# YujiaoShi/HighlyAccurate

Measured on AMD Instinct MI355X. Metric: image-pairs/sec through N-iter LM pose loop, KITTI shapes, higher is better.
Workload: dtype bf16; 1 GPU; BASELINE configs[1]: LM_S2GP.forward(mode='test'), sat 512x512, grd 256x1024, VGG-16 two-branch, level 3, 5 LM iters x 3 levels, 3-DoF, random-init weights; pairs_per_gpu=32, global_batch=32, parallelism=batch-sharded x1, no collective

## Files before the change

### highlyaccurate_amd/VGG.py

```python
from __future__ import annotations

import ctypes as C

import torch
import torch.nn as nn

from . import _lib

_W_ORDER = ['conv0', 'conv2', 'conv5', 'conv7', 'conv10', 'conv12', 'conv14',
            'conv_dec1.1', 'conv_dec1.3', 'conv_dec2.1', 'conv_dec2.3', 'conv_dec3.1', 'conv_dec3.3',
            'conf0.1', 'conf1.1', 'conf2.1', 'conf3.1']
_LEVEL_SEL = {-1: [0], -2: [1], -3: [2], 2: [1, 2], 3: [0, 1, 2], 4: [0, 1, 2, 3]}
_CH = (256, 128, 64, 16)


def _dtype_code(precision: str) -> int:
    if precision == 'bf16':
        return _lib.HLA_BF16
    if precision == 'fp16':
        return _lib.HLA_F16
    if precision == 'fp32':
        return _lib.HLA_F32
    if precision == 'fp16x3':
        return _lib.HLA_F16X3
    raise ValueError(f"precision must be 'fp32', 'fp16x3', 'bf16' or 'fp16', got {precision!r}")


def _param_table(module: 'VGGUnet'):
    sd = dict(module.named_parameters())
    prm = _lib.VggParams()
    keep, versions = [], []
    pad = {11: (64, 128), 12: (64, 64), 16: (1, 64)}
    for i, name in enumerate(_W_ORDER):
        w = sd[name + '.weight']
        versions.append((w.data_ptr(), w._version))
        w = w.detach().contiguous().float()
        if i in pad:
            if module.level != 4:
                continue
            wp = torch.zeros(pad[i][0], pad[i][1], 3, 3, device=w.device, dtype=torch.float32)
            wp[:w.shape[0], :w.shape[1]] = w
            w = wp
        keep.append(w)
        prm.w[i] = w.data_ptr()
        if i < 7:
            b = sd[name + '.bias']
            if i == 0:
                versions.append((b.data_ptr(), b._version))
            b = b.detach().contiguous().float()
            keep.append(b)
            prm.b[i] = b.data_ptr()
    return prm, keep, tuple(versions)


def _packed_weights(module: 'VGGUnet', prm, versions, dt: int, device):
    key = (dt, str(device), versions)
    cache = module.__dict__.setdefault('_hla_packed', {})
    if cache.get('key') != key:
        lib = _lib.load()
        buf = cache.get('buf')
        nbytes = lib.hla_vgg_packed_weight_bytes(dt)
        if buf is None or buf.numel() != nbytes or buf.device != device:
            buf = torch.empty(nbytes, dtype=torch.uint8, device=device)
        _lib.check(lib.hla_vgg_pack_weights(C.byref(prm), _lib.ptr(buf), dt, _lib.stream_ptr()), 'hla_vgg_pack_weights')
        cache['key'], cache['buf'] = key, buf
    return cache['buf']


def _alloc(*shape, dtype, device):
    return torch.empty(*shape, dtype=dtype, device=device)


def _image_window(x: torch.Tensor):
    x = x.float()
    B, _, H, W = x.shape
    sb, sc, sh, sw = x.stride()
    if not (sw == 1 and sh == W and sc >= H * W and (B == 1 or sb == 3 * sc)):
        x = x.contiguous()
        sc = H * W
    return x, sc


@_lib.on_device(lambda module, x, *a, **k: x)
def vgg_forward_nhwc(module: 'VGGUnet', x: torch.Tensor, want_conf: bool = True, defer_norm: bool = False,
                     save_for_backward: bool = False, first_row8: int = 0, feat16: bool = False, first_col32: int = 0,
                     col_state: dict = None):
    _lib.require_gpu(x, 'VGGUnet input')
    if x.dim() != 4 or x.shape[1] != 3:
        raise ValueError(f'expected [B,3,H,W], got {tuple(x.shape)}')
    lib = _lib.load()
    x, x_plane = _image_window(x)
    B, _, H, W = x.shape
    _lib.same_device(('input', x), ('parameters', module.conv0.weight))
    dt = _dtype_code(module.precision)
    prm, keep, versions = _param_table(module)
    packed = _packed_weights(module, prm, versions, dt, x.device)
    L = 4 if module.level == 4 else 3
    fdt = torch.float32
    if feat16:
        if not (defer_norm and not save_for_backward and L == 3 and dt in (_lib.HLA_BF16, _lib.HLA_F16)):
            raise ValueError("feat16 needs precision 'bf16' / 'fp16', defer_norm=True, level 3 and no save_for_backward")
        fdt = torch.float16
    fold = bool(getattr(module, 'folded', False))
    if fold:
        if feat16 or first_row8:
            raise ValueError('VGGUnet_G2S: feat16 / first_row8 do not apply to the folded maps')
        if W % 16:
            raise ValueError(f'VGGUnet_G2S folds [h,w] -> [2h,w/2] down to the W/8-wide map: W must be a multiple of 16, got {W}')

    def hw(l, folded):
        h, w = H >> (3 - l), W >> (3 - l)
        return (2 * h, w // 2) if folded else (h, w)

    feats = [_alloc(B, *hw(l, fold), 64 if l == 3 else _CH[l], device=x.device, dtype=fdt) for l in range(L)]
    confs = [torch.empty(B, *hw(l, fold and l > 0), device=x.device, dtype=torch.float32) if want_conf else None
             for l in range(L)]
    inv_norm = torch.empty(L, B, device=x.device, dtype=torch.float64)
    fp = (C.c_void_p * 4)(*([f.data_ptr() for f in feats] + [0] * (4 - L)))
    cp = (C.c_void_p * 4)(*([(c.data_ptr() if c is not None else 0) for c in confs] + [0] * (4 - L)))
    flags = (_lib.HLA_VGG_WANT_CONF if want_conf else 0) | (_lib.HLA_VGG_DEFER_NORM if defer_norm else 0) | \
            (_lib.HLA_VGG_FEAT16 if feat16 else 0) | (_lib.HLA_VGG_FOLD_DECODER if fold else 0)
    nbytes = lib.hla_vgg_workspace_bytes_flags(B, H, W, L, dt, flags) if fold else lib.hla_vgg_workspace_bytes(B, H, W, L, dt)
    ws = _alloc(nbytes, dtype=torch.uint8, device=x.device)
    if save_for_backward:
        if not defer_norm:
            raise ValueError('save_for_backward needs defer_norm=True (the backward works on the raw maps)')
        flags |= _lib.HLA_VGG_SAVE_FOR_BACKWARD
    c32 = _check_first_col32(first_col32, W)
    rc = lib.hla_vgg_forward_cols(_lib.ptr(x), x_plane, C.byref(prm), _lib.ptr(packed), fp, cp, _lib.ptr(inv_norm), _lib.ptr(ws), nbytes,
                                  B, H, W, L, dt, flags, int(first_row8), c32, None, _lib.stream_ptr())
    _lib.check(rc, 'hla_vgg_forward')
    if col_state is not None:
        col_state.update(x=x, x_plane=x_plane, prm=prm, keep=keep, packed=packed, feats=feats, inv_norm=inv_norm, ws=ws, B=B, H=H, W=W,
                         L=L, dt=dt, flags=flags, first_row8=int(first_row8), first_col32=c32)
    if save_for_backward:
        return feats, confs, inv_norm, dict(x=x, x_version=x._version, x_plane=x_plane, ws=ws, feats=feats, inv_norm=inv_norm, dt=dt, L=L)
    return feats, confs, inv_norm


def _check_first_col32(first_col32, W: int) -> int:
    c = int(first_col32)
    if c < 0 or (c > 0 and 128 * c >= W):
        raise ValueError(f'first_col32 must be 0 or leave a column of the maps (128 * first_col32 < W = {W}), got {first_col32}')
    return c


def promised_cols(first_col32: int):
    c = int(first_col32)
    return (16 * c + 2, 32 * c + 6, 64 * c + 14) if c > 0 else (0, 0, 0)


@_lib.on_device(lambda state, gate, *a, **k: gate)
def vgg_fixup_nhwc(state: dict, gate: torch.Tensor, one_launch: bool = True) -> None:
    s = state
    if not s or not s['first_col32']:
        return
    if gate.dtype != torch.int32 or gate.numel() != s['B'] or not gate.is_contiguous() or gate.device != s['x'].device:
        raise ValueError('gate must be a contiguous int32 [B] tensor on the device of the maps')
    L = s['L']
    fp = (C.c_void_p * 4)(*([f.data_ptr() for f in s['feats']] + [0] * (4 - L)))
    rc = _lib.load().hla_vgg_fixup(_lib.ptr(s['x']), s['x_plane'], C.byref(s['prm']), _lib.ptr(s['packed']), fp,
                                   _lib.ptr(s['inv_norm']), _lib.ptr(s['ws']), s['ws'].numel(), s['B'], s['H'], s['W'], L, s['dt'],
                                   s['flags'], s['first_row8'], s['first_col32'], _lib.ptr(gate), 1 if one_launch else 0,
                                   _lib.stream_ptr())
    _lib.check(rc, 'hla_vgg_fixup')


@_lib.on_device(lambda modules, xs, *a, **k: xs[0])
def vgg_forward_pair_nhwc(modules, xs, first_row8=(0, 0), feat16: bool = False, first_col32=(0, 0), col_state: dict = None):
    lib = _lib.load()
    if len(modules) != 2 or len(xs) != 2:
        raise ValueError('vgg_forward_pair_nhwc takes two modules and two images')
    dt = _dtype_code(modules[0].precision)
    if _dtype_code(modules[1].precision) != dt or any(m.level == 4 or getattr(m, 'folded', False) for m in modules):
        raise ValueError('vgg_forward_pair_nhwc: two unfolded extractors of one precision, level 3')
    if feat16 and dt not in (_lib.HLA_BF16, _lib.HLA_F16):
        raise ValueError("feat16 needs precision 'bf16' / 'fp16'")
    if xs[0].dim() != 4 or xs[1].dim() != 4 or xs[0].shape[1] != 3 or xs[1].shape[1] != 3 or xs[0].shape[0] != xs[1].shape[0]:
        raise ValueError(f'expected two [B,3,H,W] images with one B, got {tuple(xs[0].shape)} and {tuple(xs[1].shape)}')
    br = (_lib.VggBranch * 2)()
    keep, out = [], []
    for k, (module, x) in enumerate(zip(modules, xs)):
        _lib.require_gpu(x, 'VGGUnet input')
        x, x_plane = _image_window(x)
        B, _, H, W = x.shape
        _lib.same_device(('input', x), ('parameters', module.conv0.weight), ('first input', xs[0]))
        prm, kp, versions = _param_table(module)
        packed = _packed_weights(module, prm, versions, dt, x.device)
        feats = [_alloc(B, H >> (3 - l), W >> (3 - l), _CH[l], device=x.device, dtype=torch.float16 if feat16 else torch.float32)
                 for l in range(3)]
        inv_norm = torch.empty(3, B, device=x.device, dtype=torch.float64)
        nbytes = lib.hla_vgg_workspace_bytes(B, H, W, 3, dt)
        ws = _alloc(nbytes, dtype=torch.uint8, device=x.device)
        b = br[k]
        b.x, b.x_plane, b.params, b.packed_weights = x.data_ptr(), x_plane, C.pointer(prm), packed.data_ptr()
        for l in range(3):
            b.feat[l] = feats[l].data_ptr()
        b.inv_norm, b.workspace, b.workspace_bytes = inv_norm.data_ptr(), ws.data_ptr(), nbytes
        b.H, b.W, b.first_row8, b.first_col32 = H, W, int(first_row8[k]), _check_first_col32(first_col32[k], W)
        keep += [x, prm, kp, packed, ws]
        out.append((feats, inv_norm))
        if k == 0 and col_state is not None:
            col_state.update(x=x, x_plane=x_plane, prm=prm, keep=kp, packed=packed, feats=feats, inv_norm=inv_norm, ws=ws, B=B, H=H, W=W,
                             L=3, dt=dt, flags=_lib.HLA_VGG_DEFER_NORM | (_lib.HLA_VGG_FEAT16 if feat16 else 0),
                             first_row8=int(first_row8[k]), first_col32=b.first_col32)
    flags = _lib.HLA_VGG_DEFER_NORM | (_lib.HLA_VGG_FEAT16 if feat16 else 0)
    paired = C.c_int(0)
    rc = lib.hla_vgg_forward_pair(br, xs[0].shape[0], 3, dt, flags, C.byref(paired), _lib.stream_ptr())
    _lib.check(rc, 'hla_vgg_forward_pair')
    return out[0], out[1], bool(paired.value)


@_lib.on_device(lambda module, ctx, *a, **k: ctx['x'])
def vgg_backward_nhwc(module: 'VGGUnet', ctx: dict, d_feats, confs=None, d_confs=None, scale_invariant: bool = False,
                      first_row8: int = 0, flat: bool = False, dense: bool = False, stats: dict = None,
                      wgrad_two_phase: int = 0, workspace: torch.Tensor = None):
    lib = _lib.load()
    x, dt = ctx['x'], ctx['dt']
    if x._version != ctx.get('x_version', x._version):
        raise RuntimeError('the input image saved for the backward of VGGUnet has been modified by an inplace operation '
                           f"(version {x._version}, expected {ctx['x_version']}): conv0's weight gradient reads it again")
    B, _, H, W = x.shape
    prm, keep, versions = _param_table(module)
    cache = module.__dict__.setdefault('_hla_packed_T', {})
    key = (dt, str(x.device), versions)
    if cache.get('key') != key:
        buf = torch.empty(lib.hla_vgg_packed_weight_T_bytes(dt), dtype=torch.uint8, device=x.device)
        _lib.check(lib.hla_vgg_pack_weights_T(C.byref(prm), _lib.ptr(buf), dt, _lib.stream_ptr()), 'hla_vgg_pack_weights_T')
        cache['key'], cache['buf'] = key, buf
    sd = dict(module.named_parameters())
    grads, gs = {}, _lib.VggGrads()
    shapes = [(name + '.weight', tuple(sd[name + '.weight'].shape)) for name in _W_ORDER[:11]] + \
             [(name + '.bias', tuple(sd[name + '.bias'].shape)) for name in _W_ORDER[:7]]
    sizes = [int(torch.Size(shp).numel()) for _, shp in shapes]
    flat_buf = torch.empty(sum(sizes), device=x.device, dtype=torch.float32)
    o = 0
    for (key, shp), n in zip(shapes, sizes):
        grads[key] = flat_buf[o:o + n].view(shp)
        o += n
    for i, name in enumerate(_W_ORDER[:11]):
        gs.dw[i] = grads[name + '.weight'].data_ptr()
        if i < 7:
            gs.db[i] = grads[name + '.bias'].data_ptr()
    L = ctx.get('L', 3)
    padded = {}
    if L == 4:
        for i, name, shape in ((11, 'conv_dec3.1', (64, 128, 3, 3)), (12, 'conv_dec3.3', (64, 64, 3, 3))):
            g = torch.empty(shape, device=x.device, dtype=torch.float32)
            padded[name + '.weight'] = g
            gs.dw[i] = g.data_ptr()
    cp = dcp = None
    if d_confs is not None:
        dcs = [d.contiguous().float() for d in d_confs]
        cp = (C.c_void_p * 4)(*([c.data_ptr() for c in confs] + [0] * (4 - L)))
        dcp = (C.c_void_p * 4)(*([d.data_ptr() for d in dcs] + [0] * (4 - L)))
        for l in range(L):
            name = f'conf{l}.1.weight'
            if l == 3:
                g = torch.empty(1, 64, 3, 3, device=x.device, dtype=torch.float32)
                padded[name] = g
            else:
                g = torch.empty_like(sd[name], dtype=torch.float32, memory_format=torch.contiguous_format)
                grads[name] = g
            gs.dw[13 + l] = g.data_ptr()
    dfs = [d.contiguous().float() for d in d_feats]
    fp = (C.c_void_p * 4)(*([f.data_ptr() for f in ctx['feats']] + [0] * (4 - L)))
    dp = (C.c_void_p * 4)(*([d.data_ptr() for d in dfs] + [0] * (4 - L)))
    fold = bool(getattr(module, 'folded', False))
    nbytes = lib.hla_vgg_bwd_workspace_bytes_flags(B, H, W, L, dt, _lib.HLA_VGG_BWD_FOLD_DECODER) if fold \
        else lib.hla_vgg_bwd_workspace_bytes(B, H, W, L, dt)
    if workspace is None:
        ws = torch.empty(nbytes, dtype=torch.uint8, device=x.device)
    else:
        ws = workspace
        if ws.dtype != torch.uint8 or ws.device != x.device or not ws.is_contiguous():
            raise ValueError('workspace must be a contiguous uint8 tensor on the device of the input')
        if ws.numel() < nbytes:
            raise ValueError(f'workspace too small: {ws.numel()} bytes, the backward needs {nbytes}')
    rc = lib.hla_vgg_backward(_lib.ptr(x), ctx.get('x_plane', 0), C.byref(prm), _lib.ptr(cache['buf']), _lib.ptr(ctx['ws']), fp, _lib.ptr(ctx['inv_norm']),
                              dp, cp, dcp, C.byref(gs), _lib.ptr(ws), nbytes, B, H, W, L, dt,
                              (_lib.HLA_VGG_BWD_SCALE_INVARIANT if scale_invariant else 0)
                              | (_lib.HLA_VGG_BWD_DENSE if dense else 0)
                              | (_lib.HLA_VGG_BWD_WGRAD_TWO_PHASE if int(wgrad_two_phase) & 1 else 0)
                              | (_lib.HLA_VGG_BWD_WGRAD0_UNFUSED if int(wgrad_two_phase) & 2 else 0)
                              | (_lib.HLA_VGG_BWD_FOLD_DECODER if getattr(module, 'folded', False) else 0),
                              int(first_row8), _lib.stream_ptr())
    _lib.check(rc, 'hla_vgg_backward')
    if stats is not None and fold:
        stats['live_tiles'], stats['total_tiles'] = 0, 0
    elif stats is not None:
        torch.cuda.current_stream().synchronize()
        live, total = C.c_longlong(0), C.c_longlong(0)
        _lib.check(lib.hla_vgg_backward_live_tiles(_lib.ptr(ws), B, H, W, L, dt, C.byref(live), C.byref(total)),
                   'hla_vgg_backward_live_tiles')
        stats['live_tiles'], stats['total_tiles'] = live.value, total.value
    for name, g in padded.items():
        co, ci = sd[name].shape[:2]
        grads[name] = g[:co, :ci].contiguous()
    return (grads, flat_buf) if flat else grads


class VGGUnet(nn.Module):
    def __init__(self, level, estimate_depth=0, precision: str = 'fp32'):
        super().__init__()
        if estimate_depth:
            raise NotImplementedError('estimate_depth=1 (Ford height heads, VGG.py:85-118) is out of scope')
        if level not in _LEVEL_SEL:
            raise NotImplementedError(f'VGGUnet level {level}: the reference defines -1, -2, -3, 2, 3, 4')
        self.level = level
        _dtype_code(precision)
        self.precision = precision

        def c(ci, co, bias):
            return nn.Conv2d(ci, co, kernel_size=(3, 3), stride=(1, 1), padding=1, bias=bias)

        self.conv0, self.conv2 = c(3, 64, True), c(64, 64, True)
        self.conv5, self.conv7 = c(64, 128, True), c(128, 128, True)
        self.conv10, self.conv12, self.conv14 = c(128, 256, True), c(256, 256, True), c(256, 256, True)
        self.conv_dec1 = nn.Sequential(nn.ReLU(inplace=True), c(384, 128, False), nn.ReLU(inplace=True), c(128, 128, False))
        self.conv_dec2 = nn.Sequential(nn.ReLU(inplace=True), c(192, 64, False), nn.ReLU(inplace=True), c(64, 64, False))
        self.conv_dec3 = nn.Sequential(nn.ReLU(inplace=True), c(128, 32, False), nn.ReLU(inplace=True), c(32, 16, False))
        self.conf0 = nn.Sequential(nn.ReLU(), c(256, 1, False), nn.Sigmoid())
        self.conf1 = nn.Sequential(nn.ReLU(), c(128, 1, False), nn.Sigmoid())
        self.conf2 = nn.Sequential(nn.ReLU(), c(64, 1, False), nn.Sigmoid())
        self.conf3 = nn.Sequential(nn.ReLU(), c(16, 1, False), nn.Sigmoid())

    def forward(self, x):
        if torch.is_grad_enabled() and any(p.requires_grad for p in self.parameters()):
            names = [n for n, _ in self.named_parameters()]
            out = _VggFn.apply(self, names, x, *[p for _, p in self.named_parameters()])
            L = len(out) // 2
            feats, confs = list(out[:L]), list(out[L:])
        else:
            feats, confs, _ = vgg_forward_nhwc(self, x, want_conf=True)
        sel = _LEVEL_SEL[self.level]
        view = lambda i: (feats[i][..., :_CH[i]] if i == 3 else feats[i]).permute(0, 3, 1, 2)
        return [view(i) for i in sel], [confs[i].unsqueeze(1) for i in sel]


class VGGUnet_G2S(VGGUnet):
    folded = True

    def __init__(self, level, precision: str = 'fp32'):
        super().__init__(level, precision=precision)


class _VggFn(torch.autograd.Function):

    @staticmethod
    def forward(ctx, module, names, x, *params):
        feats, confs, inv, c = vgg_forward_nhwc(module, x, want_conf=True, defer_norm=True, save_for_backward=True)
        B = x.shape[0]
        normed = [(f.double() * inv[l].view(B, 1, 1, 1)).float() for l, f in enumerate(feats)]
        ctx.module, ctx.names, ctx.saved, ctx.n_levels = module, names, c, len(confs)
        confs = tuple(confs)
        ctx.save_for_backward(*confs)
        return tuple(normed) + confs

    @staticmethod
    def backward(ctx, *grads):
        c = ctx.saved
        if c is None:
            raise RuntimeError('VGGUnet: backward through the same forward twice (the saved activations were released after the '
                               'first backward; retain_graph is not supported by the HIP backward)')
        confs = list(ctx.saved_tensors)
        L = ctx.n_levels
        d_feats = [g if g is not None else torch.zeros_like(c['feats'][l]) for l, g in enumerate(grads[:L])]
        d_confs = [g if g is not None else torch.zeros_like(confs[l]) for l, g in enumerate(grads[L:])]
        g = vgg_backward_nhwc(ctx.module, c, d_feats, confs, d_confs, scale_invariant=False)
        ctx.saved = None
        return (None, None, None) + tuple(g.get(n) for n in ctx.names)


def L2_norm(x):
    B = x.shape[0]
    n = x.reshape(B, -1).norm(dim=1).clamp_min(1e-12)
    return x / n.view(B, 1, 1, 1)
```

### highlyaccurate_amd/_lib.py

```python
from __future__ import annotations

import ctypes as C
import os

import torch

HERE = os.path.dirname(os.path.abspath(__file__))
LIB_PATH = os.environ.get('HLA_LIB') or os.path.join(HERE, 'libhla.so')

HLA_F32, HLA_BF16, HLA_F16, HLA_F16X3 = 0, 1, 2, 3
HLA_VGG_WANT_CONF, HLA_VGG_DEFER_NORM, HLA_VGG_SAVE_FOR_BACKWARD, HLA_VGG_FEAT16 = 1, 2, 4, 8
HLA_VGG_FOLD_DECODER = 16
HLA_VGG_BWD_SCALE_INVARIANT = 1
HLA_VGG_BWD_DENSE = 2
HLA_VGG_BWD_WGRAD_TWO_PHASE = 4
HLA_VGG_BWD_WGRAD0_UNFUSED = 8
HLA_VGG_BWD_FOLD_DECODER = 16
ABI_VERSION = 32


class HlaError(RuntimeError):
    pass


class VggParams(C.Structure):
    _fields_ = [('w', C.c_void_p * 17), ('b', C.c_void_p * 7)]


class S2GLevel(C.Structure):
    _fields_ = [('sat_feat', C.c_void_p), ('grd_feat', C.c_void_p), ('grd_conf', C.c_void_p), ('xyz', C.c_void_p),
                ('sat_inv_norm', C.c_void_p), ('grd_inv_norm', C.c_void_p),
                ('A', C.c_int), ('h', C.c_int), ('w', C.c_int), ('C', C.c_int), ('row0', C.c_int), ('grd_row_skip', C.c_int),
                ('meter_per_pixel', C.c_double), ('centre', C.c_double), ('feat_dtype', C.c_int),
                ('ray', C.c_void_p), ('depth', C.c_void_p), ('depth_row', C.c_void_p), ('depth_col', C.c_void_p),
                ('depth_h', C.c_int), ('depth_w', C.c_int)]


class S2GConfig(C.Structure):
    _fields_ = [('ford', C.c_int), ('n_levels', C.c_int), ('n_iters', C.c_int), ('level_first', C.c_int),
                ('using_weight', C.c_int), ('use_hessian', C.c_int), ('dof', C.c_int),
                ('shift_range_lat', C.c_double), ('shift_range_lon', C.c_double), ('rotation_range', C.c_double),
                ('damping', C.c_double * 3), ('keep', C.c_void_p), ('keep_stride', C.c_size_t),
                ('optimizer', C.c_int), ('beta1', C.c_double), ('beta2', C.c_double), ('count_in_view', C.c_int),
                ('grd_grad_overwrite', C.c_int), ('deterministic', C.c_int), ('proj', C.c_int),
                ('reach_mode', C.c_int), ('reach_flag', C.c_void_p), ('reach_col0', C.c_int * 4)]


class VggBranch(C.Structure):
    _fields_ = [('x', C.c_void_p), ('x_plane', C.c_size_t), ('params', C.POINTER(VggParams)), ('packed_weights', C.c_void_p),
                ('feat', C.c_void_p * 4), ('conf', C.c_void_p * 4), ('inv_norm', C.c_void_p), ('workspace', C.c_void_p),
                ('workspace_bytes', C.c_size_t), ('H', C.c_int), ('W', C.c_int), ('first_row8', C.c_int),
                ('first_col32', C.c_int)]


class FillRegion(C.Structure):
    _fields_ = [('ptr', C.c_void_p), ('chunk_bytes', C.c_size_t), ('stride_bytes', C.c_size_t), ('n_chunks', C.c_int)]


class VggGrads(C.Structure):
    _fields_ = [('dw', C.c_void_p * 17), ('db', C.c_void_p * 7)]


class S2GLevelGrad(C.Structure):
    _fields_ = [('d_sat_feat', C.c_void_p), ('d_grd_feat', C.c_void_p), ('d_grd_conf', C.c_void_p)]


class ProfRecord(C.Structure):
    _fields_ = [('kernel_id', C.c_int), ('ms', C.c_float), ('flops', C.c_double), ('bytes', C.c_double)]


HLA_POSE_LOSS_F32, HLA_POSE_LOSS_F64 = 0, 1


class PoseLossArgs(C.Structure):
    _fields_ = [('x', C.c_void_p * 3), ('x_stride', (C.c_longlong * 3) * 3), ('gt', C.c_void_p * 3), ('gt_stride', C.c_longlong * 3),
                ('coe', C.c_double * 3), ('B', C.c_int), ('N', C.c_int), ('L', C.c_int), ('gt_dtype', C.c_int)]


_lib = None


def _check_binary(lib: C.CDLL, path: str) -> None:
    lib.hla_abi_version.restype = C.c_int
    have = lib.hla_abi_version()
    if have != ABI_VERSION:
        raise HlaError(f'{path}: ABI version {have}, this binding needs {ABI_VERSION}; rebuild it '
                       f'(python -m highlyaccurate_amd.build --force)')
    try:
        fn = lib.hla_sizeof_struct
    except AttributeError:
        raise HlaError(f'{path}: no hla_sizeof_struct export; rebuild it') from None
    fn.restype, fn.argtypes = C.c_size_t, [C.c_int]
    for sid, cls in enumerate((VggParams, VggGrads, S2GLevel, S2GConfig, S2GLevelGrad, ProfRecord, PoseLossArgs, FillRegion,
                                VggBranch)):
        if fn(sid) != C.sizeof(cls):
            raise HlaError(f'{path}: sizeof({cls.__name__}) is {fn(sid)} in the library and {C.sizeof(cls)} in the binding')


def load() -> C.CDLL:
    global _lib
    if _lib is not None:
        return _lib
    from . import build as _b
    try:
        want = _b.source_hash()
    except _b.SourcesMissing as e:
        if not os.path.exists(LIB_PATH):
            raise HlaError(f'{LIB_PATH} is missing and so are its sources: {e}') from None
        want = _b.lib_hash(LIB_PATH)
    if _b.lib_hash(LIB_PATH) != want and not (os.environ.get('HLA_LIB') and os.environ.get('HLA_ALLOW_STALE') == '1'):
        if os.environ.get('HLA_LIB'):
            raise HlaError(f'{LIB_PATH} (HLA_LIB) was not built from the sources in {_b.CSRC}; rebuild it')
        if not _b.have_compiler():
            what = 'is missing' if not os.path.exists(LIB_PATH) else 'is stale (built from different sources)'
            raise HlaError(f'{LIB_PATH} {what} and there is no hipcc to rebuild it; highlyaccurate_amd has no fallback path')
        _b.build()
    lib = C.CDLL(LIB_PATH)
    _check_binary(lib, LIB_PATH)
    vp, i, sz = C.c_void_p, C.c_int, C.c_size_t
    lib.hla_last_error.restype = C.c_char_p
    lib.hla_source_hash.restype = C.c_char_p
    lib.hla_vgg_workspace_bytes.restype = sz
    lib.hla_vgg_workspace_bytes.argtypes = [i, i, i, i, i]
    lib.hla_vgg_workspace_bytes_flags.restype = sz
    lib.hla_vgg_workspace_bytes_flags.argtypes = [i, i, i, i, i, i]
    lib.hla_vgg_forward.restype = i
    lib.hla_vgg_forward.argtypes = [vp, sz, C.POINTER(VggParams), vp, C.POINTER(vp), C.POINTER(vp), vp, vp, sz,
                                    i, i, i, i, i, i, i, vp]
    lib.hla_vgg_forward_cols.restype = i
    lib.hla_vgg_forward_cols.argtypes = [vp, sz, C.POINTER(VggParams), vp, C.POINTER(vp), C.POINTER(vp), vp, vp, sz,
                                         i, i, i, i, i, i, i, i, vp, vp]
    lib.hla_vgg_fixup.restype = i
    lib.hla_vgg_fixup.argtypes = [vp, sz, C.POINTER(VggParams), vp, C.POINTER(vp), vp, vp, sz, i, i, i, i, i, i, i, i, vp, i, vp]
    lib.hla_vgg_forward_pair.restype = i
    lib.hla_vgg_forward_pair.argtypes = [C.POINTER(VggBranch), i, i, i, i, C.POINTER(i), vp]
    lib.hla_vgg_packed_weight_bytes.restype = sz
    lib.hla_vgg_packed_weight_bytes.argtypes = [i]
    lib.hla_vgg_pack_weights.restype = i
    lib.hla_vgg_pack_weights.argtypes = [C.POINTER(VggParams), vp, i, vp]
    lib.hla_vgg_packed_weight_T_bytes.restype = sz
    lib.hla_vgg_packed_weight_T_bytes.argtypes = [i]
    lib.hla_vgg_pack_weights_T.restype = i
    lib.hla_vgg_pack_weights_T.argtypes = [C.POINTER(VggParams), vp, i, vp]
    lib.hla_vgg_bwd_workspace_bytes.restype = sz
    lib.hla_vgg_bwd_workspace_bytes.argtypes = [i, i, i, i, i]
    lib.hla_vgg_bwd_workspace_bytes_flags.restype = sz
    lib.hla_vgg_bwd_workspace_bytes_flags.argtypes = [i, i, i, i, i, i]
    lib.hla_vgg_backward_live_tiles.restype = i
    lib.hla_vgg_backward_live_tiles.argtypes = [vp, i, i, i, i, i, C.POINTER(C.c_longlong), C.POINTER(C.c_longlong)]
    lib.hla_vgg_backward.restype = i
    lib.hla_vgg_backward.argtypes = [vp, sz, C.POINTER(VggParams), vp, vp, C.POINTER(vp), vp, C.POINTER(vp), C.POINTER(vp), C.POINTER(vp), C.POINTER(VggGrads),
                                     vp, sz, i, i, i, i, i, i, i, vp]
    lib.hla_resize_bilinear.restype = i
    lib.hla_resize_bilinear.argtypes = [vp, vp, vp, i, vp, vp, i, vp, vp, i, i, i, i, i, vp]
    lib.hla_sat_tile.restype = i
    lib.hla_sat_tile.argtypes = [vp, vp, vp, i, i, i, vp]
    lib.hla_grid_sample.restype = i
    lib.hla_grid_sample.argtypes = [vp, vp, vp, vp, vp, i, i, i, i, i, i, i, vp]
    lib.hla_grid_sample_bwd.restype = i
    lib.hla_grid_sample_bwd.argtypes = [vp, vp, vp, vp, vp, vp, vp, vp, i, i, i, i, i, i, i, vp]
    lib.hla_s2g_workspace_bytes.restype = sz
    lib.hla_s2g_workspace_bytes.argtypes = [C.POINTER(S2GConfig), C.POINTER(S2GLevel), i]
    lib.hla_g2s_workspace_bytes.restype = sz
    lib.hla_g2s_workspace_bytes.argtypes = [C.POINTER(S2GConfig), C.POINTER(S2GLevel), i]
    lib.hla_g2s_lm_solve.restype = i
    lib.hla_g2s_lm_solve.argtypes = [C.POINTER(S2GConfig), C.POINTER(S2GLevel), vp, i, i, vp, vp, vp, vp, sz, i, vp]
    lib.hla_g2s_pose_score_workspace_bytes.restype = sz
    lib.hla_g2s_pose_score_workspace_bytes.argtypes = [C.POINTER(S2GConfig), C.POINTER(S2GLevel), i, i]
    lib.hla_g2s_pose_score.restype = i
    lib.hla_g2s_pose_score.argtypes = [C.POINTER(S2GConfig), C.POINTER(S2GLevel), vp, i, i, vp, i, vp, vp, vp, sz, i, vp]
    lib.hla_g2s_pose_score_bwd_workspace_bytes.restype = sz
    lib.hla_g2s_pose_score_bwd_workspace_bytes.argtypes = [C.POINTER(S2GConfig), C.POINTER(S2GLevel), i, i]
    lib.hla_g2s_pose_score_bwd.restype = i
    lib.hla_g2s_pose_score_bwd.argtypes = [C.POINTER(S2GConfig), C.POINTER(S2GLevel), C.POINTER(S2GLevelGrad), vp, i, i, vp, i,
                                           vp, vp, vp, sz, i, vp]
    lib.hla_g2s_bwd_workspace_bytes.restype = sz
    lib.hla_g2s_bwd_workspace_bytes.argtypes = [C.POINTER(S2GConfig), C.POINTER(S2GLevel), i]
    lib.hla_g2s_lm_solve_bwd.restype = i
    lib.hla_g2s_lm_solve_bwd.argtypes = [C.POINTER(S2GConfig), C.POINTER(S2GLevel), C.POINTER(S2GLevelGrad), vp, i, i, vp, vp,
                                         vp, vp, vp, vp, sz, i, vp]
    lib.hla_s2g_lm_solve.restype = i
    lib.hla_s2g_lm_solve.argtypes = [C.POINTER(S2GConfig), C.POINTER(S2GLevel), vp, vp, vp, vp, vp, vp, vp, sz, i, vp]
    lib.hla_s2g_pose_score_workspace_bytes.restype = sz
    lib.hla_s2g_pose_score_workspace_bytes.argtypes = [C.POINTER(S2GConfig), C.POINTER(S2GLevel), i, i]
    lib.hla_s2g_pose_score.restype = i
    lib.hla_s2g_pose_score.argtypes = [C.POINTER(S2GConfig), C.POINTER(S2GLevel), vp, vp, vp, i, vp, vp, vp, sz, i, vp]
    lib.hla_s2g_pose_score_bwd_workspace_bytes.restype = sz
    lib.hla_s2g_pose_score_bwd_workspace_bytes.argtypes = [C.POINTER(S2GConfig), C.POINTER(S2GLevel), i, i]
    lib.hla_s2g_pose_score_bwd.restype = i
    lib.hla_s2g_pose_score_bwd.argtypes = [C.POINTER(S2GConfig), C.POINTER(S2GLevel), C.POINTER(S2GLevelGrad), vp, vp, vp, i, vp, vp,
                                           vp, sz, i, vp]
    lib.hla_s2g_bwd_workspace_bytes.restype = sz
    lib.hla_s2g_bwd_workspace_bytes.argtypes = [C.POINTER(S2GConfig), C.POINTER(S2GLevel), i]
    lib.hla_s2g_lm_solve_bwd.restype = i
    lib.hla_s2g_lm_solve_bwd.argtypes = [C.POINTER(S2GConfig), C.POINTER(S2GLevel), C.POINTER(S2GLevelGrad), vp, vp, vp, vp,
                                         vp, vp, vp, vp, sz, i, vp]
    lib.hla_zero_fill.restype = i
    lib.hla_zero_fill.argtypes = [C.POINTER(FillRegion), i, i, vp]
    lib.hla_pose_loss.restype = i
    lib.hla_pose_loss.argtypes = [C.POINTER(PoseLossArgs), vp, vp]
    lib.hla_pose_loss_bwd.restype = i
    lib.hla_pose_loss_bwd.argtypes = [C.POINTER(PoseLossArgs), C.POINTER(vp), C.POINTER(vp), C.POINTER((C.c_longlong * 3) * 3), vp]
    ll, dbl = C.c_longlong, C.c_double
    lib.hla_orien_corr_workspace_bytes.restype = sz
    lib.hla_orien_corr_workspace_bytes.argtypes = [i, i, i, i, i]
    lib.hla_orien_corr.restype = i
    lib.hla_orien_corr.argtypes = [vp, vp, vp, vp, vp, vp, vp, vp, vp, sz, i, i, i, i, i, vp]
    lib.hla_orien_corr_bwd.restype = i
    lib.hla_orien_corr_bwd.argtypes = [vp, vp, vp, vp, vp, vp, vp, vp, vp, vp, vp, sz, i, i, i, i, i, vp]
    lib.hla_orien_window_bwd.restype = i
    lib.hla_orien_window_bwd.argtypes = [vp, vp, vp, vp, i, i, i, i, i, i, vp]
    lib.hla_orien_triplet_loss.restype = i
    lib.hla_orien_triplet_loss.argtypes = [vp, vp, ll, dbl, dbl, vp, i, i, i, vp]
    lib.hla_orien_triplet_loss_bwd.restype = i
    lib.hla_orien_triplet_loss_bwd.argtypes = [vp, vp, ll, dbl, dbl, vp, vp, i, i, vp]
    lib.hla_g2s_corr_workspace_bytes.restype = sz
    lib.hla_g2s_corr_workspace_bytes.argtypes = [i, i, i, i, i]
    lib.hla_g2s_corr.restype = i
    lib.hla_g2s_corr.argtypes = [vp, vp, vp, vp, vp, vp, vp, vp, vp, sz, i, i, i, i, i, vp]
    lib.hla_g2s_corr_bwd.restype = i
    lib.hla_g2s_corr_bwd.argtypes = [vp, vp, vp, vp, vp, vp, vp, vp, vp, vp, vp, sz, i, i, i, i, i, vp]
    lib.hla_g2s_corr_triplet_loss.restype = i
    lib.hla_g2s_corr_triplet_loss.argtypes = [vp, vp, ll, vp, ll, dbl, dbl, dbl, vp, i, i, i, i, vp]
    lib.hla_g2s_corr_triplet_loss_bwd.restype = i
    lib.hla_g2s_corr_triplet_loss_bwd.argtypes = [vp, vp, ll, vp, ll, dbl, dbl, dbl, vp, vp, i, i, i, vp]
    lib.hla_prof_enable.restype = i
    lib.hla_prof_enable.argtypes = [i]
    lib.hla_prof_kernel_name.restype = C.c_char_p
    lib.hla_prof_kernel_name.argtypes = [i]
    lib.hla_prof_mfma_peak.restype = i
    lib.hla_prof_mfma_peak.argtypes = [i, i, C.c_float, C.POINTER(C.c_float), vp]
    lib.hla_prof_fetch.restype = i
    lib.hla_prof_fetch.argtypes = [C.POINTER(ProfRecord), i, C.POINTER(i)]
    _lib = lib
    return lib


def zero_fill(regions, max_blocks: int = 0, stream=None) -> None:
    if not regions:
        return
    arr = (FillRegion * len(regions))()
    for k, (t, cb, sb, n) in enumerate(regions):
        arr[k].ptr = t.data_ptr() if hasattr(t, 'data_ptr') else int(t)
        arr[k].chunk_bytes, arr[k].stride_bytes, arr[k].n_chunks = int(cb), int(sb), int(n)
    check(load().hla_zero_fill(arr, len(regions), int(max_blocks), stream_ptr() if stream is None else stream), 'hla_zero_fill')


def prof_enable(on: bool) -> None:
    load().hla_prof_enable(1 if on else 0)


def prof_fetch(max_records: int = 1 << 16):
    lib = load()
    buf = (ProfRecord * max_records)()
    n = C.c_int(0)
    lib.hla_prof_fetch(buf, max_records, C.byref(n))
    return [(lib.hla_prof_kernel_name(buf[k].kernel_id).decode(), buf[k].ms, buf[k].flops, buf[k].bytes)
            for k in range(n.value)]


def check(rc: int, what: str) -> None:
    if rc != 0:
        raise HlaError(f'{what} failed (status {rc}): {load().hla_last_error().decode()}')


def stream_ptr() -> C.c_void_p:
    return C.c_void_p(torch.cuda.current_stream().cuda_stream)


def on_device(pick):
    import functools

    def deco(fn):
        @functools.wraps(fn)
        def wrapper(*a, **k):
            t = pick(*a, **k)
            if t is None or not t.is_cuda:
                return fn(*a, **k)
            if torch.cuda.current_device() == t.device.index:
                return fn(*a, **k)
            with torch.cuda.device(t.device):
                return fn(*a, **k)
        return wrapper
    return deco


def same_device(*named) -> None:
    devs = {(n, str(t.device)) for n, t in named if t is not None}
    if len({d for _, d in devs}) > 1:
        raise ValueError('all inputs and the model must be on one device, got ' + ', '.join(f'{n}: {d}' for n, d in sorted(devs)))


def require_gpu(t: torch.Tensor, name: str) -> None:
    if not t.is_cuda:
        raise HlaError(f'{name} must live on the HIP device (got {t.device}); highlyaccurate_amd has no CPU path')


def image_pair(sat_map, grd_img, param, gpu: bool = True) -> None:
    if gpu:
        require_gpu(sat_map, 'sat_map')
        require_gpu(grd_img, 'grd_img')
    if sat_map.dim() != 4 or grd_img.dim() != 4 or sat_map.shape[0] != grd_img.shape[0] or sat_map.shape[1] != 3 \
            or grd_img.shape[1] != 3 or sat_map.shape[2] != sat_map.shape[3]:
        raise ValueError(f'expected sat_map [B,3,A,A] and grd_img [B,3,H,W] with one B, got {tuple(sat_map.shape)} '
                         f'and {tuple(grd_img.shape)}')
    same_device(('sat_map', sat_map), ('grd_img', grd_img), ('parameters', param))


def ptr(t) -> C.c_void_p:
    return C.c_void_p(0 if t is None else t.data_ptr())


def mfma_sustained_tflops(dtype_code: int, data: int, ms_target: float = 8.0) -> float:
    out = C.c_float(0.0)
    check(load().hla_prof_mfma_peak(dtype_code, data, ms_target, C.byref(out), stream_ptr()), 'hla_prof_mfma_peak')
    return float(out.value)
```

### highlyaccurate_amd/_s2gp.py

```python
from __future__ import annotations

import ctypes as C

import numpy as np
import torch
import torch.nn as nn

from . import _lib, _pose, utils
from ._autograd import _side_stream, extract_saved, extractor_grads, grad_params, take_state
from ._pose import _poses_arg, eligible_cost, pose_grid
from .VGG import VGGUnet, vgg_forward_nhwc, vgg_forward_pair_nhwc, vgg_fixup_nhwc, promised_cols

KITTI_K = [[582.9802, 0.0, 496.2420], [0.0, 482.7076, 125.0034], [0.0, 0.0, 1.0]]
FORD_K_FL = [945.391406, 0.0, 855.502825, 0.0, 945.668274, 566.372868, 0.0, 0.0, 1.0]
FORD_H_FL, FORD_W_FL = 860, 1656


_FEAT_DTYPES = {torch.float32: _lib.HLA_F32, torch.bfloat16: _lib.HLA_BF16, torch.float16: _lib.HLA_F16}

PHASE_HOOK = None


def _phase(name: str):
    h = PHASE_HOOK
    if h is not None:
        h(name)


def _camera_rays(K_ori, grd_H, grd_W, ori_H, ori_W):
    K = torch.tensor(K_ori, dtype=torch.float32).reshape(1, 3, 3)
    Ks = K.clone()
    Ks[:, :1, :] = K[:, :1, :] * grd_W / ori_W
    Ks[:, 1:2, :] = K[:, 1:2, :] * grd_H / ori_H
    Kinv = torch.inverse(Ks)
    v, u = torch.meshgrid(torch.arange(0, grd_H, dtype=torch.float32),
                          torch.arange(0, grd_W, dtype=torch.float32), indexing='ij')
    uv1 = torch.stack([u, v, torch.ones_like(u)], dim=-1).unsqueeze(0)
    return torch.sum(Kinv[:, None, None, :, :] * uv1[:, :, :, None, :], dim=-1)


def ray_table(K_ori, grd_H, grd_W, ori_H, ori_W):
    return _camera_rays(K_ori, grd_H, grd_W, ori_H, ori_W)[0].contiguous()


def ground_plane_table(K_ori, grd_H, grd_W, ori_H, ori_W):
    xyz_w = _camera_rays(K_ori, grd_H, grd_W, ori_H, ori_W)
    y = xyz_w[..., 1:2]
    w = utils.Camera_height / torch.where(torch.abs(y) > utils.EPS, y, utils.EPS * torch.ones_like(y))
    return (xyz_w * w)[0].contiguous()


def nearest_indices(n_in: int, n_out: int):
    scale = np.float32(n_in) / np.float32(n_out)
    src = np.floor(np.arange(n_out, dtype=np.float32) * scale).astype(np.int64)
    return torch.from_numpy(np.minimum(src, n_in - 1).astype(np.int32))


def polar_plane_table(grd_H, grd_W):
    v, u = torch.meshgrid(torch.arange(0, grd_H, dtype=torch.float32),
                          torch.arange(0, grd_W, dtype=torch.float32), indexing='ij')
    theta = u / grd_W * np.pi / 4
    radius = (1 - v / grd_H) * 30
    z = radius * torch.cos(np.pi / 4 - theta)
    x = -radius * torch.sin(np.pi / 4 - theta)
    y = utils.Camera_height * torch.ones_like(z)
    return torch.stack([x, y, z], dim=-1).contiguous()


def ford_K_network_input():
    K = torch.tensor(FORD_K_FL, dtype=torch.float32).reshape(3, 3)
    out = torch.zeros_like(K)
    out[0] = K[0] / FORD_W_FL * 1024
    out[1] = K[1] / FORD_H_FL * 256
    out[2] = K[2]
    return out.tolist()


def _loss_tensor_ops(shift_lats, shift_lons, thetas, gt_shift_lat, gt_shift_lon, gt_theta, coe_shift_lat, coe_shift_lon, coe_theta):
    d_lat = torch.abs(shift_lats - gt_shift_lat[:, None, None]).mean(dim=0)
    d_lon = torch.abs(shift_lons - gt_shift_lon[:, None, None]).mean(dim=0)
    d_th = torch.abs(thetas - gt_theta[:, None, None]).mean(dim=0)
    losses = coe_shift_lat * d_lat + coe_shift_lon * d_lon + coe_theta * d_th
    return (losses.mean(), losses[0] - losses[-1], d_lat[0] - d_lat[-1], d_lon[0] - d_lon[-1], d_th[0] - d_th[-1],
            losses[-1], d_lat[-1], d_lon[-1], d_th[-1])


def _pose_loss_args(xs, gts, coes):
    a = _lib.PoseLossArgs()
    B, N, L = xs[0].shape
    for k in range(3):
        a.x[k], a.gt[k], a.gt_stride[k], a.coe[k] = xs[k].data_ptr(), gts[k].data_ptr(), gts[k].stride(0), float(coes[k])
        for j in range(3):
            a.x_stride[k][j] = xs[k].stride(j)
    a.B, a.N, a.L = B, N, L
    a.gt_dtype = _lib.HLA_POSE_LOSS_F64 if gts[0].dtype == torch.float64 else _lib.HLA_POSE_LOSS_F32
    return a


class _PoseLossFn(torch.autograd.Function):

    @staticmethod
    def forward(ctx, cols, coes, gt_lat, gt_lon, gt_th, *xs):
        views = [xs[0][..., c] for c in cols] if cols is not None else list(xs)
        gts = (gt_lat, gt_lon, gt_th)
        L = views[0].shape[2]
        out = torch.empty(1 + 8 * L, dtype=gt_lat.dtype, device=views[0].device)
        args = _pose_loss_args(views, gts, coes)
        _lib.check(_lib.load().hla_pose_loss(C.byref(args), _lib.ptr(out), _lib.stream_ptr()), 'hla_pose_loss')
        ctx.save_for_backward(*xs, *gts)
        ctx.cols, ctx.coes = cols, coes
        ctx.set_materialize_grads(False)
        return (out[0],) + tuple(out[1 + j * L:1 + (j + 1) * L] for j in range(8))

    @staticmethod
    @torch.autograd.function.once_differentiable
    def backward(ctx, *g):
        cols, saved = ctx.cols, ctx.saved_tensors
        nx = 1 if cols is not None else 3
        xs, gts = saved[:nx], saved[nx:]
        if cols is not None:
            d = torch.empty_like(xs[0]) if xs[0].shape[-1] == 3 and len(set(cols)) == 3 else torch.zeros_like(xs[0])
            views, dviews, grads = [xs[0][..., c] for c in cols], [d[..., c] for c in cols], (d,)
        else:
            views = list(xs)
            grads = tuple(torch.empty(x.shape, dtype=torch.float32, device=x.device) for x in xs)
            dviews = list(grads)
        args = _pose_loss_args(views, gts, ctx.coes)
        vp = C.c_void_p
        gp, keep = (vp * 9)(), []
        for j, t in enumerate(g):
            if t is not None:
                t = t.to(gts[0].dtype).contiguous()
                keep.append(t)
                gp[j] = t.data_ptr()
        dp = (vp * 3)(*[v.data_ptr() for v in dviews])
        ds = ((C.c_longlong * 3) * 3)()
        for k in range(3):
            for j in range(3):
                ds[k][j] = dviews[k].stride(j)
        _lib.check(_lib.load().hla_pose_loss_bwd(C.byref(args), gp, dp, C.byref(ds), _lib.stream_ptr()), 'hla_pose_loss_bwd')
        return (None,) * 5 + grads


def _pose_loss(cols, xs, gts, coes):
    views = [xs[0][..., c] for c in cols] if cols is not None else list(xs)
    fused = (all(isinstance(c, (int, float)) for c in coes)
             and all(v.is_cuda and v.dtype == torch.float32 and v.dim() == 3 and v.shape == views[0].shape for v in views)
             and all(t.is_cuda and t.device == views[0].device and t.dtype == gts[0].dtype and t.dim() == 1
                     and t.shape[0] == views[0].shape[0] and not t.requires_grad for t in gts)
             and gts[0].dtype in (torch.float32, torch.float64) and 0 < views[0].shape[1] * views[0].shape[2] <= 512
             and views[0].shape[0] > 0)
    if not fused:
        return _loss_tensor_ops(*views, *gts, *coes)
    with torch.cuda.device(views[0].device):
        return _PoseLossFn.apply(cols, tuple(float(c) for c in coes), *gts, *xs)


def loss_func(loss_method, ref_feat_list, pred_feat_dict, gt_feat_dict, shift_lats, shift_lons, thetas,
              gt_shift_lat, gt_shift_lon, gt_theta, pred_uv_dict, gt_uv_dict,
              coe_shift_lat=100, coe_shift_lon=100, coe_theta=100, coe_L1=100, coe_L2=100, coe_L3=100, coe_L4=100):
    if loss_method != 0:
        raise NotImplementedError('only loss_method=0 is supported (the reference marks 1-3 as failed trials)')
    out = _pose_loss(None, (shift_lats, shift_lons, thetas), (gt_shift_lat, gt_shift_lon, gt_theta),
                     (coe_shift_lat, coe_shift_lon, coe_theta))
    return (*out, None, None, None, None)


def loss_from_trace(loss_method, trace, cols, gt_shift_lat, gt_shift_lon, gt_theta, coe_shift_lat, coe_shift_lon, coe_theta):
    if loss_method != 0:
        raise NotImplementedError('only loss_method=0 is supported (the reference marks 1-3 as failed trials)')
    out = _pose_loss(tuple(cols), (trace,), (gt_shift_lat, gt_shift_lon, gt_theta), (coe_shift_lat, coe_shift_lon, coe_theta))
    return (*out, None, None, None, None)


class S2GPBase(nn.Module):
    ford = False

    def __init__(self, args):
        super().__init__()
        self.args = args
        self.level = args.level
        self.N_iters = args.N_iters
        self.using_weight = args.using_weight
        self.loss_method = args.loss_method
        if args.level not in ((2, 3, 4) if self.ford else (3, 4)):
            raise NotImplementedError('args.level must be 3 (x15, x18, x21) or 4 (+ x24)' +
                                      (', or 2 (x18, x21)' if self.ford else "; the reference's KITTI model is shape-inconsistent at level 2"))
        proj = getattr(args, 'proj', 'geo')
        if proj not in ('geo', 'polar'):
            raise NotImplementedError(f"{type(self).__name__}: proj must be 'geo' or 'polar', got {proj!r} (the reference runs its "
                                      "polar branch for any other string, 'nn' and 'CrossAttn' included: that accident is not copied)")
        self.polar = proj == 'polar'
        if self.polar and self.ford and args.level == 2:
            raise NotImplementedError("LM_S2GP_Ford(level=2, proj='polar'): the reference pairs the whole-map loop with the "
                                      "ground-plane tables there; that combination is not built (use level 3 or 4)")
        opt = getattr(args, 'Optimizer', 'LM')
        allowed = ('LM', 'GN') if self.ford else ('LM', 'SGD', 'ADAM')
        if opt not in allowed:
            raise NotImplementedError(f"{type(self).__name__}: Optimizer must be one of {allowed} ('NN' needs the NNrefine "
                                      f"network: out of scope; the reference's Ford SGD_update raises as shipped)")
        if getattr(args, 'estimate_depth', 0):
            raise NotImplementedError('estimate_depth (Ford height heads, VGG.py:85-118) is out of scope')
        precision = getattr(args, 'precision', 'fp32')
        self.SatFeatureNet = VGGUnet(self.level, precision=precision)
        self.GrdFeatureNet = VGGUnet(self.level, precision=precision)
        if self.ford or args.rotation_range > 0:
            self.damping = nn.Parameter(torch.zeros(size=(1, 3), dtype=torch.float32))
        else:
            self.damping = nn.Parameter(torch.zeros(size=(), dtype=torch.float32))
        self.meters_per_pixel = [utils.get_meter_per_pixel() * (2 ** (3 - l)) for l in range(4)]
        self._tables = {}
        self._reach = {}
        self._ray_tables = {}
        self._depth_idx = {}
        self.last_trace = None
        self.last_normal_eq = None
        self.last_keep = None
        self.keep_normal_eq = False
        self.keep_features = False
        self.last_features = None
        self.last_reach_flag = None
        self.last_search = None
        self.last_score_loss = None

    def xyz_tables(self, grd_H: int, grd_W: int, device):
        key = (grd_H, grd_W, str(device))
        if key not in self._tables:
            K = ford_K_network_input() if self.ford else KITTI_K
            hw = [(grd_H / 2 ** (3 - l), grd_W / 2 ** (3 - l)) for l in range(4)]
            self._tables[key] = [(polar_plane_table(h, w) if self.polar else ground_plane_table(K, h, w, 256, 1024)).to(device)
                                 for h, w in hw]
        return self._tables[key][1:3] if self.level == 2 else self._tables[key]

    def ray_tables(self, grd_H: int, grd_W: int, device):
        key = (grd_H, grd_W, str(device))
        if key not in self._ray_tables:
            K = ford_K_network_input() if self.ford else KITTI_K
            self._ray_tables[key] = [ray_table(K, grd_H / 2 ** (3 - l), grd_W / 2 ** (3 - l), 256, 1024).to(device) for l in range(4)]
        return self._ray_tables[key][1:3] if self.level == 2 else self._ray_tables[key]

    def depth_indices(self, h: int, w: int, dH: int, dW: int, device):
        key = (h, w, dH, dW, str(device))
        if key not in self._depth_idx:
            self._depth_idx[key] = (nearest_indices(dH, h).to(device), nearest_indices(dW, w).to(device))
        return self._depth_idx[key]

    def _depth_arg(self, gt_depth, B: int, device):
        if gt_depth is None:
            return None
        if self.polar:
            raise NotImplementedError("proj='polar' with a depth map: the reference's polar tables have no camera rays to lift "
                                      "(models_kitti.py:742 raises IndexError)")
        if gt_depth.dim() != 3 or gt_depth.shape[0] != B or gt_depth.shape[1] < 1 or gt_depth.shape[2] < 1:
            raise ValueError(f'gt_depth must be [B,dH,dW] with B = {B}, got {tuple(gt_depth.shape)}')
        return gt_depth.detach().to(device).float().contiguous()

    def sat_first_col32(self, A: int, grd_H: int, grd_W: int) -> int:
        a = self.args
        if self.ford or self.polar or self.level != 3 or A % 8:
            return 0
        key = (A, grd_H, grd_W, float(a.shift_range_lat), float(a.shift_range_lon), float(a.rotation_range))
        if key not in self._reach:
            tables = [t.cpu() for t in self.xyz_tables(grd_H, grd_W, 'cpu')]
            mpp = [utils.get_meter_per_pixel() * utils.get_process_satmap_sidelength() / (A >> (3 - l)) for l in range(3)]
            cols = sat_reach(tables[:3], [A >> (3 - l) for l in range(3)], mpp, key[3], key[4], key[5])
            self._reach[key] = first_col32_of_reach(cols, A)
        return self._reach[key]

    def _levels(self, maps):
        if self.level != 2 or maps is None:
            return maps
        return maps[1:]

    def _config(self, n_levels: int, level_first: int) -> _lib.S2GConfig:
        a = self.args
        cfg = _lib.S2GConfig()
        cfg.ford = 1 if self.ford else 0
        cfg.n_levels, cfg.n_iters, cfg.level_first = n_levels, self.N_iters, 1 if level_first else 0
        cfg.optimizer = {'LM': 0, 'SGD': 1, 'ADAM': 2, 'GN': 3}[getattr(a, 'Optimizer', 'LM')]
        cfg.using_weight = 1 if (self.using_weight and cfg.optimizer in (0, 3)) else 0
        cfg.use_hessian = 1 if getattr(a, 'use_hessian', 0) else 0
        if self.ford:
            cfg.dof = 3
        elif a.rotation_range == 0:
            cfg.dof = 2
        elif a.shift_range_lat == 0 and a.shift_range_lon == 0:
            cfg.dof = 1
        else:
            cfg.dof = 3
        cfg.shift_range_lat, cfg.shift_range_lon = float(a.shift_range_lat), float(a.shift_range_lon)
        cfg.rotation_range = float(a.rotation_range)
        cfg.beta1, cfg.beta2 = float(getattr(a, 'beta1', 0.9)), float(getattr(a, 'beta2', 0.999))
        if getattr(a, 'train_damping', 0):
            lam = (10.0 ** (-6 + torch.sigmoid(self.damping.detach().double()) * 11.0)).reshape(-1).tolist()
        else:
            lam = [float(a.damping)] * 3
        lam = (lam + lam + lam)[:3]
        if not self.ford and cfg.dof == 1 and getattr(a, 'train_damping', 0):
            lam = [lam[0]] * 3
        for i in range(3):
            cfg.damping[i] = lam[i]
        return cfg

    def _draw_reinit(self, n_steps: int, B: int, device):
        return draw_reinit(n_steps, B, device)

    def _draw_dropout(self, lv, level_first, device):
        if not getattr(self.args, 'dropout', 0) or getattr(self.args, 'Optimizer', 'LM') != 'LM':
            return None
        L, N = len(lv), self.N_iters
        order = [l for l in range(L) for _ in range(N)] if level_first else [l for _ in range(N) for l in range(L)]
        npix = [(lv[l].h - lv[l].row0) * lv[l].w for l in range(L)]
        keep = np.zeros((len(order), max(npix)), np.uint8)
        for k, l in enumerate(order):
            inds = np.random.permutation(np.arange(npix[l]))[: npix[l] // 2]
            keep[k, inds] = 1
        return torch.from_numpy(keep).to(device)

    def _lm_structs(self, sat_feats, grd_feats, grd_confs, grd_hw, extra, level_first, sat_inv_norm, grd_inv_norm, depth=None):
        dev = sat_feats[0].device
        L = len(sat_feats)
        tables = self.xyz_tables(grd_hw[0], grd_hw[1], dev)
        rays = self.ray_tables(grd_hw[0], grd_hw[1], dev) if depth is not None else None
        cfg = self._config(L, level_first)
        lv = (_lib.S2GLevel * L)()
        for l in range(L):
            s, g = sat_feats[l], grd_feats[l]
            A, w, Cn = s.shape[1], g.shape[2], g.shape[3]
            h = tables[l].shape[0]
            row0 = 0 if self.polar else h // 2
            skip = h - g.shape[1]
            if not (s.shape[2] == A and s.shape[3] == Cn and tuple(tables[l].shape) == (h, w, 3) and 0 <= skip <= row0
                    and g.shape[0] == s.shape[0] and s.is_contiguous() and g.is_contiguous()
                    and s.dtype == g.dtype and s.dtype in _FEAT_DTYPES):
                raise ValueError(f'level {l}: inconsistent feature maps sat {tuple(s.shape)} / grd {tuple(g.shape)} '
                                 f'for a {tuple(grd_hw)} ground image')
            lv[l].sat_feat, lv[l].grd_feat, lv[l].feat_dtype = s.data_ptr(), g.data_ptr(), _FEAT_DTYPES[s.dtype]
            lv[l].grd_conf = grd_confs[l].data_ptr() if (self.using_weight and grd_confs[l] is not None) else 0
            lv[l].xyz = tables[l].data_ptr()
            if depth is not None:
                ri, ci = self.depth_indices(h, w, depth.shape[1], depth.shape[2], dev)
                lv[l].ray, lv[l].depth, lv[l].depth_row, lv[l].depth_col = rays[l].data_ptr(), depth.data_ptr(), ri.data_ptr(), ci.data_ptr()
                lv[l].depth_h, lv[l].depth_w = depth.shape[1], depth.shape[2]
            lv[l].sat_inv_norm = sat_inv_norm[l].data_ptr() if sat_inv_norm is not None else 0
            lv[l].grd_inv_norm = grd_inv_norm[l].data_ptr() if grd_inv_norm is not None else 0
            lv[l].A, lv[l].h, lv[l].w, lv[l].C, lv[l].row0, lv[l].grd_row_skip = A, h, w, Cn, row0, skip
            if self.ford:
                lv[l].meter_per_pixel = float(extra['side_m']) / A
                lv[l].centre = float(A // 2)
            else:
                lv[l].meter_per_pixel = utils.get_meter_per_pixel() * utils.get_process_satmap_sidelength() / A
                lv[l].centre = A / 2.0
        R_FL = extra['R_FL'].to(dev).float().contiguous() if self.ford else None
        T_FL = extra['T_FL'].to(dev).float().contiguous() if self.ford else None
        return cfg, lv, R_FL, T_FL

    @_lib.on_device(lambda self, sat_feats, *a, **k: sat_feats[0])
    def lm_solve(self, sat_feats, grd_feats, grd_confs, grd_hw, extra=None, level_first=0, init_pose=None,
                 sat_inv_norm=None, grd_inv_norm=None, keep_normal_eq=None, gt_depth=None, reach=None):
        lib = _lib.load()
        dev = sat_feats[0].device
        B, L = sat_feats[0].shape[0], len(sat_feats)
        depth = self._depth_arg(gt_depth, B, dev)
        cfg, lv, R_FL, T_FL = self._lm_structs(sat_feats, grd_feats, grd_confs, grd_hw, extra, level_first,
                                               sat_inv_norm, grd_inv_norm, depth)
        steps = L * self.N_iters
        reinit = (self.ford or cfg.dof == 3) and cfg.optimizer in (0, 3)
        rand_uv = self._draw_reinit(steps, B, dev) if reinit else None
        self.last_keep = self._draw_dropout(lv, level_first, dev)
        if self.last_keep is not None:
            cfg.keep, cfg.keep_stride = self.last_keep.data_ptr(), self.last_keep.shape[1]
        trace = torch.empty(B, self.N_iters, L, 3, device=dev, dtype=torch.float32)
        strict = bool(getattr(self.args, 'strict_errors', 0))
        want_neq = strict or cfg.optimizer == 3 or (self.keep_normal_eq if keep_normal_eq is None else keep_normal_eq)
        cfg.count_in_view = 1 if strict else 0
        neq = torch.empty(steps, B, 16, device=dev, dtype=torch.float64) if want_neq else None
        nbytes = lib.hla_s2g_workspace_bytes(C.byref(cfg), lv, B)
        ws = torch.empty(nbytes, dtype=torch.uint8, device=dev)
        p0 = init_pose.to(dev).float().contiguous() if init_pose is not None else None
        flag = None
        if reach is not None:
            flag = torch.empty(B, dtype=torch.int32, device=dev)
            cfg.reach_mode, cfg.reach_flag = 1, flag.data_ptr()
            for l in range(L):
                cfg.reach_col0[l] = int(reach[0][l])
        rc = lib.hla_s2g_lm_solve(C.byref(cfg), lv, _lib.ptr(R_FL), _lib.ptr(T_FL), _lib.ptr(p0), _lib.ptr(rand_uv),
                                  _lib.ptr(trace), _lib.ptr(neq), _lib.ptr(ws), nbytes, B, _lib.stream_ptr())
        _lib.check(rc, 'hla_s2g_lm_solve')
        if reach is not None:
            reach[1](flag)
            cfg.reach_mode = 2
            rc = lib.hla_s2g_lm_solve(C.byref(cfg), lv, _lib.ptr(R_FL), _lib.ptr(T_FL), _lib.ptr(p0), _lib.ptr(rand_uv),
                                      _lib.ptr(trace), _lib.ptr(neq), _lib.ptr(ws), nbytes, B, _lib.stream_ptr())
            _lib.check(rc, 'hla_s2g_lm_solve (reach fallback)')
        self.last_reach_flag = flag
        risky = cfg.optimizer == 3 or (cfg.optimizer == 0 and (cfg.use_hessian or min(cfg.damping[i] for i in range(3)) <= 0.0))
        if risky or strict:
            raise_like_reference(trace, neq[:, :, 14] if strict else None, level_first,
                                 gn_norm2=neq[:, :, 0] if cfg.optimizer == 3 else None)
        self.last_trace, self.last_normal_eq = trace.detach(), neq
        return trace

    def lm_grad_buffers(self, sat_feats, grd_feats, grd_confs, row0s, row_skips, grd_first_row8=0, overwrite=True, deterministic=False):
        L = len(sat_feats)
        regions = []
        d_sat = [torch.empty_like(t) for t in sat_feats]
        if not deterministic:
            regions += [(d, d.numel() * 4, d.numel() * 4, 1) for d in d_sat]
        d_grd = []
        for l, t in enumerate(grd_feats):
            d = torch.empty_like(t)
            lo, hi = (max(0, (grd_first_row8 << l) - 2) if grd_first_row8 else 0), row0s[l] - row_skips[l]
            if not overwrite:
                hi = t.shape[1]
            if hi > lo:
                row = t.shape[2] * t.shape[3] * 4
                regions.append((d.data_ptr() + lo * row, (hi - lo) * row, t.shape[1] * row, t.shape[0]))
            d_grd.append(d)
        d_conf = [torch.empty_like(grd_confs[l]) if (self.using_weight and grd_confs[l] is not None) else None for l in range(L)]
        regions += [(d, d.numel() * 4, d.numel() * 4, 1) for d in d_conf if d is not None]
        d_lambda = torch.empty(4, device=sat_feats[0].device, dtype=torch.float64)
        keep = d_sat + d_grd
        for k0 in range(0, len(regions), 16):
            _lib.zero_fill(regions[k0:k0 + 16])
        del keep
        return d_sat, d_grd, d_conf, d_lambda

    @_lib.on_device(lambda self, sat_feats, *a, **k: sat_feats[0])
    def lm_backward(self, sat_feats, grd_feats, grd_confs, grd_hw, trace, normal_eq, d_trace, extra=None, level_first=0,
                    init_pose=None, sat_inv_norm=None, grd_inv_norm=None, keep=None, grd_first_row8=0, overwrite=True, gt_depth=None):
        lib = _lib.load()
        dev = sat_feats[0].device
        B, L = sat_feats[0].shape[0], len(sat_feats)
        depth = self._depth_arg(gt_depth, B, dev)
        cfg, lv, R_FL, T_FL = self._lm_structs(sat_feats, grd_feats, grd_confs, grd_hw, extra, level_first,
                                               sat_inv_norm, grd_inv_norm, depth)
        if keep is not None:
            cfg.keep, cfg.keep_stride = keep.data_ptr(), keep.shape[1]
        det = bool(getattr(self.args, 'deterministic_backward', 0))
        cfg.deterministic = 1 if det else 0
        cfg.grd_grad_overwrite = 1 if overwrite else 0
        d_sat, d_grd, d_conf, d_lambda = self.lm_grad_buffers(sat_feats, grd_feats, grd_confs, [lv[l].row0 for l in range(L)],
                                                              [lv[l].grd_row_skip for l in range(L)], grd_first_row8, overwrite, det)
        gr = (_lib.S2GLevelGrad * L)()
        for l in range(L):
            gr[l].d_sat_feat, gr[l].d_grd_feat = d_sat[l].data_ptr(), d_grd[l].data_ptr()
            gr[l].d_grd_conf = d_conf[l].data_ptr() if d_conf[l] is not None else 0
        dtr = d_trace.to(dev).float().contiguous()
        nbytes = lib.hla_s2g_bwd_workspace_bytes(C.byref(cfg), lv, B)
        ws = torch.empty(nbytes, dtype=torch.uint8, device=dev)
        p0 = init_pose.to(dev).float().contiguous() if init_pose is not None else None
        for attempt, bits in enumerate((1, 30) if det else (0,)):
            cfg.deterministic = bits
            if attempt:
                for t in d_conf:
                    if t is not None:
                        t.zero_()
                if not overwrite:
                    for t in d_grd:
                        t.zero_()
            rc = lib.hla_s2g_lm_solve_bwd(C.byref(cfg), lv, gr, _lib.ptr(R_FL), _lib.ptr(T_FL), _lib.ptr(p0), _lib.ptr(trace),
                                          _lib.ptr(normal_eq), _lib.ptr(dtr), _lib.ptr(d_lambda), _lib.ptr(ws), nbytes, B,
                                          _lib.stream_ptr())
            _lib.check(rc, 'hla_s2g_lm_solve_bwd')
            if not det or float(d_lambda[3]) == 0.0:
                break
        else:
            raise RuntimeError(f'deterministic_backward: the fixed-point range of d(loss)/d(sat map) was exceeded in {int(d_lambda[3])} '
                               '(step, sample) pairs even with 2^20 of head room -- the adjoints of the LM chain grow by more than that '
                               'from its last step to an earlier one; the result is not valid (run without args.deterministic_backward)')
        return d_sat, d_grd, d_conf, d_lambda[:3]

    def _score_structs(self, sat_feats, grd_feats, grd_confs, grd_hw, extra, sat_inv_norm, grd_inv_norm):
        cfg, lv, R_FL, T_FL = self._lm_structs(sat_feats, grd_feats, grd_confs, grd_hw, extra, 0, sat_inv_norm, grd_inv_norm)
        return cfg, lv, (R_FL, T_FL)

    @_lib.on_device(lambda self, sat_feats, *a, **k: sat_feats[0])
    def score_poses(self, sat_feats, grd_feats, grd_confs, grd_hw, poses, level, extra=None, sat_inv_norm=None, grd_inv_norm=None):
        structs = lambda: self._score_structs(sat_feats, grd_feats, grd_confs, grd_hw, extra, sat_inv_norm, grd_inv_norm)
        return _pose.score_poses('hla_s2g_pose_score', structs, sat_feats, poses, level)

    @_lib.on_device(lambda self, sat_feats, *a, **k: sat_feats[0])
    def score_poses_bwd(self, sat_feats, grd_feats, grd_confs, grd_hw, poses, level, sums, d_cost, extra=None, sat_inv_norm=None,
                        grd_inv_norm=None):
        structs = lambda: self._score_structs(sat_feats, grd_feats, grd_confs, grd_hw, extra, sat_inv_norm, grd_inv_norm)
        return _pose.score_poses_bwd('hla_s2g_pose_score_bwd', structs, sat_feats, grd_feats, grd_confs, poses, level, sums, d_cost)

    def _score_checks(self, what, sat_map, grd_img):
        if getattr(self.args, 'dropout', 0):
            raise NotImplementedError(f'{what} with args.dropout: a pose is scored on every pixel, the dropout loop on a random '
                                      'half -- their objectives differ')
        if self.level != 3:
            raise NotImplementedError(f'{what} is built for args.level = 3 (x15, x18, x21), got level {self.level}')
        _lib.image_pair(sat_map, grd_img, self.damping)

    @_lib.on_device(lambda self, sat_map, *a, **k: sat_map)
    def score_candidates(self, sat_map, grd_img, poses, levels=None, extra=None):
        self._score_checks('score_candidates', sat_map, grd_img)
        cand = _poses_arg(poses, sat_map.shape[0]).to(sat_map.device).contiguous()
        lvls = _pose.levels_arg(levels, self.level)
        under = grad_params(self)
        if under:
            out = _ScoreFn.apply(self, under[0], sat_map, grd_img, cand, lvls, extra, *under[1])
            return list(out[:len(lvls)]), list(out[len(lvls):])
        with torch.no_grad():
            sat_feats, sat_inv, grd_feats, grd_confs, grd_inv = self._features(sat_map, grd_img, bool(self.using_weight), False)
            res = [self.score_poses(sat_feats, grd_feats, grd_confs, grd_img.shape[-2:], cand, l, extra, sat_inv, grd_inv) for l in lvls]
        return [r[0] for r in res], [r[1] for r in res]

    def _score_loss(self, sat_map, grd_img, extra, candidates, gt_pose, levels, min_in_view):
        self._score_checks('score_loss', sat_map, grd_img)
        poses = _pose.true_pose_first(gt_pose, candidates, sat_map.shape[0], sat_map.device)
        costs, sums = self.score_candidates(sat_map, grd_img, poses, levels, extra)
        return _pose.score_loss_tail(self, costs, sums, min_in_view)

    @_lib.on_device(lambda self, sat_map, *a, **k: sat_map)
    def _search(self, sat_map, grd_img, extra, candidates, top_m, score_level, min_in_view, level_first):
        if getattr(self.args, 'dropout', 0):
            raise NotImplementedError('forward_search with args.dropout: a pose is scored on every pixel, the dropout loop on a '
                                      'random half -- their objectives differ')
        _lib.image_pair(sat_map, grd_img, self.damping)
        cand, M = _pose.search_candidates(candidates, top_m, sat_map)
        with torch.no_grad():
            sat_feats, sat_inv, grd_feats, grd_confs, grd_inv = self._features(sat_map, grd_img, bool(self.using_weight), False)
            hw = grd_img.shape[-2:]
            score = lambda poses, level: self.score_poses(sat_feats, grd_feats, grd_confs, hw, poses, level, extra, sat_inv, grd_inv)
            solve = lambda p0: self.lm_solve(sat_feats, grd_feats, grd_confs, hw, extra, level_first, p0, sat_inv, grd_inv)
            return _pose.search(self, cand, M, score, solve, score_level, len(sat_feats) - 1, min_in_view)

    def _features(self, sat_map, grd_img, want_conf, return_confs, sat_c32=0, col_state=None):
        f16 = (self.SatFeatureNet.precision in ('bf16', 'fp16') and self.level == 3 and bool(getattr(self.args, 'lm_feat16', 1)))
        small = sat_map.shape[0] <= int(getattr(self.args, 'small_batch_two_streams', 4))
        dead_ok = (not return_confs and self.level == 3 and getattr(self.args, 'Optimizer', 'LM') == 'LM'
                   and bool(getattr(self.args, 'ground_crop', 1)) and not self.polar)
        skip = dead_ground_rows(grd_img.shape[-2]) if dead_ok else 0
        grd_in = grd_img[:, :, skip:, :] if skip else grd_img
        f8 = ((grd_img.shape[-2] // 8) // 2 - skip // 8) if dead_ok else 0
        f8 = f8 if f8 >= 4 else 0
        if (not small and not want_conf and self.level != 4 and bool(getattr(self.args, 'pair_extractor_launches', 1))
                and self.GrdFeatureNet.precision == self.SatFeatureNet.precision):
            (sat_feats, sat_inv), (grd_feats, grd_inv), _ = vgg_forward_pair_nhwc(
                (self.SatFeatureNet, self.GrdFeatureNet), (sat_map, grd_in), first_row8=(0, f8), feat16=f16,
                first_col32=(sat_c32, 0), col_state=col_state)
            L = self._levels
            return L(sat_feats), L(sat_inv), L(grd_feats), L([None] * 3), L(grd_inv)
        if small:
            cur = torch.cuda.current_stream()
            side = _side_stream(sat_map.device)
            side.wait_stream(cur)
            with torch.cuda.stream(side):
                sat_feats, _, sat_inv = vgg_forward_nhwc(self.SatFeatureNet, sat_map, want_conf=False, defer_norm=True, feat16=f16,
                                                         first_col32=sat_c32, col_state=col_state)
            sat_map.record_stream(side)
        else:
            sat_feats, _, sat_inv = vgg_forward_nhwc(self.SatFeatureNet, sat_map, want_conf=False, defer_norm=True, feat16=f16,
                                                     first_col32=sat_c32, col_state=col_state)
        grd_feats, grd_confs, grd_inv = vgg_forward_nhwc(self.GrdFeatureNet, grd_in, want_conf=want_conf, defer_norm=True,
                                                         first_row8=f8, feat16=f16)
        if small:
            cur.wait_stream(side)
            for t in list(sat_feats) + [sat_inv]:
                t.record_stream(cur)
            if col_state:
                col_state['ws'].record_stream(cur)
        L = self._levels
        return L(sat_feats), L(sat_inv), L(grd_feats), L(grd_confs), L(grd_inv)

    @_lib.on_device(lambda self, sat_map, *a, **k: sat_map)
    def localise(self, sat_map, grd_img, want_conf, extra, level_first, init_pose, return_confs=True, gt_depth=None):
        _lib.image_pair(sat_map, grd_img, self.damping, gpu=False)
        gt_depth = self._depth_arg(gt_depth, sat_map.shape[0], sat_map.device)
        if self.polar and self.ford and level_first:
            raise NotImplementedError("LM_S2GP_Ford(proj='polar') with level_first=1: the reference's level-first loop reads only "
                                      "the bottom half of the polar maps (it has no proj branch); that combination is not built")
        under = grad_params(self)
        if under:
            out = _LocaliseFn.apply(self, under[0], sat_map, grd_img, want_conf, extra, level_first, init_pose, gt_depth, *under[1])
            return out[0], list(out[1:]) if want_conf else [None] * self.level
        a = self.args
        c32 = 0
        if (bool(getattr(a, 'sat_reach_crop', 1)) and not return_confs and not want_conf and gt_depth is None and not self.ford
                and not self.polar and self.level == 3 and getattr(a, 'Optimizer', 'LM') == 'LM'
                and not getattr(a, 'strict_errors', 0) and self.SatFeatureNet.precision != 'fp16x3'):
            c32 = self.sat_first_col32(sat_map.shape[-1], grd_img.shape[-2], grd_img.shape[-1])
        state = {} if c32 else None
        sat_feats, sat_inv, grd_feats, grd_confs, grd_inv = self._features(sat_map, grd_img, want_conf, return_confs, c32, state)
        reach = (promised_cols(c32), lambda flag: vgg_fixup_nhwc(state, flag, bool(getattr(a, 'fixup_one_launch', 1)))) if c32 else None
        trace = self.lm_solve(sat_feats, grd_feats, grd_confs, grd_img.shape[-2:], extra, level_first, init_pose,
                              sat_inv, grd_inv, gt_depth=gt_depth, reach=reach)
        if self.keep_features:
            self.last_features = (sat_feats, sat_inv, grd_feats, grd_inv)
        return trace, grd_confs


def draw_reinit(n_steps: int, B: int, device):
    r = torch.rand(n_steps, 2, B).mul_(2.0).add_(-1.0)
    if torch.device(device).type == 'cuda':
        return r.pin_memory().to(device, non_blocking=True)
    return r.to(device)


def raise_like_reference(trace, in_view, level_first, gn_norm2=None):
    B, N, L, _ = trace.shape
    steps = N * L
    tr = (trace.permute(0, 2, 1, 3) if level_first else trace).reshape(B, steps, 3)
    bad = ~torch.isfinite(tr).all(-1)
    if gn_norm2 is not None:
        first = torch.where(bad.any(1), bad.float().argmax(1), torch.full((B,), steps - 1, device=bad.device))
        poisoned = bad.any(1) & (gn_norm2.t().gather(1, first[:, None])[:, 0] == 0)
        bad = bad & ~poisoned[:, None]
    bad = bad.any(0)
    k_s = int(torch.nonzero(bad)[0]) if bool(bad.any()) else steps
    k_a = steps
    if in_view is not None:
        empty = in_view.sum(1) == 0
        k_a = int(torch.nonzero(empty)[0]) if bool(empty.any()) else steps
    if k_a < steps and k_a <= k_s:
        raise AssertionError(f'grid_sample: no pixel of the batch is sampled inside the map in LM step {k_a} (jacobian.py:172)')
    if k_s < steps:
        raise RuntimeError(f'linalg.inv: the normal matrix of LM step {k_s} is singular '
                           '(use_hessian / zero damping / Gauss-Newton with no Jacobian support in one pose component)')


def sat_reach(tables, sizes, mpp, shift_range_lat, shift_range_lon, rotation_range, n: int = 5):
    axis = np.linspace(-1.0, 1.0, n)
    out = []
    for t, A, m in zip(tables, sizes, mpp):
        t = np.asarray(t, dtype=np.float64)
        h = t.shape[0]
        P = t[h // 2:].reshape(-1, 3)
        P = P[P[:, 2] > 0]
        X, Z = P[:, 0], P[:, 2]
        best, im, ctr = float(A), 1.0 / m, A / 2.0
        for th in axis:
            ang = th * rotation_range / 180.0 * np.pi
            c, s = np.cos(ang), np.sin(ang)
            for su in axis * shift_range_lon:
                for sv in axis * shift_range_lat:
                    u = s * im * X + c * im * Z + (c * su - s * sv) * im + ctr
                    v = c * im * X - s * im * Z + (-c * sv - s * su) * im + ctr
                    ok = (u >= 0) & (u <= A - 1) & (v >= 0) & (v <= A - 1)
                    if ok.any():
                        best = min(best, float(np.floor(u[ok].min())))
        out.append(int(best))
    return out


def reach_walk(p0: int, p1: int, p2: int) -> dict:
    x18 = min(p1, (p2 - 2) >> 1)
    x15 = min(p0, (x18 - 2) >> 1)
    x8 = min(2 * x15 - 3, x18 - 2)
    x3 = min(2 * x8 - 2, p2 - 2)
    return {'x21': p2, 'dec2.1': p2 - 1, 'x18': x18, 'dec1.1': x18 - 1, 'x15': x15, 'conv14': 2 * x15, 'conv12': 2 * x15 - 1,
            'conv10': 2 * x15 - 2, 'x8': x8, 'conv7': 2 * x8, 'conv5': 2 * x8 - 1, 'x3': x3, 'conv2': 2 * x3}


_REACH_QUANTUM = {'x21': 64, 'dec2.1': 64, 'x18': 32, 'dec1.1': 32, 'x15': 16, 'conv14': 32, 'conv12': 32, 'conv10': 32, 'x8': 32,
                  'conv7': 64, 'conv5': 64, 'x3': 64, 'conv2': 128}


def first_col32_of_reach(cols, A: int) -> int:
    need = reach_walk(*[int(x) for x in cols])
    c = min(max(v, 0) // _REACH_QUANTUM[k] for k, v in need.items())
    return max(0, min(c, (A - 1) // 128))


def dead_ground_rows(H: int) -> int:
    return max(0, ((H // 2 - 34) // 8) * 8)


def _bwd_first_row8(model, grd_hw, x21_rows: int) -> int:
    inv = getattr(model.args, 'Optimizer', 'LM') == 'LM' and not model.polar
    f8 = (grd_hw[0] // 8) // 2 - (grd_hw[0] - x21_rows * 2) // 8
    return f8 if (inv and f8 >= 4 and model.level == 3 and bool(getattr(model.args, 'bwd_trim', 1))) else 0


class _LocaliseFn(torch.autograd.Function):

    @staticmethod
    def forward(ctx, model, names, sat_map, grd_img, want_conf, extra, level_first, init_pose, gt_depth, *params):
        sat_feats, _, sat_inv, cs = vgg_forward_nhwc(model.SatFeatureNet, sat_map, want_conf=False, defer_norm=True,
                                                     save_for_backward=True)
        _phase('fwd_sat')
        skip = 0
        if (getattr(model.args, 'train_ground_crop', 0) and model.level == 3 and getattr(model.args, 'Optimizer', 'LM') == 'LM'
                and not model.polar):
            skip = dead_ground_rows(grd_img.shape[-2])
        grd_in = grd_img[:, :, skip:, :] if skip else grd_img
        grd_feats, grd_confs, grd_inv, cg = vgg_forward_nhwc(model.GrdFeatureNet, grd_in, want_conf=want_conf,
                                                             defer_norm=True, save_for_backward=True)
        _phase('fwd_grd')
        L = model._levels
        ctx.conf0 = grd_confs[0] if (model.level == 2 and grd_confs is not None) else None
        sat_feats, sat_inv, grd_feats, grd_confs, grd_inv = L(sat_feats), L(sat_inv), L(grd_feats), L(grd_confs), L(grd_inv)
        trace = model.lm_solve(sat_feats, grd_feats, grd_confs, grd_img.shape[-2:], extra, level_first, init_pose,
                               sat_inv, grd_inv, keep_normal_eq=True, gt_depth=gt_depth)
        _phase('lm_fwd')
        ctx.model, ctx.names, ctx.extra, ctx.level_first, ctx.init_pose = model, names, extra, level_first, init_pose
        ctx.gt_depth = gt_depth
        ctx.state = (sat_feats, grd_feats, grd_confs, tuple(grd_img.shape[-2:]), trace.detach(), model.last_normal_eq, sat_inv, grd_inv, cs, cg,
                     model.last_keep)
        out_confs = ()
        if want_conf:
            out_confs = tuple(grd_confs)
            if skip:
                out_confs = tuple(torch.nn.functional.pad(c, (0, 0, skip >> (3 - l), 0)) for l, c in enumerate(grd_confs))
            ctx.mark_non_differentiable(*out_confs)
        ctx.set_materialize_grads(False)
        return (trace,) + out_confs

    @staticmethod
    def backward(ctx, d_trace, *unused):
        model = ctx.model
        _phase('loss')
        sat_feats, grd_feats, grd_confs, grd_hw, trace, neq, sat_inv, grd_inv, cs, cg, keep = take_state(ctx)
        if d_trace is None:
            d_trace = torch.zeros_like(trace)
        f8 = _bwd_first_row8(model, grd_hw, grd_feats[-1].shape[1])
        d_sat, d_grd, d_conf, d_lam = model.lm_backward(sat_feats, grd_feats, grd_confs, grd_hw, trace, neq, d_trace, ctx.extra,
                                                   ctx.level_first, ctx.init_pose, sat_inv, grd_inv, keep, grd_first_row8=f8,
                                                   gt_depth=ctx.gt_depth)
        _phase('lm_bwd')
        if model.level == 2:
            zf = lambda cx: torch.zeros_like(cx['feats'][0], dtype=torch.float32)
            d_sat, d_grd = [zf(cs)] + list(d_sat), [zf(cg)] + list(d_grd)
            if grd_confs is not None and all(c is not None for c in d_conf):
                grd_confs, d_conf = [ctx.conf0] + list(grd_confs), [torch.zeros_like(ctx.conf0)] + list(d_conf)
        a = model.args
        use_w = model.using_weight and all(c is not None for c in d_conf)
        grads = extractor_grads(model, cs, cg, d_sat, d_grd, grd_confs if use_w else None, d_conf if use_w else None,
                                scale_invariant=getattr(a, 'Optimizer', 'LM') == 'LM', first_row8=f8,
                                dense=not bool(getattr(a, 'bwd_trim', 1)), wgrad_two_phase=int(getattr(a, 'wgrad_two_phase', 0)),
                                stats=getattr(model, 'bwd_stats', None), two_streams=bool(getattr(a, 'bwd_two_streams', 1)))
        if getattr(a, 'train_damping', 0):
            d = model.damping.detach().double()
            sg = torch.sigmoid(d)
            lam = 10.0 ** (-6 + sg * 11.0)
            dlam_dd = lam * np.log(10.0) * 11.0 * sg * (1 - sg)
            if d.dim() == 0:
                n = 2 if a.rotation_range == 0 else 1
                grads['damping'] = (d_lam[:n].sum() * dlam_dd).float()
            else:
                grads['damping'] = (d_lam.view(1, 3) * dlam_dd).float()
            sync = getattr(model, 'grad_sync', None)
            if sync:
                sync.finish(sync.start({'damping': grads['damping']}))
        _phase('vgg_bwd')
        return (None,) * 9 + tuple(grads.get(n) for n in ctx.names)


class _ScoreFn(torch.autograd.Function):

    @staticmethod
    def forward(ctx, model, names, sat_map, grd_img, poses, levels, extra, *params):
        sat_feats, sat_inv, grd_feats, grd_confs, grd_inv, cs, cg = extract_saved(model, sat_map, grd_img, bool(model.using_weight))
        hw = tuple(grd_img.shape[-2:])
        res = [model.score_poses(sat_feats, grd_feats, grd_confs, hw, poses, l, extra, sat_inv, grd_inv) for l in levels]
        costs, sums = tuple(r[0] for r in res), tuple(r[1] for r in res)
        ctx.model, ctx.names, ctx.extra, ctx.levels = model, names, extra, levels
        ctx.state = (sat_feats, grd_feats, grd_confs, hw, poses, sums, sat_inv, grd_inv, cs, cg)
        ctx.mark_non_differentiable(*sums)
        ctx.set_materialize_grads(False)
        return costs + sums

    @staticmethod
    def backward(ctx, *d_out):
        model = ctx.model
        sat_feats, grd_feats, grd_confs, hw, poses, sums, sat_inv, grd_inv, cs, cg = take_state(ctx, 'score_candidates call')
        bwd = lambda n, l: model.score_poses_bwd(sat_feats, grd_feats, grd_confs, hw, poses, l, sums[n], d_out[n], ctx.extra,
                                                 sat_inv, grd_inv)
        d_sat, d_grd, d_conf = _pose.score_level_grads(model, bwd, ctx.levels, d_out, sat_feats, grd_feats, grd_confs)
        f8 = 0 if model.polar else _bwd_first_row8(model, hw, grd_feats[-1].shape[1])
        grads = extractor_grads(model, cs, cg, d_sat, d_grd, grd_confs if d_conf else None, d_conf, scale_invariant=True,
                                first_row8=f8, dense=not bool(getattr(model.args, 'bwd_trim', 1)),
                                wgrad_two_phase=int(getattr(model.args, 'wgrad_two_phase', 0)))
        return (None,) * 7 + tuple(grads.get(n) for n in ctx.names)
```

### highlyaccurate_amd/csrc/capi.hip

```cpp
#include "common.h"
#include <string.h>

static thread_local char g_err[512] = "";

void hla_set_error(const char* fmt, ...) {
  va_list ap;
  va_start(ap, fmt);
  vsnprintf(g_err, sizeof(g_err), fmt, ap);
  va_end(ap);
}

extern "C" const char* hla_last_error(void) { return g_err; }
extern "C" int hla_abi_version(void) { return HLA_ABI_VERSION; }

#ifndef HLA_SOURCE_HASH_HEX
#define HLA_SOURCE_HASH_HEX "unknown"
#endif
static const char kSourceHash[] = "HLA_SOURCE_HASH=" HLA_SOURCE_HASH_HEX;
extern "C" const char* hla_source_hash(void) { return kSourceHash + 16; }

extern "C" size_t hla_sizeof_struct(int id) {
  switch (id) {
    case HLA_STRUCT_VGG_PARAMS: return sizeof(hla_vgg_params);
    case HLA_STRUCT_VGG_GRADS: return sizeof(hla_vgg_grads);
    case HLA_STRUCT_S2G_LEVEL: return sizeof(hla_s2g_level);
    case HLA_STRUCT_S2G_CONFIG: return sizeof(hla_s2g_config);
    case HLA_STRUCT_S2G_LEVEL_GRAD: return sizeof(hla_s2g_level_grad);
    case HLA_STRUCT_PROF_RECORD: return sizeof(hla_prof_record);
    case HLA_STRUCT_POSE_LOSS_ARGS: return sizeof(hla_pose_loss_args);
    case HLA_STRUCT_FILL_REGION: return sizeof(hla_fill_region);
    case HLA_STRUCT_VGG_BRANCH: return sizeof(hla_vgg_branch);
    default: return 0;
  }
}
```

### highlyaccurate_amd/csrc/lm_host.h

```cpp
#pragma once
#include "lm_common.h"
#include <type_traits>

struct LmPlan {
  int L, N, level_first;
  int steps() const { return L * N; }
  int level(int k) const { return level_first ? k / N : k % L; }
  int iter(int k) const { return level_first ? k % N : k / L; }
  size_t slot(int k) const { return ((size_t)iter(k) * L + level(k)) * 3; }
  int trace_stride() const { return N * L * 3; }
  bool first_visit_reversed(int k) const { return iter(k) == N - 1; }
};
static inline LmPlan lm_plan_of(const hla_s2g_config* cfg) { return LmPlan{cfg->n_levels, cfg->n_iters, cfg->level_first}; }

struct LmTiling { int npix, TP, nt; };
template <class Pick>
static inline LmTiling lm_tiling(int npix, Pick pick) {
  const int tp = pick(npix);
  return LmTiling{npix, tp, (npix + tp - 1) / tp};
}
static inline int lm_npix_s2g(const hla_s2g_level& v) { return (v.h - v.row0) * v.w; }
static inline int lm_npix_g2s(const hla_s2g_level& v) { return v.A * v.A; }

template <class TilingOf>
static inline int lm_max_nt(const hla_s2g_config* cfg, const hla_s2g_level* lv, TilingOf tiling_of) {
  int m = 1;
  for (int l = 0; l < cfg->n_levels; ++l) m = max(m, tiling_of(lv[l]).nt);
  return m;
}

static inline int lm_xcd_affine(int B) { return B >= 8 ? 1 : 0; }
static inline int lm_grid_blocks(int xcd_affine, int nb, int per) { return xcd_affine ? 8 * ((nb + 7) / 8) * per : nb * per; }

struct LmBump {
  size_t o = 0;
  size_t take(size_t bytes) { const size_t at = o; o += hla_align_up(bytes, 256); return at; }
};
static inline size_t lm_one_region_bytes(size_t bytes) { LmBump ws; ws.take(bytes); return ws.o; }
static inline int lm_workspace_short(const char* who, size_t have, size_t need) {
  hla_set_error("%s: workspace %zu < %zu", who, have, need);
  return HLA_ERR_WORKSPACE;
}

static inline bool lm_newton(const hla_s2g_config* cfg) { return cfg->optimizer == 0 || cfg->optimizer == 3; }
static inline bool lm_reinit(const hla_s2g_config* cfg) { return (cfg->ford || cfg->dof == 3) && lm_newton(cfg); }
static inline LmGeom lm_geom_of(const hla_s2g_config* cfg, const hla_s2g_level& v) {
  LmGeom g{};
  g.ford = cfg->ford; g.lat = cfg->shift_range_lat; g.lon = cfg->shift_range_lon; g.rot = cfg->rotation_range;
  g.mpp = v.meter_per_pixel; g.ctr = v.centre;
  return g;
}
static inline LmSolveCfg lm_solve_cfg_of(const hla_s2g_config* cfg) {
  LmSolveCfg s{};
  s.gn = cfg->optimizer == 3 ? 1 : 0;
  s.dof = cfg->dof; s.use_hessian = s.gn ? 0 : cfg->use_hessian;
  for (int i = 0; i < 3; ++i) s.lam[i] = s.gn ? 0.0 : cfg->damping[i];
  return s;
}

template <class Args>
static inline void lm_fill_s2g_dims(Args& a, const hla_s2g_level& v, const LmTiling& t) {
  a.A = v.A; a.h = v.h; a.w = v.w; a.row0 = v.row0; a.npix = t.npix; a.TP = t.TP; a.nt = t.nt;
  a.hs = v.h - v.grd_row_skip; a.rskip = v.grd_row_skip;
}
template <class Args>
static inline void lm_fill_g2s_dims(Args& a, const hla_s2g_level& v, const LmTiling& t) {
  a.A = v.A; a.h = v.h; a.w = v.w; a.ctr = v.A / 2; a.npix = t.npix; a.nt = t.nt;
}
static inline int lm_prof_id(int C) { return C == 256 ? K_LM256 : C == 128 ? K_LM128 : C == 64 ? K_LM64 : K_LM16; }

template <int C0, int... Cs, class F>
static inline void lm_dispatch_c(int C, F&& f) {
  if (C == C0) f(std::integral_constant<int, C0>{});
  else if constexpr (sizeof...(Cs) > 0) lm_dispatch_c<Cs...>(C, f);
}
```

### highlyaccurate_amd/csrc/lm_solve.hip

```cpp
#include "lm_host.h"
#include <cstring>
#include <mutex>

struct SolveArgs {
  const double* part;
  const double* sat_inv;
  const double* grd_inv;
  int nt, part_ld;
  float* pose;
  float* trace_out;
  int trace_stride;
  const float* rand_uv;
  double* normal_eq;
  double* coef;
  const float* R_FL;
  const float* T_FL;
  int B, reinit;
  int optimizer, t;
  double beta1, beta2;
  double* adam;
  const int* in_view;
  LmSolveCfg cfg;
  LmGeom next;
  unsigned* zero_ticket;
  int zero_steps, zero_pose;
  int* reach_clear;
  const int* gate;
};

template <bool COHERENT, bool LOCAL = false>
__device__ __forceinline__ void lm_solve_body(const SolveArgs& a, int b, int lane, float* lpose = nullptr, double* lcoef = nullptr) {
  float su = LOCAL ? lpose[0] : a.pose[b * 3 + 0], sv = LOCAL ? lpose[1] : a.pose[b * 3 + 1], th = LOCAL ? lpose[2] : a.pose[b * 3 + 2];
  if (!a.part) {
    if (a.reach_clear && lane == 0) a.reach_clear[b] = 0;
    if (a.zero_ticket)
      for (int k = lane; k < a.zero_steps; k += 64) a.zero_ticket[(size_t)k * a.B + b] = 0u;
    if (a.zero_pose) {
      su = sv = th = 0.f;
      if (lane < 3) (LOCAL ? lpose[lane] : a.pose[b * 3 + lane]) = 0.f;
    }
  }

  if (a.part) {
    double s[14];
#pragma unroll
    for (int k = 0; k < 14; ++k) s[k] = 0.0;
    for (int i = lane; i < a.nt; i += 64) {
      const double* p = a.part + ((size_t)b * a.part_ld + i) * PART_N;
#pragma unroll
      for (int k = 0; k < 14; ++k)
        s[k] += COHERENT ? __hip_atomic_load(p + k, __ATOMIC_RELAXED, __HIP_MEMORY_SCOPE_AGENT) : p[k];
    }
#pragma unroll
    for (int k = 0; k < 14; ++k) s[k] = wave_sum_f64(s[k]);

    if (lane == 0) {
      const double as = a.sat_inv ? a.sat_inv[b] : 1.0, ag = a.grd_inv ? a.grd_inv[b] : 1.0;
      s[0] *= as * as; s[1] *= ag * ag;
      for (int k = 2; k < 11; ++k) s[k] *= as * as;
      for (int k = 11; k < 14; ++k) s[k] *= as * ag;
      if (a.normal_eq) {
        for (int k = 0; k < 14; ++k) a.normal_eq[(size_t)b * 16 + k] = s[k];
        a.normal_eq[(size_t)b * 16 + 14] = a.in_view ? (double)a.in_view[b] : 0.0;
        a.normal_eq[(size_t)b * 16 + 15] = 0.0;
      }
      double H[3][3], g[3], Mi[3][3], d[3], ns, ng;
      if (a.optimizer == 0 || a.optimizer == 3) {
        lm_solve_step(a.cfg, s, H, g, Mi, d, ns, ng);
      } else {
        for (int p = 0; p < 3; ++p) d[p] = 2.0 * (s[8 + p] - s[11 + p]);
        if (a.optimizer == 2) {
          double* mv = a.adam + (size_t)b * 6;
          for (int p = 0; p < 3; ++p) {
            const double m = a.beta1 * mv[p] + (1.0 - a.beta1) * d[p];
            const double v = a.beta2 * mv[3 + p] + (1.0 - a.beta2) * d[p] * d[p];
            mv[p] = m; mv[3 + p] = v;
            d[p] = (m / (1.0 - pow(a.beta1, a.t + 1))) / (sqrt(v / (1.0 - pow(a.beta2, a.t + 1))) + 1e-8);
          }
        }
        for (int p = 0; p < 3; ++p) d[p] *= 0.01;
      }
      su = (float)((double)su - d[0]);
      sv = (float)((double)sv - d[1]);
      th = (float)((double)th - d[2]);
      if (a.reinit) {
        const float ru = a.rand_uv[b], rv = a.rand_uv[a.B + b];
        su = (su > -2.5f && su < 2.5f) ? su : ru;
        sv = (sv > -2.5f && sv < 2.5f) ? sv : rv;
      }
      if (LOCAL) { lpose[0] = su; lpose[1] = sv; lpose[2] = th; }
      else { a.pose[b * 3 + 0] = su; a.pose[b * 3 + 1] = sv; a.pose[b * 3 + 2] = th; }
      float* tr = a.trace_out + (size_t)b * a.trace_stride;
      tr[0] = su; tr[1] = sv; tr[2] = th;
    }
  }
  if ((LOCAL ? lcoef : a.coef) && lane == 0)
    lm_coefficients(a.next, su, sv, th, a.R_FL ? a.R_FL + (size_t)b * 9 : nullptr, a.T_FL ? a.T_FL + (size_t)b * 3 : nullptr,
                    LOCAL ? lcoef : a.coef + (size_t)b * COEF_N);
}

__global__ __launch_bounds__(64) void lm_solve(SolveArgs a) {
  if (a.gate && a.gate[blockIdx.x] == 0) return;
  lm_solve_body<false>(a, blockIdx.x, threadIdx.x);
}

struct AccumArgs {
  const void* sat;
  const void* grd;
  const float* conf;
  LmPoints pts;
  const double* coef;
  double* part;
  int A, h, w, row0, npix, TP, nt, part_ld, xcd_affine;
  int b0, nb;
  int hs, rskip;
  const unsigned char* keep;
  unsigned* ticket;
  int col0;
  int* reach_flag;
  const int* gate;
};

typedef float lm_f2 __attribute__((ext_vector_type(2)));
__device__ __forceinline__ lm_f2 lm_fma2(float w, lm_f2 x, lm_f2 y) { return __builtin_elementwise_fma(lm_f2{w, w}, x, y); }
template <typename F> __device__ __forceinline__ lm_f2 lm_pair(const uint4& v, int ep);
template <> __device__ __forceinline__ lm_f2 lm_pair<float>(const uint4& v, int ep) {
  lm_f2 r;
  r.x = __uint_as_float(ep == 0 ? v.x : v.z);
  r.y = __uint_as_float(ep == 0 ? v.y : v.w);
  return r;
}
template <> __device__ __forceinline__ lm_f2 lm_pair<__bf16>(const uint4& v, int ep) {
  const unsigned w = ep == 0 ? v.x : ep == 1 ? v.y : ep == 2 ? v.z : v.w;
  lm_f2 r;
  r.x = __uint_as_float(w << 16);
  r.y = __uint_as_float(w & 0xffff0000u);
  return r;
}
template <> __device__ __forceinline__ lm_f2 lm_pair<_Float16>(const uint4& v, int ep) {
  typedef _Float16 h2 __attribute__((ext_vector_type(2)));
  const unsigned w = ep == 0 ? v.x : ep == 1 ? v.y : ep == 2 ? v.z : v.w;
  const h2 h = __builtin_bit_cast(h2, w);
  lm_f2 r;
  r.x = (float)h[0];
  r.y = (float)h[1];
  return r;
}

#define LM_OCC 6
#define LM_UNROLL(F) (sizeof(F) == 4 ? 2 : 1)
#define FWD_MAX_TP 512
static inline int lm_pick_tile_fwd(int npix) { return npix >= 16384 ? 512 : (npix >= 4096 ? 256 : 128); }

template <int C, bool USE_W, typename F>
__global__ __launch_bounds__(256, LM_OCC) void lm_accum(AccumArgs a, SolveArgs sa) {
  __shared__ PixParam pp[FWD_MAX_TP];
  __shared__ float red[4][14];
  __shared__ double redd[14];
  int b, tile;
  if (!lm_block_map(a.xcd_affine, a.nt, a.nb, b, tile, a.b0)) return;
  if (a.gate && a.gate[b] == 0) return;
  const int t = threadIdx.x;
  constexpr bool active = true;
#define LM_TILE_COEF (a.coef + (size_t)b * COEF_N)
#define LM_TILE_BEFORE_PUBLISH if (wave != 0) return;
#include "lm_tile_body.h"
#undef LM_TILE_COEF
#undef LM_TILE_BEFORE_PUBLISH
  const unsigned old = lm_draw_ticket(a.ticket + b, lane);
  if (old + 1 != (unsigned)a.nt) return;
  lm_solve_body<true>(sa, b, lane);
}

struct RepairLevel {
  const void* sat; const void* grd;
  LmPoints pts;
  const double* sat_inv; const double* grd_inv;
  int A, h, w, row0, npix, TP, nt, hs, rskip, C;
  double mpp, ctr;
};
struct RepairArgs {
  RepairLevel lv[4];
  SolveArgs sa;
  double* part;
  const unsigned char* keep; size_t keep_stride;
  float* trace; const float* rand_uv; double* normal_eq;
  int L, N, level_first;
};
#define LM_REPAIR_GROUPS 4

template <typename F>
__global__ __launch_bounds__(256 * LM_REPAIR_GROUPS) void lm_repair_loop(RepairArgs ra) {
  __shared__ PixParam s_pp[LM_REPAIR_GROUPS][FWD_MAX_TP];
  __shared__ float s_red[LM_REPAIR_GROUPS][4][14];
  __shared__ double s_redd[LM_REPAIR_GROUPS][14];
  __shared__ double s_cf[COEF_N];
  __shared__ float s_pose[3];
  const int b = blockIdx.x;
  if (ra.sa.gate[b] == 0) return;
  const int wt = threadIdx.x, vg = wt >> 8, vt = wt & 255;
  const int L = ra.L, N = ra.N, steps = L * N;
  auto step_level = [&](int k) { return ra.level_first ? k / N : k % L; };

  if (wt < 3) s_pose[wt] = ra.sa.pose[b * 3 + wt];
  __syncthreads();
  if (wt < 64) {
    SolveArgs sa = ra.sa;
    const RepairLevel& n = ra.lv[step_level(0)];
    sa.part = nullptr; sa.next.mpp = n.mpp; sa.next.ctr = n.ctr;
    lm_solve_body<false, true>(sa, b, wt, s_pose, s_cf);
  }
  __syncthreads();

  for (int k = 0; k < steps; ++k) {
    const int l = step_level(k), it = ra.level_first ? k % N : k / L;
    const RepairLevel& lv = ra.lv[l];
    AccumArgs a{};
    a.sat = lv.sat; a.grd = lv.grd; a.pts = lv.pts; a.part = ra.part;
    a.A = lv.A; a.h = lv.h; a.w = lv.w; a.row0 = lv.row0; a.npix = lv.npix; a.TP = lv.TP; a.nt = lv.nt; a.part_ld = ra.sa.part_ld;
    a.hs = lv.hs; a.rskip = lv.rskip;
    a.keep = ra.keep ? ra.keep + (size_t)k * ra.keep_stride : nullptr;
    for (int tile0 = 0; tile0 < lv.nt; tile0 += LM_REPAIR_GROUPS) {
      const int tile = tile0 + vg;
      const bool active = tile < lv.nt;
      constexpr bool USE_W = false;
      const int t = vt;
      PixParam* const pp = s_pp[vg];
      float (*const red)[14] = s_red[vg];
      double* const redd = s_redd[vg];
#define LM_TILE_COEF s_cf
#define LM_TILE_BEFORE_PUBLISH
      switch (lv.C) {
        case 256: {
          constexpr int C = 256;
#include "lm_tile_body.h"
        } break;
        case 128: {
          constexpr int C = 128;
#include "lm_tile_body.h"
        } break;
        default: {
          constexpr int C = 64;
#include "lm_tile_body.h"
        } break;
      }
#undef LM_TILE_COEF
#undef LM_TILE_BEFORE_PUBLISH
    }
    asm volatile("s_waitcnt vmcnt(0)" ::: "memory");
    __syncthreads();
    if (wt < 64) {
      SolveArgs sa = ra.sa;
      sa.t = k;
      sa.part = ra.part; sa.nt = lv.nt; sa.sat_inv = lv.sat_inv; sa.grd_inv = lv.grd_inv;
      sa.trace_out = ra.trace + ((size_t)it * L + l) * 3; sa.trace_stride = N * L * 3;
      sa.rand_uv = ra.sa.reinit ? ra.rand_uv + (size_t)k * 2 * ra.sa.B : nullptr;
      sa.normal_eq = ra.normal_eq ? ra.normal_eq + (size_t)k * ra.sa.B * 16 : nullptr;
      if (k + 1 < steps) {
        const RepairLevel& n = ra.lv[step_level(k + 1)];
        sa.next.mpp = n.mpp; sa.next.ctr = n.ctr;
      }
      lm_solve_body<true, true>(sa, b, wt, s_pose, k + 1 < steps ? s_cf : nullptr);
    }
    __syncthreads();
  }
  if (wt < 3) ra.sa.pose[b * 3 + wt] = s_pose[wt];
}

__global__ __launch_bounds__(256) void lm_inview_kernel(const double* __restrict__ coef, LmPoints pts, int w, int A,
                                                        int npix, int* __restrict__ count, int b0) {
  const int b = b0 + blockIdx.y, p = blockIdx.x * 256 + threadIdx.x;
  const double* cf = coef + (size_t)b * COEF_N;
  int in = 0;
  if (p < npix) {
    float q[3];
    (void)lm_point(pts, b, p / w, p % w, w, q);
    const double X = q[0], Y = q[1], Z = q[2];
    const double u = cf[0] * X + cf[1] * Y + cf[2] * Z + cf[3];
    const double v = cf[4] * X + cf[5] * Y + cf[6] * Z + cf[7];
    const double lim = (double)(A - 1);
    in = ((u >= 0.0) && (u <= lim) && (v >= 0.0) && (v <= lim)) ? 1 : 0;
  }
  const unsigned long long m = __ballot(in);
  if ((threadIdx.x & 63) == 0 && m) atomicAdd(count + b, __popcll(m));
}

static LmTiling fwd_tiling(const hla_s2g_level& v) { return lm_tiling(lm_npix_s2g(v), lm_pick_tile_fwd); }
struct FwdWs { size_t coef, pose, part, ticket, in_view, adam, total; int part_ld; };
static FwdWs fwd_ws(const hla_s2g_config* cfg, const hla_s2g_level* lv, int B) {
  FwdWs W{};
  W.part_ld = lm_max_nt(cfg, lv, fwd_tiling);
  const size_t per_step = (size_t)B * cfg->n_levels * cfg->n_iters;
  LmBump ws;
  W.coef = ws.take((size_t)B * COEF_N * sizeof(double));
  W.pose = ws.take((size_t)B * 3 * sizeof(float));
  W.part = ws.take((size_t)B * W.part_ld * PART_N * sizeof(double));
  W.ticket = ws.take(per_step * sizeof(unsigned));
  W.in_view = ws.take(per_step * sizeof(int));
  W.adam = ws.take((size_t)B * 6 * sizeof(double));
  W.total = ws.o;
  return W;
}

extern "C" size_t hla_s2g_workspace_bytes(const hla_s2g_config* cfg, const hla_s2g_level* levels, int B) {
  return fwd_ws(cfg, levels, B).total;
}

template <bool W, typename F>
static void launch_accum_f(int C, dim3 grid, hipStream_t st, const AccumArgs& a, const SolveArgs& sa) {
  lm_dispatch_c<256, 128, 64, 16>(C, [&](auto c) { hipLaunchKernelGGL((lm_accum<decltype(c)::value, W, F>), grid, dim3(256), 0, st, a, sa); });
}
template <bool W>
static void launch_accum(int C, int feat_dtype, dim3 grid, hipStream_t st, const AccumArgs& a, const SolveArgs& sa) {
  if (feat_dtype == HLA_BF16) launch_accum_f<W, __bf16>(C, grid, st, a, sa);
  else if (feat_dtype == HLA_F16) launch_accum_f<W, _Float16>(C, grid, st, a, sa);
  else launch_accum_f<W, float>(C, grid, st, a, sa);
}

int hla_s2g_validate(const char* who, const hla_s2g_config* cfg, const hla_s2g_level* lv, const float* R_FL,
                     const float* T_FL, int B) {
  HLA_REQUIRE(cfg && lv, "%s: null argument", who);
  HLA_REQUIRE(B > 0 && cfg->n_levels >= 1 && cfg->n_levels <= 4 && cfg->n_iters >= 1, "%s: bad sizes", who);
  HLA_REQUIRE(cfg->dof >= 1 && cfg->dof <= 3, "%s: dof must be 1..3", who);
  HLA_REQUIRE(cfg->proj == 0, "%s: cfg->proj selects the projection of hla_g2s_* only (must be 0 here)", who);
  HLA_REQUIRE(!cfg->ford || (R_FL && T_FL), "%s: Ford mode needs R_FL and T_FL", who);
  HLA_REQUIRE(cfg->reach_mode == 0 || (!strcmp(who, "hla_s2g_lm_solve") && cfg->reach_mode >= 1 && cfg->reach_mode <= 2 && cfg->reach_flag),
              "%s: cfg->reach_mode is 0, or 1 / 2 with reach_flag in hla_s2g_lm_solve", who);
  for (int l = 0; l < cfg->n_levels; ++l) {
    const int C = lv[l].C;
    HLA_REQUIRE(C == 256 || C == 128 || C == 64 || C == 16, "%s: unsupported channel count %d", who, C);
    HLA_REQUIRE(lv[l].feat_dtype == HLA_F32 || lv[l].feat_dtype == HLA_BF16 || lv[l].feat_dtype == HLA_F16,
                "%s: level %d feat_dtype must be HLA_F32, HLA_BF16 or HLA_F16", who, l);
    HLA_REQUIRE(lv[l].sat_feat && lv[l].grd_feat && lv[l].xyz, "%s: level %d has null maps", who, l);
    HLA_REQUIRE(!cfg->using_weight || lv[l].grd_conf, "%s: using_weight needs grd_conf", who);
    HLA_REQUIRE(lv[l].row0 >= 0 && lv[l].row0 < lv[l].h, "%s: bad row0", who);
    HLA_REQUIRE(lv[l].grd_row_skip >= 0 && lv[l].grd_row_skip <= lv[l].row0, "%s: grd_row_skip must be in [0,row0]", who);
    HLA_REQUIRE((size_t)lv[l].A * lv[l].A * C < (1u << 31), "%s: satellite map too large", who);
    HLA_REQUIRE(cfg->reach_mode != 1 || (cfg->reach_col0[l] >= 0 && cfg->reach_col0[l] < lv[l].A),
                "%s: cfg->reach_col0[%d] must be in [0, A)", who, l);
    if (lv[l].depth) {
      HLA_REQUIRE(!cfg->ford, "%s: level %d: a depth map is not supported with cfg->ford = 1 (models_ford.py has no gt_depth)", who, l);
      HLA_REQUIRE(lv[l].ray && lv[l].depth_row && lv[l].depth_col && lv[l].depth_h > 0 && lv[l].depth_w > 0,
                  "%s: level %d: depth needs ray, depth_row, depth_col and depth_h, depth_w > 0", who, l);
      HLA_REQUIRE((size_t)B * lv[l].depth_h * lv[l].depth_w < (1u << 31), "%s: level %d: depth map too large", who, l);
    } else {
      HLA_REQUIRE(!lv[l].ray && !lv[l].depth_row && !lv[l].depth_col && !lv[l].depth_h && !lv[l].depth_w,
                  "%s: level %d: ray / depth_row / depth_col / depth_h / depth_w given without depth", who, l);
    }
  }
  return HLA_OK;
}

constexpr int LM_GROUPS = 2;
constexpr int LM_SPLIT_MIN = 16;
static_assert(LM_GROUPS >= 2 && LM_GROUPS <= 4 && LM_SPLIT_MIN > 8, "a batch of up to 8 samples is one XCD octet and never splits");

struct LmSideStreams {
  std::mutex mu;
  bool ready = false, failed = false;
  hipStream_t side[LM_GROUPS] = {};
  hipEvent_t fork = nullptr, join[LM_GROUPS] = {};
};
static LmSideStreams g_lm_side[64];

static bool lm_side_create(LmSideStreams& S) {
  if (S.ready || S.failed) return S.ready;
  hipError_t r = hipEventCreateWithFlags(&S.fork, hipEventDisableTiming);
  for (int g = 1; g < LM_GROUPS && r == hipSuccess; ++g) {
    r = hipStreamCreateWithFlags(&S.side[g], hipStreamNonBlocking);
    if (r == hipSuccess) r = hipEventCreateWithFlags(&S.join[g], hipEventDisableTiming);
  }
  if (r != hipSuccess) {
    (void)hipGetLastError();
    if (S.fork) (void)hipEventDestroy(S.fork);
    for (int g = 1; g < LM_GROUPS; ++g) {
      if (S.join[g]) (void)hipEventDestroy(S.join[g]);
      if (S.side[g]) (void)hipStreamDestroy(S.side[g]);
    }
    S.failed = true;
    return false;
  }
  S.ready = true;
  return true;
}

extern "C" int hla_s2g_lm_solve(const hla_s2g_config* cfg, const hla_s2g_level* lv, const float* R_FL,
                                const float* T_FL, const float* pose0, const float* rand_uv, float* trace,
                                double* normal_eq, void* workspace, size_t workspace_bytes, int B,
                                hla_stream_t stream) {
  HLA_REQUIRE(trace && workspace, "hla_s2g_lm_solve: null argument");
  const int rc = hla_s2g_validate("hla_s2g_lm_solve", cfg, lv, R_FL, T_FL, B);
  if (rc) return rc;
  HLA_REQUIRE(cfg->optimizer >= 0 && cfg->optimizer <= 3, "hla_s2g_lm_solve: optimizer must be 0 (LM), 1 (SGD), 2 (ADAM) or 3 (GN)");
  HLA_REQUIRE(cfg->optimizer == 0 || !cfg->level_first, "hla_s2g_lm_solve: SGD / ADAM / GN exist for the iteration-first loop only");
  HLA_REQUIRE(cfg->optimizer != 3 || cfg->ford, "hla_s2g_lm_solve: GN_update exists in the Ford model only");
  const bool newton = lm_newton(cfg), reinit = lm_reinit(cfg);
  HLA_REQUIRE(!reinit || rand_uv, "hla_s2g_lm_solve: rand_uv required");
  const FwdWs W = fwd_ws(cfg, lv, B);
  if (workspace_bytes < W.total) return lm_workspace_short("hla_s2g_lm_solve", workspace_bytes, W.total);
  hipStream_t st = (hipStream_t)stream;
  char* ws = (char*)workspace;
  double* coef = (double*)(ws + W.coef);
  float* pose = (float*)(ws + W.pose);
  double* part = (double*)(ws + W.part);
  unsigned* ticket = (unsigned*)(ws + W.ticket);
  int* in_view = (int*)(ws + W.in_view);
  double* adam = (double*)(ws + W.adam);

  if (pose0) HLA_CHECK_HIP(hipMemcpyAsync(pose, pose0, (size_t)B * 3 * sizeof(float), hipMemcpyDeviceToDevice, st));

  const LmPlan plan = lm_plan_of(cfg);
  const int L = plan.L, steps = plan.steps();
  const bool count = cfg->count_in_view && normal_eq;
  if (count) HLA_CHECK_HIP(hipMemsetAsync(in_view, 0, (size_t)B * steps * sizeof(int), st));
  if (cfg->optimizer == 2) HLA_CHECK_HIP(hipMemsetAsync(adam, 0, (size_t)B * 6 * sizeof(double), st));
  SolveArgs sa{};
  sa.optimizer = cfg->optimizer; sa.beta1 = cfg->beta1; sa.beta2 = cfg->beta2; sa.adam = adam;
  sa.pose = pose; sa.B = B; sa.part_ld = W.part_ld; sa.reinit = reinit ? 1 : 0; sa.R_FL = R_FL; sa.T_FL = T_FL;
  sa.cfg = lm_solve_cfg_of(cfg);
  sa.coef = coef;

  bool repair = cfg->reach_mode == 2 && newton && !cfg->using_weight && !count && lv[0].feat_dtype != HLA_F32;
  for (int l = 0; l < L && repair; ++l) repair = lv[l].C != 16 && lv[l].feat_dtype == lv[0].feat_dtype;
  if (repair) {
    RepairArgs ra{};
    for (int l = 0; l < L; ++l) {
      const hla_s2g_level& v = lv[l];
      RepairLevel& r = ra.lv[l];
      r.sat = v.sat_feat; r.grd = v.grd_feat; r.pts = lm_points_of(v); r.sat_inv = v.sat_inv_norm; r.grd_inv = v.grd_inv_norm;
      lm_fill_s2g_dims(r, v, fwd_tiling(v));
      r.C = v.C; r.mpp = v.meter_per_pixel; r.ctr = v.centre;
    }
    ra.sa = sa;
    ra.sa.next = lm_geom_of(cfg, lv[0]);
    ra.sa.zero_pose = pose0 ? 0 : 1;
    ra.sa.gate = cfg->reach_flag;
    ra.part = part;
    ra.keep = cfg->keep; ra.keep_stride = (size_t)cfg->keep_stride;
    ra.trace = trace; ra.rand_uv = rand_uv; ra.normal_eq = normal_eq;
    ra.L = L; ra.N = plan.N; ra.level_first = plan.level_first;
    hla_prof_begin(K_LMREPAIR, 0, 0, st);
    if (lv[0].feat_dtype == HLA_BF16) hipLaunchKernelGGL(lm_repair_loop<__bf16>, dim3(B), dim3(256 * LM_REPAIR_GROUPS), 0, st, ra);
    else hipLaunchKernelGGL(lm_repair_loop<_Float16>, dim3(B), dim3(256 * LM_REPAIR_GROUPS), 0, st, ra);
    hla_prof_end(st);
    HLA_CHECK_HIP(hipGetLastError());
    return HLA_OK;
  }

  sa.part = nullptr; sa.next = lm_geom_of(cfg, lv[plan.level(0)]);
  sa.zero_ticket = ticket; sa.zero_steps = steps; sa.zero_pose = pose0 ? 0 : 1;
  sa.reach_clear = cfg->reach_mode == 1 ? cfg->reach_flag : nullptr;
  sa.gate = cfg->reach_mode == 2 ? cfg->reach_flag : nullptr;
  hipLaunchKernelGGL(lm_solve, dim3(B), dim3(64), 0, st, sa);
  sa.zero_ticket = nullptr; sa.zero_steps = 0; sa.zero_pose = 0; sa.reach_clear = nullptr;

  int ng = 1, gb0[LM_GROUPS + 1] = {0};
  LmSideStreams* side = nullptr;
  std::unique_lock<std::mutex> side_lock;
  if (B >= LM_SPLIT_MIN && !hla_prof_on() && cfg->reach_mode != 2) {
    hipStreamCaptureStatus cap = hipStreamCaptureStatusNone;
    int d = -1;
    if (hipStreamIsCapturing(st, &cap) != hipSuccess || hipGetDevice(&d) != hipSuccess) { (void)hipGetLastError(); d = -1; }
    if (cap == hipStreamCaptureStatusNone && d >= 0 && d < 64) {
      side_lock = std::unique_lock<std::mutex>(g_lm_side[d].mu);
      if (lm_side_create(g_lm_side[d])) side = &g_lm_side[d];
      else side_lock.unlock();
    }
  }
  if (side) {
    const int oct = (B + 7) / 8;
    ng = oct < LM_GROUPS ? oct : LM_GROUPS;
    for (int g = 0; g < ng; ++g) gb0[g + 1] = gb0[g] + 8 * (oct / ng + (g < oct % ng ? 1 : 0));
  }
  gb0[ng] = B;
  hipStream_t gst[LM_GROUPS];
  gst[0] = st;
  int forked = 0;
  hipError_t err = hipSuccess;
  if (ng > 1) {
    err = hipEventRecord(side->fork, st);
    for (int g = 1; g < ng && err == hipSuccess; ++g) {
      gst[g] = side->side[g];
      err = hipStreamWaitEvent(gst[g], side->fork, 0);
      if (err == hipSuccess) forked = g;
    }
  }

  for (int k = 0; k < steps && err == hipSuccess; ++k) {
    const int l = plan.level(k);
    const hla_s2g_level& v = lv[l];
    AccumArgs aa{};
    aa.sat = v.sat_feat; aa.grd = v.grd_feat; aa.conf = v.grd_conf; aa.pts = lm_points_of(v); aa.coef = coef; aa.part = part;
    lm_fill_s2g_dims(aa, v, fwd_tiling(v));
    aa.keep = cfg->keep ? cfg->keep + (size_t)k * cfg->keep_stride : nullptr;
    aa.part_ld = W.part_ld; aa.xcd_affine = lm_xcd_affine(B);
    aa.ticket = ticket + (size_t)k * B;
    if (cfg->reach_mode == 1) { aa.col0 = cfg->reach_col0[l]; aa.reach_flag = cfg->reach_flag; }
    aa.gate = sa.gate;
    sa.t = k;
    sa.part = part; sa.nt = aa.nt; sa.sat_inv = v.sat_inv_norm; sa.grd_inv = v.grd_inv_norm;
    sa.trace_out = trace + plan.slot(k); sa.trace_stride = plan.trace_stride();
    sa.rand_uv = reinit ? rand_uv + (size_t)k * 2 * B : nullptr;
    sa.normal_eq = normal_eq ? normal_eq + (size_t)k * B * 16 : nullptr;
    sa.in_view = count ? in_view + (size_t)k * B : nullptr;
    if (k + 1 < steps) { sa.coef = coef; sa.next = lm_geom_of(cfg, lv[plan.level(k + 1)]); }
    else sa.coef = nullptr;
    const double esz = v.feat_dtype == HLA_F32 ? 4.0 : 2.0;
    for (int g = 0; g < ng; ++g) {
      hipStream_t gs = gst[g];
      aa.b0 = gb0[g]; aa.nb = gb0[g + 1] - gb0[g];
      if (count)
        hipLaunchKernelGGL(lm_inview_kernel, dim3((v.h * v.w + 255) / 256, aa.nb), dim3(256), 0, gs, coef, aa.pts, v.w, v.A, v.h * v.w,
                           in_view + (size_t)k * B, aa.b0);
      const int nblk = lm_grid_blocks(aa.xcd_affine, aa.nb, aa.nt);
      hla_prof_begin(lm_prof_id(v.C), 0, (double)aa.nb * ((double)v.A * v.A + (double)aa.npix) * v.C * esz, gs);
      if (cfg->using_weight && newton) launch_accum<true>(v.C, v.feat_dtype, dim3(nblk), gs, aa, sa);
      else launch_accum<false>(v.C, v.feat_dtype, dim3(nblk), gs, aa, sa);
      hla_prof_end(gs);
    }
  }
  for (int g = 1; g <= forked; ++g) {
    hipError_t e = hipEventRecord(side->join[g], gst[g]);
    if (e == hipSuccess) e = hipStreamWaitEvent(st, side->join[g], 0);
    if (err == hipSuccess) err = e;
  }
  HLA_CHECK_HIP(err);
  HLA_CHECK_HIP(hipGetLastError());
  return HLA_OK;
}
```

### highlyaccurate_amd/csrc/vgg.hip

```cpp
#include "conv_kernels.h"
#include "vgg_layers.h"
#include <type_traits>

template <typename T>
void vgg_pack_all(const hla_vgg_params* prm, char* packed, int dtype, hipStream_t st) {
  constexpr bool SPLIT = Prec<T>::SPLIT;
  std::conditional_t<SPLIT, SplitPackTable, PackTable> tb{};
  if constexpr (!SPLIT) tb.b0 = prm->b[0];
  int n = 0;
  for (int l = 0; l < kAllLayers; ++l) {
    if (l >= kPackedLayers && !prm->w[l]) continue;
    tb.w[n] = prm->w[l]; tb.off[n] = packed_offset(l, dtype); tb.cout[n] = kLayers[l].cout; tb.cin[n] = kLayers[l].cin;
    tb.first[n] = l == 0 ? 1 : 0;
    if constexpr (SPLIT) tb.slot[n] = l;
    else tb.shape[n] = l >= 2 ? conv_shape<T, false>(conv_class(kLayers[l].cout, vgg_layer_pools(l))) : SHAPE_32x32x16;
    ++n;
  }
  if constexpr (!SPLIT) {
    hla_prof_begin(K_PACK, 0, (double)packed_offset(kAllLayers, dtype) * (1.0 + 4.0 / sizeof(T)), st);
    hipLaunchKernelGGL((pack_weights_multi_kernel<T>), dim3(256, n), dim3(256), 0, st, tb, packed);
  } else {
    float* tail = (float*)(packed + packed_offset(kAllLayers, dtype));
    unsigned* scratch = (unsigned*)tail + 32;
    (void)hipMemsetAsync(tail, 0, kPackTailBytes, st);
    hla_prof_begin(K_PACK, 0, (double)packed_offset(kAllLayers, dtype) * 3.0, st);
    hipLaunchKernelGGL(absmax_multi_kernel, dim3(64, n), dim3(256), 0, st, tb, scratch, (unsigned*)tail + 16);
    hipLaunchKernelGGL(pack_weights_split_multi_kernel, dim3(256, n), dim3(256), 0, st, tb, packed, (const unsigned*)scratch, tail);
  }
  hla_prof_end(st);
}

struct VggFwdCall {
  const float* x; size_t x_plane; const hla_vgg_params* prm; const char* packed;
  void* const* feat; float* const* conf; double* inv_norm; char* ws; size_t ws_bytes;
  int B, H, W, level, dtype, flags, first_row8, first_col32;
  const int* col_gate;
  hipStream_t st;
  VggPlan pl;
};

struct VggConvSet {
  Conv02Args c02;
  ConvArgs conv[kAllLayers];
  bool used[kAllLayers], pool[kAllLayers];
  int np_used[4];
};
template <typename T>
static void vgg_build_convs(const VggFwdCall& c, bool want_conf, VggConvSet& S) {
  const VggPlan& pl = c.pl;
  const int B = c.B, H = c.H, W = c.W, flags = c.flags;
  const bool level4 = c.level == 4, fold = (flags & HLA_VGG_FOLD_DECODER) != 0, train = (flags & HLA_VGG_SAVE_FOR_BACKWARD) != 0;
  const bool fixup = c.col_gate != nullptr;
  auto W_ = [&](int l) { return (const uint4*)(c.packed + packed_offset(l, c.dtype)); };
  char* w = c.ws;
  auto act = [&](int m) { return m >= 0 ? w + pl.act[m] : (char*)nullptr; };
  constexpr bool SPLIT = Prec<T>::SPLIT;
  const float* wtail = (const float*)(c.packed + packed_offset(kAllLayers, c.dtype));
  unsigned* amax = (unsigned*)(w + pl.amax);
  auto AM = [&](int slot) { return (SPLIT && slot >= 0) ? amax + (size_t)slot * B : (unsigned*)nullptr; };
  const VggFwdRows rows = vgg_fwd_rows(c.first_row8, level4, train, want_conf);
  S = VggConvSet{};
  for (int l = 0; l < 4; ++l) S.np_used[l] = pl.np[l];
  {
    Conv02Args& a = S.c02;
    a.x_plane = c.x_plane ? c.x_plane : (size_t)H * W;
    a.x = c.x; a.w0 = W_(0); a.b0 = c.prm->b[0]; a.w2 = W_(1); a.b2 = c.prm->b[1];
    a.out_act = act(AM_X3);
    if (train) {
      a.a0_out = act(AM_A0);
      a.idx_out = (unsigned char*)(w + pl.idx[IDX_3]);
    }
    if (level4) a.a2_out = act(AM_X2);
    a.wtail = wtail; a.amax_out = AM(AM_X3); a.amax_a2_out = level4 ? AM(AM_X2) : nullptr;
    a.amax_a0_out = train ? AM(AM_A0) : nullptr;
    a.row_begin = rows.row[1];
    const VggCols cc = vgg_cols(1, c.first_col32, fixup);
    a.col_begin = cc.begin;
    a.gate = c.col_gate;
    const int txf = (W + 31) / 32;
    a.B = B; a.H = H; a.W = W; a.tiles_y = (H - a.row_begin + 7) / 8;
    a.tiles_x = cc.tiles ? (cc.tiles < txf ? cc.tiles : txf) : txf - a.col_begin;
  }
  const bool x21r_dead = !level4 && !want_conf && !train && (flags & HLA_VGG_FEAT16) && sizeof(T) == 2;
  for (int l = 2; l < (level4 ? kAllLayers : kPackedLayers); ++l) {
    const VggFwdLaunch& f = kFwd[l];
    const VggHW g = vgg_layer_hw(l, H, W, fold);
    ConvArgs& a = S.conv[l];
    S.used[l] = true; S.pool[l] = vgg_layer_pools(l);
    void* raw = f.level >= 0 ? c.feat[f.level] : nullptr;
    a.raw16 = (raw && (flags & HLA_VGG_FEAT16)) ? 1 : 0;
    a.row_begin = rows.row[l];
    const VggCols cc = vgg_cols(l, c.first_col32, fixup);
    a.col_begin = cc.begin; a.col_tiles = cc.tiles;
    a.gate = c.col_gate;
    a.idx_out = (train && f.idx >= 0) ? (unsigned char*)(w + pl.idx[f.idx]) : nullptr;
    a.src1 = act(f.src); a.src2 = act(f.skip);
    a.C1 = kActMaps[f.src].C; a.C2 = f.skip >= 0 ? kActMaps[f.skip].C : 0; a.up1 = f.skip >= 0 ? 1 : 0; a.wpk = W_(l);
    a.bias = kLayers[l].has_bias ? c.prm->b[l] : nullptr;
    a.out_act = (f.out == AM_X21 && x21r_dead) ? (char*)nullptr : act(f.out); a.out_raw = (float*)raw;
    a.sumsq = f.level >= 0 ? (double*)(w + pl.ss[f.level]) : nullptr;
    a.B = B; a.H = g.h; a.W = g.w; a.Cout = kLayers[l].cout;
    a.relu_act = 1;
    if (SPLIT) {
      a.amax1 = AM(f.src); a.amax2 = AM(f.skip); a.amax_out = AM(f.out); a.wscale = wtail + l;
    }
    if (f.level >= 0) S.np_used[f.level] = vgg_level_partials(l, H, W, fold, a.row_begin);
  }
}

template <typename T>
static int launch_conv02(hipStream_t st, Conv02Args a, const Conv02Args* a1) {
  constexpr int lds_bytes = conv02_lds_bytes<T>();
#if HLA_CONV_STAMPS
  a.stamps = nullptr;
  if (!a1 && g_hla_stamp.buf && g_hla_stamp.want <= -10 && g_hla_stamp.want++ == -10) {
    a.stamps = g_hla_stamp.buf; g_hla_stamp.want = -1000;
    g_hla_stamp.grid_x = a.tiles_x * a.tiles_y * a.B; g_hla_stamp.grid_y = 1;
  }
#endif
  auto P = [](const Conv02Args& c) {
    const int x1 = (c.col_begin + c.tiles_x) * 32;
    return (double)c.B * (c.H - c.row_begin) * ((x1 < c.W ? x1 : c.W) - c.col_begin * 32);
  };
  const double Pt = P(a) + (a1 ? P(*a1) : 0.0);
  static HlaPerDeviceOnce attr_once[2];
  HLA_CHECK_HIP(attr_once[a1 ? 1 : 0].run([a1] {
    const void* fn = a1 ? (const void*)conv02_pair_kernel<T, 2> : (const void*)conv02_kernel<T, 2>;
    return hipFuncSetAttribute(fn, hipFuncAttributeMaxDynamicSharedMemorySize, lds_bytes);
  }));
  hla_prof_begin(K_CONV02, 2.0 * 9 * (3 + 64) * 64 * Pt, Pt * (3 * 4 + 16 * sizeof(T)), st);
  if (a1) {
    PairArgs<Conv02Args> pa{{a, *a1}, a.tiles_x * a.tiles_y * a.B};
#if HLA_CONV_STAMPS
    pa.s[1].stamps = nullptr;
#endif
    hipLaunchKernelGGL((conv02_pair_kernel<T, 2>), dim3(pa.n0 + a1->tiles_x * a1->tiles_y * a1->B), dim3(256), lds_bytes, st, pa);
  } else
    hipLaunchKernelGGL((conv02_kernel<T, 2>), dim3(a.tiles_x * a.tiles_y * a.B), dim3(256), lds_bytes, st, a);
  hla_prof_end(st);
  return HLA_OK;
}

static int vgg_norms(int nb, const VggFwdCall* const* net, const VggConvSet* S, int NL) {
  const VggFwdCall& c0 = *net[0];
  const int B = c0.B;
  hipStream_t st = c0.st;
  InvNormArgs ia{};
  ia.gate = c0.col_gate;
  double bytes = 0;
  for (int k = 0; k < nb; ++k)
    for (int l = 0; l < NL; ++l) {
      const VggFwdCall& n = *net[k];
      ia.ss[k * NL + l] = (const double*)(n.ws + n.pl.ss[l]); ia.np[k * NL + l] = S[k].np_used[l];
      ia.inv[k * NL + l] = (n.inv_norm ? n.inv_norm : (double*)(n.ws + n.pl.inv)) + (size_t)l * B;
      bytes += (double)B * n.pl.np[l] * 8;
    }
  hla_prof_begin(K_L2NORM, 0, bytes, st);
  hipLaunchKernelGGL(inv_norm_multi_kernel, dim3(B, nb * NL), dim3(256), 0, st, ia);
  hla_prof_end(st);
  for (int k = 0; k < nb; ++k)
    for (int l = 0; l < NL; ++l) {
      if (c0.flags & HLA_VGG_DEFER_NORM) continue;
      const size_t per = vgg_map_elems(kActMaps[kLevelMap[l]], net[k]->H, net[k]->W);
      int bps = (int)(per / 4 / 256 / 4);
      bps = bps < 1 ? 1 : (bps > 64 ? 64 : bps);
      hla_prof_begin(K_L2NORM, 0, (double)B * per * 8, st);
      hipLaunchKernelGGL(scale_kernel, dim3(B * bps), dim3(256), 0, st, (float*)net[k]->feat[l], ia.inv[k * NL + l], per, bps);
      hla_prof_end(st);
    }
  return HLA_OK;
}

template <typename T>
int vgg_forward_t(const VggFwdCall& c) {
  const VggPlan& pl = c.pl;
  const int NL = c.level == 4 ? 4 : 3, B = c.B;
  hipStream_t st = c.st;
  constexpr bool SPLIT = Prec<T>::SPLIT;
  if (SPLIT) HLA_CHECK_HIP(hipMemsetAsync(c.ws + pl.amax, 0, (size_t)kAmaxSlots * B * sizeof(unsigned), st));
  const bool want_conf = (c.flags & HLA_VGG_WANT_CONF) && c.conf;
  VggConvSet S;
  vgg_build_convs<T>(c, want_conf, S);
  if (const int rc = launch_conv02<T>(st, S.c02, nullptr)) return rc;
  bool launch_ok = true;
  for (int l = 2; l < kAllLayers; ++l)
    if (S.used[l] && !launch_conv<T>(st, S.conv[l], S.pool[l])) launch_ok = false;
  if (want_conf) {
    using CT = std::conditional_t<SPLIT, float, T>;
    for (int l = 0; l < NL; ++l) {
      if (!c.conf[l]) continue;
      const VggMapDef& m = kActMaps[kLevelMap[l]];
      const VggHW g = vgg_map_hw(m, c.H, c.W, (c.flags & HLA_VGG_FOLD_DECODER) != 0);
      const CT* act = (const CT*)(c.ws + pl.act[kLevelMap[l]]);
      const size_t npix = (size_t)B * g.h * g.w;
      const int grid = B * ((g.h + CONF_TH - 1) / CONF_TH) * ((g.w + CONF_TW - 1) / CONF_TW);
      hla_prof_begin(K_CONF, 2.0 * 9 * m.C * (double)npix, (double)npix * (m.C * sizeof(CT) + 4), st);
      if (m.C == 256) hipLaunchKernelGGL((conf_kernel<CT, 256>), dim3(grid), dim3(256), 0, st, act, c.prm->w[13 + l], c.conf[l], B, g.h, g.w);
      else if (m.C == 128) hipLaunchKernelGGL((conf_kernel<CT, 128>), dim3(grid), dim3(256), 0, st, act, c.prm->w[13 + l], c.conf[l], B, g.h, g.w);
      else hipLaunchKernelGGL((conf_kernel<CT, 64>), dim3(grid), dim3(256), 0, st, act, c.prm->w[13 + l], c.conf[l], B, g.h, g.w);
      hla_prof_end(st);
    }
  }
  const VggFwdCall* net = &c;
  if (const int rc = vgg_norms(1, &net, &S, NL)) return rc;
  HLA_CHECK_HIP(hipGetLastError());
  return launch_ok ? HLA_OK : HLA_ERR_ARG;
}

template <typename T>
int vgg_fixup_t(const VggFwdCall& c) {
  static_assert(sizeof(T) == 2, "vgg_fixup_loop: bf16 / fp16");
  VggConvSet S;
  vgg_build_convs<T>(c, false, S);
  VggFixupArgs fa{};
  fa.c02 = S.c02;
  for (int k = 0; k < kFixupConvs; ++k) {
    const int l = k + 2;
    ConvArgs a = S.conv[l];
    const bool ok = S.used[l] && (a.Cout >= 128 || !S.pool[l]) && !a.idx_out;
    HLA_REQUIRE(ok, "vgg_fixup: layer %d is not one of the level-3 inference launches", l);
    if (conv_plan<T, false>(a, S.pool[l]).small) a.tiles_y = (a.H - a.row_begin + 7) / 8;
    fa.conv[k] = a;
    if (S.pool[l]) fa.pooled |= 1 << k;
  }
  for (int l = kFixupConvs + 2; l < kAllLayers; ++l) HLA_REQUIRE(!S.used[l], "vgg_fixup: level 3 only");
  for (int l = 0; l < 3; ++l) {
    fa.ss[l] = (const double*)(c.ws + c.pl.ss[l]); fa.np[l] = S.np_used[l];
    fa.inv[l] = (c.inv_norm ? c.inv_norm : (double*)(c.ws + c.pl.inv)) + (size_t)l * c.B;
  }
  fa.gate = c.col_gate;
  constexpr int lds_bytes = vgg_fixup_lds_bytes<T>();
  static HlaPerDeviceOnce attr_once;
  HLA_CHECK_HIP(attr_once.run([] {
    return hipFuncSetAttribute((const void*)vgg_fixup_loop<T>, hipFuncAttributeMaxDynamicSharedMemorySize, lds_bytes);
  }));
  hipLaunchKernelGGL((vgg_fixup_loop<T>), dim3(c.B), dim3(256), lds_bytes, c.st, fa);
  HLA_CHECK_HIP(hipGetLastError());
  return HLA_OK;
}

constexpr int HLA_PAIR_FALLBACK = -1000;
template <typename T>
int vgg_forward_pair_t(const VggFwdCall c[2]) {
  constexpr bool SPLIT = Prec<T>::SPLIT;
  hipStream_t st = c[0].st;
  VggConvSet S[2];
  for (int k = 0; k < 2; ++k) vgg_build_convs<T>(c[k], false, S[k]);
  for (int l = 2; l < kAllLayers; ++l) {
    if (S[0].used[l] != S[1].used[l]) return HLA_PAIR_FALLBACK;
    if (!S[0].used[l]) continue;
    ConvArgs a0 = S[0].conv[l], a1 = S[1].conv[l];
    if (conv_plan<T, false>(a0, S[0].pool[l]).small != conv_plan<T, false>(a1, S[1].pool[l]).small) return HLA_PAIR_FALLBACK;
  }
  if (SPLIT)
    for (int k = 0; k < 2; ++k)
      HLA_CHECK_HIP(hipMemsetAsync(c[k].ws + c[k].pl.amax, 0, (size_t)kAmaxSlots * c[k].B * sizeof(unsigned), st));
  if (const int rc = launch_conv02<T>(st, S[0].c02, &S[1].c02)) return rc;
  bool launch_ok = true;
  for (int l = 2; l < kAllLayers; ++l)
    if (S[0].used[l] && !launch_conv_pair<T>(st, S[0].conv[l], S[1].conv[l], S[0].pool[l])) launch_ok = false;
  const VggFwdCall* nets[2] = {&c[0], &c[1]};
  if (const int rc = vgg_norms(2, nets, S, 3)) return rc;
  HLA_CHECK_HIP(hipGetLastError());
  return launch_ok ? HLA_OK : HLA_ERR_ARG;
}

struct HlaConvLayerSeg {
  const void* src;
  const float* w;
  void* wpk;
  void* out;
  float* raw;
  double* sumsq;
  int H, W;
};
struct HlaConvLayerCall { int B, Cin, Cout, pool, nseg; HlaConvLayerSeg seg[2]; hipStream_t st; };
template <typename T>
int vgg_conv_layer_t(const HlaConvLayerCall& c) {
  ConvArgs a[2] = {};
  for (int k = 0; k < c.nseg; ++k) {
    const HlaConvLayerSeg& s = c.seg[k];
    PackTable tb{};
    tb.w[0] = s.w; tb.off[0] = 0; tb.cout[0] = c.Cout; tb.cin[0] = c.Cin; tb.first[0] = 0;
    tb.shape[0] = conv_shape<T, false>(conv_class(c.Cout, c.pool != 0));
    hipLaunchKernelGGL((pack_weights_multi_kernel<T>), dim3(64, 1), dim3(256), 0, c.st, tb, (char*)s.wpk);
    a[k].src1 = s.src; a[k].wpk = (const uint4*)s.wpk; a[k].out_act = s.out; a[k].out_raw = s.raw; a[k].sumsq = s.raw ? s.sumsq : nullptr;
    a[k].C1 = c.Cin; a[k].B = c.B; a[k].H = s.H; a[k].W = s.W; a[k].Cout = c.Cout; a[k].relu_act = 1;
  }
  const bool ok = c.nseg == 2 ? launch_conv_pair<T>(c.st, a[0], a[1], c.pool != 0) : launch_conv<T>(c.st, a[0], c.pool != 0);
  HLA_CHECK_HIP(hipGetLastError());
  return ok ? HLA_OK : HLA_ERR_ARG;
}

#if HLA_TU_DTYPE >= 0
#if HLA_TU_DTYPE == 1 || HLA_TU_DTYPE == 2
template int vgg_conv_layer_t<TuT>(const HlaConvLayerCall& c);
#endif
template void vgg_pack_all<TuT>(const hla_vgg_params* prm, char* packed, int dtype, hipStream_t st);
template int vgg_forward_t<TuT>(const VggFwdCall& c);
template int vgg_forward_pair_t<TuT>(const VggFwdCall c[2]);
#if HLA_TU_DTYPE == 1 || HLA_TU_DTYPE == 2
template int vgg_fixup_t<TuT>(const VggFwdCall& c);
#endif
#else
#define HLA_EXTERN_T(T) \
  extern template void vgg_pack_all<T>(const hla_vgg_params* prm, char* packed, int dtype, hipStream_t st); \
  extern template int vgg_forward_t<T>(const VggFwdCall& c); \
  extern template int vgg_forward_pair_t<T>(const VggFwdCall c[2]);
HLA_EXTERN_T(float) HLA_EXTERN_T(bf16) HLA_EXTERN_T(f16) HLA_EXTERN_T(split32)
extern template int vgg_fixup_t<bf16>(const VggFwdCall& c);
extern template int vgg_fixup_t<f16>(const VggFwdCall& c);
extern template int vgg_conv_layer_t<bf16>(const HlaConvLayerCall& c);
extern template int vgg_conv_layer_t<f16>(const HlaConvLayerCall& c);

extern "C" int hla_debug_conv_layer(int dtype, int B, int Cin, int Cout, int pool, const void* seg, int nseg, hla_stream_t stream) {
  HLA_REQUIRE(seg && (nseg == 1 || nseg == 2), "hla_debug_conv_layer: one or two segments");
  HLA_REQUIRE(dtype == HLA_BF16 || dtype == HLA_F16, "hla_debug_conv_layer: bf16 / fp16 only");
  HLA_REQUIRE(B > 0 && Cin >= 32 && Cin % 32 == 0 && (Cout == 64 || (Cout >= 128 && Cout % 128 == 0)),
              "hla_debug_conv_layer: Cin a multiple of 32, Cout 64 or a multiple of 128 (got %d, %d)", Cin, Cout);
  HlaConvLayerCall c{B, Cin, Cout, pool, nseg, {}, (hipStream_t)stream};
  for (int k = 0; k < nseg; ++k) {
    c.seg[k] = ((const HlaConvLayerSeg*)seg)[k];
    const HlaConvLayerSeg& s = c.seg[k];
    HLA_REQUIRE(s.src && s.w && s.wpk && s.out && s.H > 0 && s.W > 0 && (!pool || (s.H % 2 == 0 && s.W % 2 == 0)) && (!s.raw || s.sumsq),
                "hla_debug_conv_layer: segment %d: null argument, odd size under the pool, or raw without sumsq", k);
  }
  return dtype == HLA_BF16 ? vgg_conv_layer_t<bf16>(c) : vgg_conv_layer_t<f16>(c);
}

extern "C" size_t hla_vgg_packed_weight_bytes(int dtype) {
  return packed_offset(kAllLayers, dtype) + (dtype == HLA_F16X3 ? kPackTailBytes : 0);
}

extern "C" int hla_vgg_pack_weights(const hla_vgg_params* params, void* packed, int dtype, hla_stream_t stream) {
  HLA_REQUIRE(params && packed, "hla_vgg_pack_weights: null argument");
  HLA_REQUIRE(hla_dtype_ok(dtype), "hla_vgg_pack_weights: bad dtype %d", dtype);
  HLA_REQUIRE(params->w[0] && params->b[0], "hla_vgg_pack_weights: conv0's weight and bias are required (the bias is packed with it)");
  hla_dispatch_dtype(dtype, [&](auto t) { vgg_pack_all<typename decltype(t)::type>(params, (char*)packed, dtype, (hipStream_t)stream); });
  HLA_CHECK_HIP(hipGetLastError());
  return HLA_OK;
}

extern "C" size_t hla_vgg_workspace_bytes(int B, int H, int W, int level, int dtype) {
  VggPlan p;
  vgg_plan(B, H, W, dtype, true, &p, level == 4);
  return p.total;
}

extern "C" size_t hla_vgg_workspace_bytes_flags(int B, int H, int W, int level, int dtype, int flags) {
  VggPlan p;
  vgg_plan(B, H, W, dtype, true, &p, level == 4, (flags & HLA_VGG_FOLD_DECODER) != 0);
  return p.total;
}

static inline int vgg_first_col32(int first_col32, int level, int dtype, int flags) {
  const bool ok = level == 3 && dtype != HLA_F16X3 && (flags & HLA_VGG_DEFER_NORM) &&
                  !(flags & (HLA_VGG_SAVE_FOR_BACKWARD | HLA_VGG_FOLD_DECODER | HLA_VGG_WANT_CONF));
  return ok ? first_col32 : 0;
}

static int vgg_forward_check(VggFwdCall& c, bool silent) {
#define VGG_REQUIRE(cond, ...) \
  do { if (!(cond)) { if (!silent) hla_set_error(__VA_ARGS__); return HLA_ERR_ARG; } } while (0)
  const int H = c.H, W = c.W, level = c.level, dtype = c.dtype, flags = c.flags, first_row8 = c.first_row8, first_col32 = c.first_col32;
  VGG_REQUIRE(c.x && c.prm && c.packed && c.feat && c.ws, "hla_vgg_forward: null argument");
  VGG_REQUIRE(hla_dtype_ok(dtype), "hla_vgg_forward: dtype must be HLA_F32, HLA_BF16, HLA_F16 or HLA_F16X3 (got %d)", dtype);
  VGG_REQUIRE(c.B > 0 && H >= 8 && W >= 8 && H % 8 == 0 && W % 8 == 0, "hla_vgg_forward: H and W must be multiples of 8");
  VGG_REQUIRE(c.x_plane == 0 || c.x_plane >= (size_t)H * W, "hla_vgg_forward: x_plane (%zu) must be 0 or >= H*W", c.x_plane);
  VGG_REQUIRE((size_t)H * W * 64 * 4 < ((size_t)1 << 31), "hla_vgg_forward: image too large (H*W must be below 2^23 pixels)");
  VGG_REQUIRE(level == 3 || level == 4, "hla_vgg_forward: level must be 3 (x15,x18,x21) or 4 (+x24), got %d", level);
  VGG_REQUIRE(c.feat[0] && c.feat[1] && c.feat[2], "hla_vgg_forward: feat[0..2] are required");
  VGG_REQUIRE(level == 3 || (c.feat[3] && c.prm->w[11] && c.prm->w[12]),
              "hla_vgg_forward: level 4 needs feat[3] ([B,H,W,64], 16 real channels) and the zero-padded conv_dec3 weights in w[11], w[12]");
  VGG_REQUIRE(level == 3 || !(flags & HLA_VGG_WANT_CONF) || !c.conf || !c.conf[3] || c.prm->w[16], "hla_vgg_forward: conf[3] needs w[16]");
  VGG_REQUIRE(!(flags & HLA_VGG_DEFER_NORM) || c.inv_norm, "hla_vgg_forward: HLA_VGG_DEFER_NORM needs inv_norm");
  VGG_REQUIRE(!(flags & HLA_VGG_FEAT16) || ((dtype == HLA_BF16 || dtype == HLA_F16) && (flags & HLA_VGG_DEFER_NORM) &&
                                            !(flags & HLA_VGG_SAVE_FOR_BACKWARD) && level == 3),
              "hla_vgg_forward: HLA_VGG_FEAT16 needs dtype HLA_BF16 / HLA_F16, HLA_VGG_DEFER_NORM, level 3 and no HLA_VGG_SAVE_FOR_BACKWARD");
  VGG_REQUIRE(first_row8 == 0 || (first_row8 >= 4 && first_row8 < H / 8), "hla_vgg_forward: first_row8 must be 0 or in [4, H/8)");
  VGG_REQUIRE(!(flags & HLA_VGG_FOLD_DECODER) || (W % 16 == 0 && first_row8 == 0 && !(flags & HLA_VGG_FEAT16)),
              "hla_vgg_forward: HLA_VGG_FOLD_DECODER needs W %% 16 == 0 (folded maps are W/16, W/8, W/4 wide), first_row8 == 0 and no "
              "HLA_VGG_FEAT16 (got W = %d, first_row8 = %d)", W, first_row8);
  VGG_REQUIRE(first_col32 >= 0 && (first_col32 == 0 || 128 * first_col32 < W),
              "hla_vgg_forward_cols: first_col32 must be 0 or leave a column of the map (128 * first_col32 < W; got %d, W = %d)", first_col32, W);
  VGG_REQUIRE(!c.col_gate || first_col32 > 0, "hla_vgg_forward_cols: col_gate is the fix-up pass of a forward made with first_col32 > 0");
#undef VGG_REQUIRE
  c.first_col32 = vgg_first_col32(first_col32, level, dtype, flags);
  if (c.col_gate && !c.first_col32) return HLA_OK;
  vgg_plan(c.B, H, W, dtype, (flags & HLA_VGG_SAVE_FOR_BACKWARD) != 0, &c.pl, level == 4, (flags & HLA_VGG_FOLD_DECODER) != 0);
  if (c.ws_bytes < c.pl.total) {
    if (!silent) hla_set_error("hla_vgg_forward: workspace %zu < %zu", c.ws_bytes, c.pl.total);
    return HLA_ERR_WORKSPACE;
  }
  return HLA_OK;
}

static int vgg_forward_cols_impl(VggFwdCall c, bool fixup_one_launch) {
  if (const int rc = vgg_forward_check(c, false)) return rc;
  if (c.col_gate && !c.first_col32) return HLA_OK;
  const bool one_launch = c.col_gate && fixup_one_launch && !hla_prof_on();
  return hla_dispatch_dtype(c.dtype, [&](auto t) {
    using T = typename decltype(t)::type;
    if constexpr (std::is_same_v<T, bf16> || std::is_same_v<T, f16>)
      if (one_launch) return vgg_fixup_t<T>(c);
    return vgg_forward_t<T>(c);
  });
}

extern "C" int hla_vgg_forward(const float* x, size_t x_plane, const hla_vgg_params* params, const void* packed_weights,
                               void* const feat[4], float* const conf[4], double* inv_norm, void* workspace,
                               size_t workspace_bytes, int B, int H, int W, int level, int dtype, int flags,
                               int first_row8, hla_stream_t stream) {
  return hla_vgg_forward_cols(x, x_plane, params, packed_weights, feat, conf, inv_norm, workspace, workspace_bytes, B, H, W, level, dtype,
                              flags, first_row8, 0, nullptr, stream);
}

extern "C" int hla_vgg_forward_cols(const float* x, size_t x_plane, const hla_vgg_params* params, const void* packed_weights,
                                    void* const feat[4], float* const conf[4], double* inv_norm, void* workspace,
                                    size_t workspace_bytes, int B, int H, int W, int level, int dtype, int flags,
                                    int first_row8, int first_col32, const int* col_gate, hla_stream_t stream) {
  return vgg_forward_cols_impl(VggFwdCall{x, x_plane, params, (const char*)packed_weights, feat, conf, inv_norm, (char*)workspace,
                                          workspace_bytes, B, H, W, level, dtype, flags, first_row8, first_col32, col_gate,
                                          (hipStream_t)stream, {}}, true);
}

extern "C" int hla_vgg_fixup(const float* x, size_t x_plane, const hla_vgg_params* params, const void* packed_weights,
                             void* const feat[4], double* inv_norm, void* workspace, size_t workspace_bytes, int B, int H, int W,
                             int level, int dtype, int flags, int first_row8, int first_col32, const int* col_gate, int one_launch,
                             hla_stream_t stream) {
  HLA_REQUIRE(col_gate, "hla_vgg_fixup: col_gate is required");
  return vgg_forward_cols_impl(VggFwdCall{x, x_plane, params, (const char*)packed_weights, feat, nullptr, inv_norm, (char*)workspace,
                                          workspace_bytes, B, H, W, level, dtype, flags, first_row8, first_col32, col_gate,
                                          (hipStream_t)stream, {}}, one_launch != 0);
}

extern "C" int hla_vgg_forward_pair(const hla_vgg_branch br[2], int B, int level, int dtype, int flags, int* paired_out, hla_stream_t stream) {
  HLA_REQUIRE(br, "hla_vgg_forward_pair: null argument");
  if (paired_out) *paired_out = 0;
  auto plain = [&]() -> int {
    for (int k = 0; k < 2; ++k)
      if (const int rc = hla_vgg_forward_cols(br[k].x, br[k].x_plane, br[k].params, br[k].packed_weights, br[k].feat, br[k].conf, br[k].inv_norm,
                                         br[k].workspace, br[k].workspace_bytes, B, br[k].H, br[k].W, level, dtype, flags, br[k].first_row8,
                                         br[k].first_col32, nullptr, stream))
        return rc;
    return HLA_OK;
  };
  if (level != 3 || (flags & (HLA_VGG_SAVE_FOR_BACKWARD | HLA_VGG_FOLD_DECODER | HLA_VGG_WANT_CONF)) || !hla_dtype_ok(dtype)) return plain();
  VggFwdCall c[2];
  for (int k = 0; k < 2; ++k) {
    const hla_vgg_branch& b = br[k];
    c[k] = VggFwdCall{b.x, b.x_plane, b.params, (const char*)b.packed_weights, b.feat, nullptr, b.inv_norm, (char*)b.workspace,
                      b.workspace_bytes, B, b.H, b.W, level, dtype, flags, b.first_row8, b.first_col32, nullptr, (hipStream_t)stream, {}};
    if (vgg_forward_check(c[k], true) != HLA_OK) return plain();
  }
  const int rc = hla_dispatch_dtype(dtype, [&](auto t) { return vgg_forward_pair_t<typename decltype(t)::type>(c); });
  if (rc == HLA_PAIR_FALLBACK) return plain();
  if (rc == HLA_OK && paired_out) *paired_out = 1;
  return rc;
}
#endif
```

### include/hla.h

```cpp
#ifndef HLA_H
#define HLA_H

#include <stddef.h>
#include <stdint.h>

#ifdef __cplusplus
extern "C" {
#endif

typedef void* hla_stream_t;

typedef enum hla_status {
  HLA_OK = 0,
  HLA_ERR_ARG = -1,
  HLA_ERR_HIP = -2,
  HLA_ERR_WORKSPACE = -3
} hla_status;

typedef enum hla_dtype {
  HLA_F32 = 0,
  HLA_BF16 = 1,
  HLA_F16 = 2,
  HLA_F16X3 = 3
} hla_dtype;

const char* hla_last_error(void);

#define HLA_ABI_VERSION 32
int hla_abi_version(void);
const char* hla_source_hash(void);
typedef enum hla_struct_id {
  HLA_STRUCT_VGG_PARAMS = 0, HLA_STRUCT_VGG_GRADS = 1, HLA_STRUCT_S2G_LEVEL = 2, HLA_STRUCT_S2G_CONFIG = 3,
  HLA_STRUCT_S2G_LEVEL_GRAD = 4, HLA_STRUCT_PROF_RECORD = 5, HLA_STRUCT_POSE_LOSS_ARGS = 6, HLA_STRUCT_FILL_REGION = 7,
  HLA_STRUCT_VGG_BRANCH = 8
} hla_struct_id;
size_t hla_sizeof_struct(int id);


typedef struct hla_vgg_params {
  const float* w[17];
  const float* b[7];
} hla_vgg_params;

enum {
  HLA_VGG_WANT_CONF = 1,
  HLA_VGG_DEFER_NORM = 2,
  HLA_VGG_SAVE_FOR_BACKWARD = 4,
  HLA_VGG_FOLD_DECODER = 16,
  HLA_VGG_FEAT16 = 8
};

size_t hla_vgg_packed_weight_bytes(int dtype);
int hla_vgg_pack_weights(const hla_vgg_params* params, void* packed, int dtype, hla_stream_t stream);

size_t hla_vgg_workspace_bytes(int B, int H, int W, int level, int dtype);
size_t hla_vgg_workspace_bytes_flags(int B, int H, int W, int level, int dtype, int flags);

int hla_vgg_forward(const float* x, size_t x_plane, const hla_vgg_params* params, const void* packed_weights, void* const feat[4],
                    float* const conf[4], double* inv_norm, void* workspace, size_t workspace_bytes, int B, int H,
                    int W, int level, int dtype, int flags, int first_row8, hla_stream_t stream);

int hla_vgg_forward_cols(const float* x, size_t x_plane, const hla_vgg_params* params, const void* packed_weights,
                         void* const feat[4], float* const conf[4], double* inv_norm, void* workspace, size_t workspace_bytes,
                         int B, int H, int W, int level, int dtype, int flags, int first_row8, int first_col32,
                         const int* col_gate, hla_stream_t stream);

int hla_vgg_fixup(const float* x, size_t x_plane, const hla_vgg_params* params, const void* packed_weights, void* const feat[4],
                  double* inv_norm, void* workspace, size_t workspace_bytes, int B, int H, int W, int level, int dtype, int flags,
                  int first_row8, int first_col32, const int* col_gate, int one_launch, hla_stream_t stream);

typedef struct hla_vgg_branch {
  const float* x;
  size_t x_plane;
  const hla_vgg_params* params;
  const void* packed_weights;
  void* feat[4];
  float* conf[4];
  double* inv_norm;
  void* workspace;
  size_t workspace_bytes;
  int H, W, first_row8;
  int first_col32;
} hla_vgg_branch;

int hla_vgg_forward_pair(const hla_vgg_branch br[2], int B, int level, int dtype, int flags, int* paired_out, hla_stream_t stream);

typedef struct hla_vgg_grads {
  float* dw[17];
  float* db[7];
} hla_vgg_grads;

size_t hla_vgg_packed_weight_T_bytes(int dtype);
int hla_vgg_pack_weights_T(const hla_vgg_params* params, void* packed_T, int dtype, hla_stream_t stream);
size_t hla_vgg_bwd_workspace_bytes(int B, int H, int W, int level, int dtype);
size_t hla_vgg_bwd_workspace_bytes_flags(int B, int H, int W, int level, int dtype, int flags);

#define HLA_VGG_BWD_SCALE_INVARIANT 1
#define HLA_VGG_BWD_DENSE 2
#define HLA_VGG_BWD_WGRAD_TWO_PHASE 4
#define HLA_VGG_BWD_FOLD_DECODER 16
#define HLA_VGG_BWD_WGRAD0_UNFUSED 8
int hla_vgg_backward(const float* x, size_t x_plane, const hla_vgg_params* params, const void* packed_weights_T,
                     const void* fwd_workspace, const float* const feat[4], const double* inv_norm,
                     const float* const d_feat[4], const float* const conf[4], const float* const d_conf[4],
                     const hla_vgg_grads* grads, void* workspace, size_t workspace_bytes, int B, int H, int W, int level,
                     int dtype, int flags, int first_row8, hla_stream_t stream);

int hla_vgg_backward_live_tiles(const void* workspace, int B, int H, int W, int level, int dtype, long long* live,
                                long long* total);

int hla_sat_tile(const unsigned char* src, const double* stages, float* out, int B, int S, int crop, hla_stream_t stream);

int hla_resize_bilinear(const unsigned char* src, const int* hbounds, const int* htaps, int hksize, const int* vbounds,
                        const int* vtaps, int vksize, unsigned char* mid, float* out, int B, int H, int W, int out_h,
                        int out_w, hla_stream_t stream);

int hla_grid_sample(const float* image, const float* optical, const float* jac, float* out, float* jac_out,
                    int N, int C, int IH, int IW, int H, int W, int M, hla_stream_t stream);

int hla_grid_sample_bwd(const float* image, const float* optical, const float* jac, const float* d_out,
                        const float* d_jac_out, float* d_image, float* d_optical, float* d_jac,
                        int N, int C, int IH, int IW, int H, int W, int M, hla_stream_t stream);

typedef struct hla_s2g_level {
  const void* sat_feat;
  const void* grd_feat;
  const float* grd_conf;
  const float* xyz;
  const double* sat_inv_norm;
  const double* grd_inv_norm;
  int A, h, w, C;
  int row0;
  int grd_row_skip;
  double meter_per_pixel;
  double centre;
  int feat_dtype;
  const float* ray;
  const float* depth;
  const int* depth_row;
  const int* depth_col;
  int depth_h, depth_w;
} hla_s2g_level;

typedef struct hla_s2g_config {
  int ford;
  int n_levels, n_iters;
  int level_first;
  int using_weight;
  int use_hessian;
  int dof;
  double shift_range_lat, shift_range_lon, rotation_range;
  double damping[3];
  const unsigned char* keep;
  size_t keep_stride;
  int optimizer;
  double beta1, beta2;
  int count_in_view;
  int grd_grad_overwrite;
  int deterministic;
  int proj;
  int reach_mode;
  int* reach_flag;
  int reach_col0[4];
} hla_s2g_config;

size_t hla_s2g_workspace_bytes(const hla_s2g_config* cfg, const hla_s2g_level* levels, int B);

int hla_s2g_lm_solve(const hla_s2g_config* cfg, const hla_s2g_level* levels, const float* R_FL,
                     const float* T_FL, const float* pose0, const float* rand_uv, float* trace,
                     double* normal_eq, void* workspace, size_t workspace_bytes, int B, hla_stream_t stream);

size_t hla_s2g_pose_score_workspace_bytes(const hla_s2g_config* cfg, const hla_s2g_level* level, int B, int K);
int hla_s2g_pose_score(const hla_s2g_config* cfg, const hla_s2g_level* level, const float* R_FL, const float* T_FL,
                       const float* poses, int K, double* sums, float* cost, void* workspace, size_t workspace_bytes, int B,
                       hla_stream_t stream);

size_t hla_g2s_workspace_bytes(const hla_s2g_config* cfg, const hla_s2g_level* levels, int B);
int hla_g2s_lm_solve(const hla_s2g_config* cfg, const hla_s2g_level* levels, const float* camera_k, int ori_h, int ori_w,
                     const float* pose0, float* trace, double* normal_eq, void* workspace, size_t workspace_bytes,
                     int B, hla_stream_t stream);

size_t hla_g2s_pose_score_workspace_bytes(const hla_s2g_config* cfg, const hla_s2g_level* level, int B, int K);
int hla_g2s_pose_score(const hla_s2g_config* cfg, const hla_s2g_level* level, const float* camera_k, int ori_h, int ori_w,
                       const float* poses, int K, double* sums, float* cost, void* workspace, size_t workspace_bytes, int B,
                       hla_stream_t stream);

typedef struct hla_s2g_level_grad {
  float* d_sat_feat;
  float* d_grd_feat;
  float* d_grd_conf;
} hla_s2g_level_grad;

size_t hla_s2g_bwd_workspace_bytes(const hla_s2g_config* cfg, const hla_s2g_level* levels, int B);

int hla_s2g_lm_solve_bwd(const hla_s2g_config* cfg, const hla_s2g_level* levels, const hla_s2g_level_grad* grads,
                         const float* R_FL, const float* T_FL, const float* pose0, const float* trace,
                         const double* normal_eq, const float* d_trace, double* d_damping, void* workspace,
                         size_t workspace_bytes, int B, hla_stream_t stream);

size_t hla_s2g_pose_score_bwd_workspace_bytes(const hla_s2g_config* cfg, const hla_s2g_level* level, int B, int K);
int hla_s2g_pose_score_bwd(const hla_s2g_config* cfg, const hla_s2g_level* level, const hla_s2g_level_grad* grad,
                           const float* R_FL, const float* T_FL, const float* poses, int K, const double* sums,
                           const float* d_cost, void* workspace, size_t workspace_bytes, int B, hla_stream_t stream);

size_t hla_g2s_pose_score_bwd_workspace_bytes(const hla_s2g_config* cfg, const hla_s2g_level* level, int B, int K);
int hla_g2s_pose_score_bwd(const hla_s2g_config* cfg, const hla_s2g_level* level, const hla_s2g_level_grad* grad,
                           const float* camera_k, int ori_h, int ori_w, const float* poses, int K, const double* sums,
                           const float* d_cost, void* workspace, size_t workspace_bytes, int B, hla_stream_t stream);

size_t hla_g2s_bwd_workspace_bytes(const hla_s2g_config* cfg, const hla_s2g_level* levels, int B);
int hla_g2s_lm_solve_bwd(const hla_s2g_config* cfg, const hla_s2g_level* levels, const hla_s2g_level_grad* grads,
                         const float* camera_k, int ori_h, int ori_w, const float* pose0, const float* trace,
                         const double* normal_eq, const float* d_trace, double* d_damping, void* workspace,
                         size_t workspace_bytes, int B, hla_stream_t stream);


typedef struct hla_fill_region {
  void* ptr;
  size_t chunk_bytes, stride_bytes;
  int n_chunks;
} hla_fill_region;
int hla_zero_fill(const hla_fill_region* regions, int n_regions, int max_blocks, hla_stream_t stream);

enum { HLA_POSE_LOSS_F32 = 0, HLA_POSE_LOSS_F64 = 1 };
typedef struct hla_pose_loss_args {
  const float* x[3];
  long long x_stride[3][3];
  const void* gt[3];
  long long gt_stride[3];
  double coe[3];
  int B, N, L;
  int gt_dtype;
} hla_pose_loss_args;
int hla_pose_loss(const hla_pose_loss_args* args, void* out, hla_stream_t stream);
int hla_pose_loss_bwd(const hla_pose_loss_args* args, const void* const g_out[9], float* const dx[3],
                      const long long dx_stride[3][3], hla_stream_t stream);

size_t hla_orien_corr_workspace_bytes(int B, int H, int W, int C, int S);
int hla_orien_corr(const float* P1, const float* grd_feat, const double* p1_inv_norm, const double* grd_inv_norm, double* dot,
                   double* E, double* gnorm, float* corr, void* workspace, size_t workspace_bytes, int B, int H, int W, int C,
                   int S, hla_stream_t stream);
int hla_orien_corr_bwd(const float* P1, const float* grd_feat, const double* p1_inv_norm, const double* grd_inv_norm,
                       const double* dot, const double* E, const double* gnorm, const float* d_corr, float* d_P1,
                       float* d_grd_feat, void* workspace, size_t workspace_bytes, int B, int H, int W, int C, int S,
                       hla_stream_t stream);
int hla_orien_window_bwd(const float* optical, const float* d_out, double* acc, float* d_image, int N, int C, int IH, int IW,
                         int H, int W, hla_stream_t stream);
int hla_orien_triplet_loss(const float* corr, const float* gt_heading, long long gt_stride, double rotation_range,
                           double degree_per_pixel, float* loss, int accumulate, int B, int S, hla_stream_t stream);
int hla_orien_triplet_loss_bwd(const float* corr, const float* gt_heading, long long gt_stride, double rotation_range,
                               double degree_per_pixel, const float* g_loss, float* d_corr, int B, int S, hla_stream_t stream);

size_t hla_g2s_corr_workspace_bytes(int B, int A, int Hc, int Wc, int C);
int hla_g2s_corr(const float* sat, const float* g2s, const double* sat_inv_norm, const double* g2s_inv_norm, double* dot, double* E,
                 double* gnorm, float* corr, void* workspace, size_t workspace_bytes, int B, int A, int Hc, int Wc, int C,
                 hla_stream_t stream);
int hla_g2s_corr_bwd(const float* sat, const float* g2s, const double* sat_inv_norm, const double* g2s_inv_norm, const double* dot,
                     const double* E, const double* gnorm, const float* d_corr, float* d_sat, float* d_g2s, void* workspace,
                     size_t workspace_bytes, int B, int A, int Hc, int Wc, int C, hla_stream_t stream);
int hla_g2s_corr_triplet_loss(const float* corr, const float* gt_shift_u, long long gt_u_stride, const float* gt_shift_v,
                              long long gt_v_stride, double shift_range_lat, double shift_range_lon, double meters_per_pixel,
                              float* loss, int accumulate, int B, int Ny, int Nx, hla_stream_t stream);
int hla_g2s_corr_triplet_loss_bwd(const float* corr, const float* gt_shift_u, long long gt_u_stride, const float* gt_shift_v,
                                  long long gt_v_stride, double shift_range_lat, double shift_range_lon, double meters_per_pixel,
                                  const float* g_loss, float* d_corr, int B, int Ny, int Nx, hla_stream_t stream);

#define HLA_PROF_NKERNELS 20
typedef struct hla_prof_record {
  int kernel_id;
  float ms;
  double flops;
  double bytes;
} hla_prof_record;
int hla_prof_enable(int on);
const char* hla_prof_kernel_name(int kernel_id);
int hla_prof_fetch(hla_prof_record* out, int max_records, int* n_out);
int hla_prof_mfma_peak(int dtype, int data, float ms_target, float* tflops_out, hla_stream_t stream);

#ifdef __cplusplus
}
#endif
#endif
```

Measured before the change: 6164 pairs/s.

## Overlap LM solve of first sample group with decoder of remaining samples

Splits the VGG decoder layers and the deferred norms into two sample ranges. An event is recorded once the first group's features are ready, so the LM solver for that group can start on a side stream while the decoder still runs on the rest of the batch. Random draws are moved ahead of the feature pass so the solver needs no host work between the two. This adds cross-stream event plumbing, workspace lifetime holding and an ABI bump, and it splits decoder launches into smaller per-range convs.

```diff
diff --git a/highlyaccurate_amd/VGG.py b/highlyaccurate_amd/VGG.py
--- a/highlyaccurate_amd/VGG.py
+++ b/highlyaccurate_amd/VGG.py
@@ -167,7 +167,8 @@
 
 
 @_lib.on_device(lambda modules, xs, *a, **k: xs[0])
-def vgg_forward_pair_nhwc(modules, xs, first_row8=(0, 0), feat16: bool = False, first_col32=(0, 0), col_state: dict = None):
+def vgg_forward_pair_nhwc(modules, xs, first_row8=(0, 0), feat16: bool = False, first_col32=(0, 0), col_state: dict = None,
+                          split=None, hold: list = None, info: dict = None):
     lib = _lib.load()
     if len(modules) != 2 or len(xs) != 2:
         raise ValueError('vgg_forward_pair_nhwc takes two modules and two images')
@@ -206,7 +207,17 @@
                              first_row8=int(first_row8[k]), first_col32=b.first_col32)
     flags = _lib.HLA_VGG_DEFER_NORM | (_lib.HLA_VGG_FEAT16 if feat16 else 0)
     paired = C.c_int(0)
-    rc = lib.hla_vgg_forward_pair(br, xs[0].shape[0], 3, dt, flags, C.byref(paired), _lib.stream_ptr())
+    if split is None:
+        rc = lib.hla_vgg_forward_pair(br, xs[0].shape[0], 3, dt, flags, C.byref(paired), _lib.stream_ptr())
+    else:
+        if hold is None:
+            raise ValueError('vgg_forward_pair_nhwc: split needs hold (the workspaces outlive the call)')
+        hold += keep
+        sp = _lib.VggSplit(int(split[0]), split[1].cuda_event)
+        did = C.c_int(0)
+        rc = lib.hla_vgg_forward_pair_split(br, xs[0].shape[0], 3, dt, flags, C.byref(sp), C.byref(paired), C.byref(did), _lib.stream_ptr())
+        if info is not None:
+            info['split'] = bool(did.value)
     _lib.check(rc, 'hla_vgg_forward_pair')
     return out[0], out[1], bool(paired.value)
 
diff --git a/highlyaccurate_amd/_lib.py b/highlyaccurate_amd/_lib.py
--- a/highlyaccurate_amd/_lib.py
+++ b/highlyaccurate_amd/_lib.py
@@ -16,7 +16,7 @@
 HLA_VGG_BWD_WGRAD_TWO_PHASE = 4
 HLA_VGG_BWD_WGRAD0_UNFUSED = 8
 HLA_VGG_BWD_FOLD_DECODER = 16
-ABI_VERSION = 32
+ABI_VERSION = 33
 
 
 class HlaError(RuntimeError):
@@ -43,7 +43,8 @@
                 ('damping', C.c_double * 3), ('keep', C.c_void_p), ('keep_stride', C.c_size_t),
                 ('optimizer', C.c_int), ('beta1', C.c_double), ('beta2', C.c_double), ('count_in_view', C.c_int),
                 ('grd_grad_overwrite', C.c_int), ('deterministic', C.c_int), ('proj', C.c_int),
-                ('reach_mode', C.c_int), ('reach_flag', C.c_void_p), ('reach_col0', C.c_int * 4)]
+                ('reach_mode', C.c_int), ('reach_flag', C.c_void_p), ('reach_col0', C.c_int * 4),
+                ('group0_ready', C.c_void_p), ('group0_samples', C.c_int)]
 
 
 class VggBranch(C.Structure):
@@ -51,6 +52,10 @@
                 ('feat', C.c_void_p * 4), ('conf', C.c_void_p * 4), ('inv_norm', C.c_void_p), ('workspace', C.c_void_p),
                 ('workspace_bytes', C.c_size_t), ('H', C.c_int), ('W', C.c_int), ('first_row8', C.c_int),
                 ('first_col32', C.c_int)]
+
+
+class VggSplit(C.Structure):
+    _fields_ = [('split_b', C.c_int), ('ready', C.c_void_p)]
 
 
 class FillRegion(C.Structure):
@@ -92,7 +97,7 @@
         raise HlaError(f'{path}: no hla_sizeof_struct export; rebuild it') from None
     fn.restype, fn.argtypes = C.c_size_t, [C.c_int]
     for sid, cls in enumerate((VggParams, VggGrads, S2GLevel, S2GConfig, S2GLevelGrad, ProfRecord, PoseLossArgs, FillRegion,
-                                VggBranch)):
+                                VggBranch, VggSplit)):
         if fn(sid) != C.sizeof(cls):
             raise HlaError(f'{path}: sizeof({cls.__name__}) is {fn(sid)} in the library and {C.sizeof(cls)} in the binding')
 
@@ -134,6 +139,10 @@
     lib.hla_vgg_fixup.argtypes = [vp, sz, C.POINTER(VggParams), vp, C.POINTER(vp), vp, vp, sz, i, i, i, i, i, i, i, i, vp, i, vp]
     lib.hla_vgg_forward_pair.restype = i
     lib.hla_vgg_forward_pair.argtypes = [C.POINTER(VggBranch), i, i, i, i, C.POINTER(i), vp]
+    lib.hla_vgg_forward_pair_split.restype = i
+    lib.hla_vgg_forward_pair_split.argtypes = [C.POINTER(VggBranch), i, i, i, i, C.POINTER(VggSplit), C.POINTER(i), C.POINTER(i), vp]
+    lib.hla_s2g_split_b.restype = i
+    lib.hla_s2g_split_b.argtypes = [i]
     lib.hla_vgg_packed_weight_bytes.restype = sz
     lib.hla_vgg_packed_weight_bytes.argtypes = [i]
     lib.hla_vgg_pack_weights.restype = i
diff --git a/highlyaccurate_amd/_s2gp.py b/highlyaccurate_amd/_s2gp.py
--- a/highlyaccurate_amd/_s2gp.py
+++ b/highlyaccurate_amd/_s2gp.py
@@ -213,12 +213,14 @@
         self._reach = {}
         self._ray_tables = {}
         self._depth_idx = {}
+        self._ready_events = {}
         self.last_trace = None
         self.last_normal_eq = None
         self.last_keep = None
         self.keep_normal_eq = False
         self.keep_features = False
         self.last_features = None
+        self.last_under_decoder = False
         self.last_reach_flag = None
         self.last_search = None
         self.last_score_loss = None
@@ -304,6 +306,26 @@
 
     def _draw_reinit(self, n_steps: int, B: int, device):
         return draw_reinit(n_steps, B, device)
+
+    def _ready_event(self, device):
+        key = torch.device(device).index
+        ev = self._ready_events.get(key)
+        if ev is None:
+            ev = torch.cuda.Event(enable_timing=False)
+            ev.record()
+            self._ready_events[key] = ev
+        return ev
+
+    def _predraw(self, B: int, grd_hw, level_first, init_pose, device) -> dict:
+        from types import SimpleNamespace
+        tables = self.xyz_tables(grd_hw[0], grd_hw[1], device)[:3]
+        cfg = self._config(3, level_first)
+        reinit = (self.ford or cfg.dof == 3) and cfg.optimizer in (0, 3)
+        rand_uv = self._draw_reinit(3 * self.N_iters, B, device) if reinit else None
+        lv = [SimpleNamespace(h=t.shape[0], w=t.shape[1], row0=0 if self.polar else t.shape[0] // 2) for t in tables]
+        keep = self._draw_dropout(lv, level_first, device)
+        p0 = init_pose.to(device).float().contiguous() if init_pose is not None else None
+        return dict(rand_uv=rand_uv, keep=keep, p0=p0)
 
     def _draw_dropout(self, lv, level_first, device):
         if not getattr(self.args, 'dropout', 0) or getattr(self.args, 'Optimizer', 'LM') != 'LM':
@@ -357,7 +379,7 @@
 
     @_lib.on_device(lambda self, sat_feats, *a, **k: sat_feats[0])
     def lm_solve(self, sat_feats, grd_feats, grd_confs, grd_hw, extra=None, level_first=0, init_pose=None,
-                 sat_inv_norm=None, grd_inv_norm=None, keep_normal_eq=None, gt_depth=None, reach=None):
+                 sat_inv_norm=None, grd_inv_norm=None, keep_normal_eq=None, gt_depth=None, reach=None, pre=None):
         lib = _lib.load()
         dev = sat_feats[0].device
         B, L = sat_feats[0].shape[0], len(sat_feats)
@@ -366,8 +388,11 @@
                                                sat_inv_norm, grd_inv_norm, depth)
         steps = L * self.N_iters
         reinit = (self.ford or cfg.dof == 3) and cfg.optimizer in (0, 3)
-        rand_uv = self._draw_reinit(steps, B, dev) if reinit else None
-        self.last_keep = self._draw_dropout(lv, level_first, dev)
+        if pre is None:
+            rand_uv = self._draw_reinit(steps, B, dev) if reinit else None
+            self.last_keep = self._draw_dropout(lv, level_first, dev)
+        else:
+            rand_uv, self.last_keep = pre['rand_uv'], pre['keep']
         if self.last_keep is not None:
             cfg.keep, cfg.keep_stride = self.last_keep.data_ptr(), self.last_keep.shape[1]
         trace = torch.empty(B, self.N_iters, L, 3, device=dev, dtype=torch.float32)
@@ -377,7 +402,9 @@
         neq = torch.empty(steps, B, 16, device=dev, dtype=torch.float64) if want_neq else None
         nbytes = lib.hla_s2g_workspace_bytes(C.byref(cfg), lv, B)
         ws = torch.empty(nbytes, dtype=torch.uint8, device=dev)
-        p0 = init_pose.to(dev).float().contiguous() if init_pose is not None else None
+        p0 = pre['p0'] if pre is not None else (init_pose.to(dev).float().contiguous() if init_pose is not None else None)
+        if pre is not None and pre.get('ready') is not None:
+            cfg.group0_ready, cfg.group0_samples = pre['ready'][0].cuda_event, int(pre['ready'][1])
         flag = None
         if reach is not None:
             flag = torch.empty(B, dtype=torch.int32, device=dev)
@@ -389,7 +416,7 @@
         _lib.check(rc, 'hla_s2g_lm_solve')
         if reach is not None:
             reach[1](flag)
-            cfg.reach_mode = 2
+            cfg.reach_mode, cfg.group0_ready, cfg.group0_samples = 2, None, 0
             rc = lib.hla_s2g_lm_solve(C.byref(cfg), lv, _lib.ptr(R_FL), _lib.ptr(T_FL), _lib.ptr(p0), _lib.ptr(rand_uv),
                                       _lib.ptr(trace), _lib.ptr(neq), _lib.ptr(ws), nbytes, B, _lib.stream_ptr())
             _lib.check(rc, 'hla_s2g_lm_solve (reach fallback)')
@@ -528,7 +555,20 @@
             solve = lambda p0: self.lm_solve(sat_feats, grd_feats, grd_confs, hw, extra, level_first, p0, sat_inv, grd_inv)
             return _pose.search(self, cand, M, score, solve, score_level, len(sat_feats) - 1, min_in_view)
 
-    def _features(self, sat_map, grd_img, want_conf, return_confs, sat_c32=0, col_state=None):
+    def _pairs_launches(self, B: int, want_conf) -> bool:
+        small = B <= int(getattr(self.args, 'small_batch_two_streams', 4))
+        return (not small and not want_conf and self.level != 4 and bool(getattr(self.args, 'pair_extractor_launches', 1))
+                and self.GrdFeatureNet.precision == self.SatFeatureNet.precision)
+
+    def _under_decoder(self, B: int, want_conf, return_confs, gt_depth) -> int:
+        a = self.args
+        ok = (bool(getattr(a, 'lm_under_decoder', 1)) and not return_confs and not want_conf and gt_depth is None and not self.ford
+              and self.level == 3 and getattr(a, 'Optimizer', 'LM') == 'LM' and not getattr(a, 'strict_errors', 0)
+              and self.SatFeatureNet.precision in ('bf16', 'fp16') and bool(getattr(a, 'lm_feat16', 1))
+              and self._pairs_launches(B, want_conf) and B >= 16)
+        return _lib.load().hla_s2g_split_b(B) if ok else 0
+
+    def _features(self, sat_map, grd_img, want_conf, return_confs, sat_c32=0, col_state=None, split=None, hold=None, info=None):
         f16 = (self.SatFeatureNet.precision in ('bf16', 'fp16') and self.level == 3 and bool(getattr(self.args, 'lm_feat16', 1)))
         small = sat_map.shape[0] <= int(getattr(self.args, 'small_batch_two_streams', 4))
         dead_ok = (not return_confs and self.level == 3 and getattr(self.args, 'Optimizer', 'LM') == 'LM'
@@ -537,11 +577,10 @@
         grd_in = grd_img[:, :, skip:, :] if skip else grd_img
         f8 = ((grd_img.shape[-2] // 8) // 2 - skip // 8) if dead_ok else 0
         f8 = f8 if f8 >= 4 else 0
-        if (not small and not want_conf and self.level != 4 and bool(getattr(self.args, 'pair_extractor_launches', 1))
-                and self.GrdFeatureNet.precision == self.SatFeatureNet.precision):
+        if self._pairs_launches(sat_map.shape[0], want_conf):
             (sat_feats, sat_inv), (grd_feats, grd_inv), _ = vgg_forward_pair_nhwc(
                 (self.SatFeatureNet, self.GrdFeatureNet), (sat_map, grd_in), first_row8=(0, f8), feat16=f16,
-                first_col32=(sat_c32, 0), col_state=col_state)
+                first_col32=(sat_c32, 0), col_state=col_state, split=split, hold=hold, info=info)
             L = self._levels
             return L(sat_feats), L(sat_inv), L(grd_feats), L([None] * 3), L(grd_inv)
         if small:
@@ -584,10 +623,19 @@
                 and not getattr(a, 'strict_errors', 0) and self.SatFeatureNet.precision != 'fp16x3'):
             c32 = self.sat_first_col32(sat_map.shape[-1], grd_img.shape[-2], grd_img.shape[-1])
         state = {} if c32 else None
-        sat_feats, sat_inv, grd_feats, grd_confs, grd_inv = self._features(sat_map, grd_img, want_conf, return_confs, c32, state)
+        split_b = self._under_decoder(sat_map.shape[0], want_conf, return_confs, gt_depth)
+        pre, split, hold, info = None, None, None, {}
+        if split_b:
+            pre = self._predraw(sat_map.shape[0], grd_img.shape[-2:], level_first, init_pose, sat_map.device)
+            pre['ready'] = (self._ready_event(sat_map.device), split_b)
+            split, hold = (split_b, pre['ready'][0]), []
+        sat_feats, sat_inv, grd_feats, grd_confs, grd_inv = self._features(sat_map, grd_img, want_conf, return_confs, c32, state,
+                                                                           split, hold, info)
+        self.last_under_decoder = bool(info.get('split'))
         reach = (promised_cols(c32), lambda flag: vgg_fixup_nhwc(state, flag, bool(getattr(a, 'fixup_one_launch', 1)))) if c32 else None
         trace = self.lm_solve(sat_feats, grd_feats, grd_confs, grd_img.shape[-2:], extra, level_first, init_pose,
-                              sat_inv, grd_inv, gt_depth=gt_depth, reach=reach)
+                              sat_inv, grd_inv, gt_depth=gt_depth, reach=reach, pre=pre)
+        del hold
         if self.keep_features:
             self.last_features = (sat_feats, sat_inv, grd_feats, grd_inv)
         return trace, grd_confs
diff --git a/highlyaccurate_amd/csrc/capi.hip b/highlyaccurate_amd/csrc/capi.hip
--- a/highlyaccurate_amd/csrc/capi.hip
+++ b/highlyaccurate_amd/csrc/capi.hip
@@ -30,6 +30,7 @@
     case HLA_STRUCT_POSE_LOSS_ARGS: return sizeof(hla_pose_loss_args);
     case HLA_STRUCT_FILL_REGION: return sizeof(hla_fill_region);
     case HLA_STRUCT_VGG_BRANCH: return sizeof(hla_vgg_branch);
+    case HLA_STRUCT_VGG_SPLIT: return sizeof(hla_vgg_split);
     default: return 0;
   }
 }
diff --git a/highlyaccurate_amd/csrc/lm_host.h b/highlyaccurate_amd/csrc/lm_host.h
--- a/highlyaccurate_amd/csrc/lm_host.h
+++ b/highlyaccurate_amd/csrc/lm_host.h
@@ -1,5 +1,6 @@
 #pragma once
 #include "lm_common.h"
+#include "split_plan.h"
 #include <type_traits>
 
 struct LmPlan {
diff --git a/highlyaccurate_amd/csrc/lm_solve.hip b/highlyaccurate_amd/csrc/lm_solve.hip
--- a/highlyaccurate_amd/csrc/lm_solve.hip
+++ b/highlyaccurate_amd/csrc/lm_solve.hip
@@ -99,9 +99,10 @@
                     LOCAL ? lcoef : a.coef + (size_t)b * COEF_N);
 }
 
-__global__ __launch_bounds__(64) void lm_solve(SolveArgs a) {
-  if (a.gate && a.gate[blockIdx.x] == 0) return;
-  lm_solve_body<false>(a, blockIdx.x, threadIdx.x);
+__global__ __launch_bounds__(64) void lm_solve(SolveArgs a, int b0) {
+  const int b = b0 + blockIdx.x;
+  if (a.gate && a.gate[b] == 0) return;
+  lm_solve_body<false>(a, b, threadIdx.x);
 }
 
 struct AccumArgs {
@@ -305,6 +306,7 @@
 extern "C" size_t hla_s2g_workspace_bytes(const hla_s2g_config* cfg, const hla_s2g_level* levels, int B) {
   return fwd_ws(cfg, levels, B).total;
 }
+extern "C" int hla_s2g_split_b(int B) { return lm_split_b(B); }
 
 template <bool W, typename F>
 static void launch_accum_f(int C, dim3 grid, hipStream_t st, const AccumArgs& a, const SolveArgs& sa) {
@@ -351,10 +353,6 @@
   return HLA_OK;
 }
 
-constexpr int LM_GROUPS = 2;
-constexpr int LM_SPLIT_MIN = 16;
-static_assert(LM_GROUPS >= 2 && LM_GROUPS <= 4 && LM_SPLIT_MIN > 8, "a batch of up to 8 samples is one XCD octet and never splits");
-
 struct LmSideStreams {
   std::mutex mu;
   bool ready = false, failed = false;
@@ -407,11 +405,45 @@
   int* in_view = (int*)(ws + W.in_view);
   double* adam = (double*)(ws + W.adam);
 
-  if (pose0) HLA_CHECK_HIP(hipMemcpyAsync(pose, pose0, (size_t)B * 3 * sizeof(float), hipMemcpyDeviceToDevice, st));
-
   const LmPlan plan = lm_plan_of(cfg);
   const int L = plan.L, steps = plan.steps();
   const bool count = cfg->count_in_view && normal_eq;
+
+  LmGroups G = lm_groups_of(B, false);
+  LmSideStreams* side = nullptr;
+  std::unique_lock<std::mutex> side_lock;
+  {
+    hipStreamCaptureStatus cap = hipStreamCaptureStatusNone;
+    int d = -1;
+    if (hipStreamIsCapturing(st, &cap) != hipSuccess || hipGetDevice(&d) != hipSuccess) { (void)hipGetLastError(); d = -1; }
+    if (lm_may_split(B, hla_prof_on(), cap != hipStreamCaptureStatusNone, cfg->reach_mode) && d >= 0 && d < 64) {
+      side_lock = std::unique_lock<std::mutex>(g_lm_side[d].mu);
+      if (lm_side_create(g_lm_side[d])) side = &g_lm_side[d];
+      else side_lock.unlock();
+    }
+  }
+  if (side) G = lm_groups_of(B, true);
+  const int ng = G.ng;
+  const int* gb0 = G.b0;
+  const bool under = lm_under_decoder(G, cfg->group0_ready != nullptr, cfg->group0_samples) && !count && cfg->optimizer != 2;
+  hipStream_t gst[LM_GROUPS];
+  for (int g = 0; g < ng; ++g) gst[g] = g == 0 ? st : side->side[g];
+  if (under) { gst[0] = side->side[1]; gst[1] = st; }
+  int forked = 0;
+  hipError_t err = hipSuccess;
+  if (under) {
+    err = hipStreamWaitEvent(gst[0], (hipEvent_t)cfg->group0_ready, 0);
+    if (err == hipSuccess) forked = 1;
+    else { (void)hipGetLastError(); return HLA_ERR_HIP; }
+  }
+
+  if (pose0) {
+    if (!under) HLA_CHECK_HIP(hipMemcpyAsync(pose, pose0, (size_t)B * 3 * sizeof(float), hipMemcpyDeviceToDevice, st));
+    else
+      for (int g = 0; g < ng && err == hipSuccess; ++g)
+        err = hipMemcpyAsync(pose + (size_t)gb0[g] * 3, pose0 + (size_t)gb0[g] * 3, (size_t)(gb0[g + 1] - gb0[g]) * 3 * sizeof(float),
+                             hipMemcpyDeviceToDevice, gst[g]);
+  }
   if (count) HLA_CHECK_HIP(hipMemsetAsync(in_view, 0, (size_t)B * steps * sizeof(int), st));
   if (cfg->optimizer == 2) HLA_CHECK_HIP(hipMemsetAsync(adam, 0, (size_t)B * 6 * sizeof(double), st));
   SolveArgs sa{};
@@ -451,41 +483,24 @@
   sa.zero_ticket = ticket; sa.zero_steps = steps; sa.zero_pose = pose0 ? 0 : 1;
   sa.reach_clear = cfg->reach_mode == 1 ? cfg->reach_flag : nullptr;
   sa.gate = cfg->reach_mode == 2 ? cfg->reach_flag : nullptr;
-  hipLaunchKernelGGL(lm_solve, dim3(B), dim3(64), 0, st, sa);
+  if (!under) hipLaunchKernelGGL(lm_solve, dim3(B), dim3(64), 0, st, sa, 0);
+  else
+    for (int g = 0; g < ng && err == hipSuccess; ++g) hipLaunchKernelGGL(lm_solve, dim3(gb0[g + 1] - gb0[g]), dim3(64), 0, gst[g], sa, gb0[g]);
   sa.zero_ticket = nullptr; sa.zero_steps = 0; sa.zero_pose = 0; sa.reach_clear = nullptr;
 
-  int ng = 1, gb0[LM_GROUPS + 1] = {0};
-  LmSideStreams* side = nullptr;
-  std::unique_lock<std::mutex> side_lock;
-  if (B >= LM_SPLIT_MIN && !hla_prof_on() && cfg->reach_mode != 2) {
-    hipStreamCaptureStatus cap = hipStreamCaptureStatusNone;
-    int d = -1;
-    if (hipStreamIsCapturing(st, &cap) != hipSuccess || hipGetDevice(&d) != hipSuccess) { (void)hipGetLastError(); d = -1; }
-    if (cap == hipStreamCaptureStatusNone && d >= 0 && d < 64) {
-      side_lock = std::unique_lock<std::mutex>(g_lm_side[d].mu);
-      if (lm_side_create(g_lm_side[d])) side = &g_lm_side[d];
-      else side_lock.unlock();
-    }
-  }
-  if (side) {
-    const int oct = (B + 7) / 8;
-    ng = oct < LM_GROUPS ? oct : LM_GROUPS;
-    for (int g = 0; g < ng; ++g) gb0[g + 1] = gb0[g] + 8 * (oct / ng + (g < oct % ng ? 1 : 0));
-  }
-  gb0[ng] = B;
-  hipStream_t gst[LM_GROUPS];
-  gst[0] = st;
-  int forked = 0;
-  hipError_t err = hipSuccess;
-  if (ng > 1) {
+  if (ng > 1 && !under) {
     err = hipEventRecord(side->fork, st);
     for (int g = 1; g < ng && err == hipSuccess; ++g) {
-      gst[g] = side->side[g];
       err = hipStreamWaitEvent(gst[g], side->fork, 0);
       if (err == hipSuccess) forked = g;
     }
   }
 
+#ifndef HLA_LM_UNDER_GROUPED
+#define HLA_LM_UNDER_GROUPED 1
+#endif
+  const bool grouped = under && HLA_LM_UNDER_GROUPED;
+  for (int only = grouped ? 0 : -1; only < (grouped ? ng : 0); ++only)
   for (int k = 0; k < steps && err == hipSuccess; ++k) {
     const int l = plan.level(k);
     const hla_s2g_level& v = lv[l];
@@ -507,6 +522,7 @@
     else sa.coef = nullptr;
     const double esz = v.feat_dtype == HLA_F32 ? 4.0 : 2.0;
     for (int g = 0; g < ng; ++g) {
+      if (only >= 0 && g != only) continue;
       hipStream_t gs = gst[g];
       aa.b0 = gb0[g]; aa.nb = gb0[g + 1] - gb0[g];
       if (count)
@@ -520,7 +536,7 @@
     }
   }
   for (int g = 1; g <= forked; ++g) {
-    hipError_t e = hipEventRecord(side->join[g], gst[g]);
+    hipError_t e = hipEventRecord(side->join[g], side->side[g]);
     if (e == hipSuccess) e = hipStreamWaitEvent(st, side->join[g], 0);
     if (err == hipSuccess) err = e;
   }
diff --git a/highlyaccurate_amd/csrc/split_plan.h b/highlyaccurate_amd/csrc/split_plan.h
--- /dev/null
+++ b/highlyaccurate_amd/csrc/split_plan.h
@@ -0,0 +1,31 @@
+#pragma once
+
+constexpr int kVggSplitFirstLayer = 9;
+static inline bool vgg_split_b_ok(int split_b, int B) { return split_b > 0 && split_b < B && split_b % 8 == 0; }
+static inline bool vgg_split_applies(bool paired, bool sixteen_bit, bool prof_on) { return paired && sixteen_bit && !prof_on; }
+
+constexpr int LM_GROUPS = 2;
+constexpr int LM_SPLIT_MIN = 16;
+static_assert(LM_GROUPS >= 2 && LM_GROUPS <= 4 && LM_SPLIT_MIN > 8, "a batch of up to 8 samples is one XCD octet and never splits");
+
+struct LmGroups { int ng, b0[LM_GROUPS + 1]; };
+static inline bool lm_may_split(int B, bool prof_on, bool capturing, int reach_mode) {
+  return B >= LM_SPLIT_MIN && !prof_on && !capturing && reach_mode != 2;
+}
+static inline LmGroups lm_groups_of(int B, bool split) {
+  LmGroups g{1, {0}};
+  if (split) {
+    const int oct = (B + 7) / 8;
+    g.ng = oct < LM_GROUPS ? oct : LM_GROUPS;
+    for (int k = 0; k < g.ng; ++k) g.b0[k + 1] = g.b0[k] + 8 * (oct / g.ng + (k < oct % g.ng ? 1 : 0));
+  }
+  g.b0[g.ng] = B;
+  return g;
+}
+static inline int lm_split_b(int B) {
+  const LmGroups g = lm_groups_of(B, B >= LM_SPLIT_MIN);
+  return g.ng > 1 ? g.b0[1] : 0;
+}
+static inline bool lm_under_decoder(const LmGroups& g, bool has_event, int group0_samples) {
+  return has_event && g.ng == 2 && g.b0[1] == group0_samples;
+}
diff --git a/highlyaccurate_amd/csrc/vgg.hip b/highlyaccurate_amd/csrc/vgg.hip
--- a/highlyaccurate_amd/csrc/vgg.hip
+++ b/highlyaccurate_amd/csrc/vgg.hip
@@ -1,5 +1,6 @@
 #include "conv_kernels.h"
 #include "vgg_layers.h"
+#include "split_plan.h"
 #include <type_traits>
 
 template <typename T>
@@ -141,9 +142,9 @@
   return HLA_OK;
 }
 
-static int vgg_norms(int nb, const VggFwdCall* const* net, const VggConvSet* S, int NL) {
+static int vgg_norms(int nb, const VggFwdCall* const* net, const VggConvSet* S, int NL, int b0 = 0, int range_n = 0) {
   const VggFwdCall& c0 = *net[0];
-  const int B = c0.B;
+  const int B = c0.B, nB = range_n > 0 ? range_n : B;
   hipStream_t st = c0.st;
   InvNormArgs ia{};
   ia.gate = c0.col_gate;
@@ -151,12 +152,12 @@
   for (int k = 0; k < nb; ++k)
     for (int l = 0; l < NL; ++l) {
       const VggFwdCall& n = *net[k];
-      ia.ss[k * NL + l] = (const double*)(n.ws + n.pl.ss[l]); ia.np[k * NL + l] = S[k].np_used[l];
-      ia.inv[k * NL + l] = (n.inv_norm ? n.inv_norm : (double*)(n.ws + n.pl.inv)) + (size_t)l * B;
-      bytes += (double)B * n.pl.np[l] * 8;
+      ia.ss[k * NL + l] = (const double*)(n.ws + n.pl.ss[l]) + (size_t)b0 * S[k].np_used[l]; ia.np[k * NL + l] = S[k].np_used[l];
+      ia.inv[k * NL + l] = (n.inv_norm ? n.inv_norm : (double*)(n.ws + n.pl.inv)) + (size_t)l * B + b0;
+      bytes += (double)nB * n.pl.np[l] * 8;
     }
   hla_prof_begin(K_L2NORM, 0, bytes, st);
-  hipLaunchKernelGGL(inv_norm_multi_kernel, dim3(B, nb * NL), dim3(256), 0, st, ia);
+  hipLaunchKernelGGL(inv_norm_multi_kernel, dim3(nB, nb * NL), dim3(256), 0, st, ia);
   hla_prof_end(st);
   for (int k = 0; k < nb; ++k)
     for (int l = 0; l < NL; ++l) {
@@ -241,14 +242,28 @@
 
 constexpr int HLA_PAIR_FALLBACK = -1000;
 template <typename T>
-int vgg_forward_pair_t(const VggFwdCall c[2]) {
+static ConvArgs conv_sample_range(ConvArgs a, int b0, int nb, int np) {
+  static_assert(!Prec<T>::SPLIT, "the split-fp16 mode's per-sample maxima are not moved");
+  const size_t px = (size_t)a.H * a.W, px1 = a.up1 ? (size_t)(a.H >> 1) * (a.W >> 1) : px, es = sizeof(T);
+  auto at = [b0](auto* p, size_t bytes_per_sample) { return p ? (decltype(p))((char*)p + (size_t)b0 * bytes_per_sample) : p; };
+  a.src1 = at((char*)a.src1, px1 * a.C1 * es);
+  a.src2 = at((char*)a.src2, px * a.C2 * es);
+  a.out_act = at((char*)a.out_act, px * a.Cout * es);
+  a.out_raw = (float*)at((char*)a.out_raw, px * a.Cout * (a.raw16 ? sizeof(f16) : sizeof(float)));
+  a.sumsq = at(a.sumsq, (size_t)np * sizeof(double));
+  a.B = nb;
+  return a;
+}
+template <typename T>
+int vgg_forward_pair_t(const VggFwdCall c[2], const hla_vgg_split* sp) {
   constexpr bool SPLIT = Prec<T>::SPLIT;
   hipStream_t st = c[0].st;
   VggConvSet S[2];
   for (int k = 0; k < 2; ++k) vgg_build_convs<T>(c[k], false, S[k]);
+  const int whole_end = sp ? kVggSplitFirstLayer : kAllLayers;
   for (int l = 2; l < kAllLayers; ++l) {
     if (S[0].used[l] != S[1].used[l]) return HLA_PAIR_FALLBACK;
-    if (!S[0].used[l]) continue;
+    if (!S[0].used[l] || l >= whole_end) continue;
     ConvArgs a0 = S[0].conv[l], a1 = S[1].conv[l];
     if (conv_plan<T, false>(a0, S[0].pool[l]).small != conv_plan<T, false>(a1, S[1].pool[l]).small) return HLA_PAIR_FALLBACK;
   }
@@ -257,10 +272,33 @@
       HLA_CHECK_HIP(hipMemsetAsync(c[k].ws + c[k].pl.amax, 0, (size_t)kAmaxSlots * c[k].B * sizeof(unsigned), st));
   if (const int rc = launch_conv02<T>(st, S[0].c02, &S[1].c02)) return rc;
   bool launch_ok = true;
-  for (int l = 2; l < kAllLayers; ++l)
+  for (int l = 2; l < whole_end; ++l)
     if (S[0].used[l] && !launch_conv_pair<T>(st, S[0].conv[l], S[1].conv[l], S[0].pool[l])) launch_ok = false;
   const VggFwdCall* nets[2] = {&c[0], &c[1]};
-  if (const int rc = vgg_norms(2, nets, S, 3)) return rc;
+  if (!sp) {
+    if (const int rc = vgg_norms(2, nets, S, 3)) return rc;
+  } else if constexpr (!SPLIT) {
+    const int B = c[0].B, cut[3] = {0, sp->split_b, B};
+    hipError_t ev = hipSuccess;
+    for (int r = 0; r < 2; ++r) {
+      const int b0 = cut[r], nb = cut[r + 1] - cut[r];
+      for (int l = whole_end; l < kAllLayers; ++l) {
+        if (!S[0].used[l]) continue;
+        const int lvl = kFwd[l].level;
+        ConvArgs a0 = conv_sample_range<T>(S[0].conv[l], b0, nb, lvl >= 0 ? S[0].np_used[lvl] : 0);
+        ConvArgs a1 = conv_sample_range<T>(S[1].conv[l], b0, nb, lvl >= 0 ? S[1].np_used[lvl] : 0);
+        ConvArgs p0 = a0, p1 = a1;
+        const bool pool = S[0].pool[l];
+        if (conv_plan<T, false>(p0, pool).small == conv_plan<T, false>(p1, pool).small) {
+          if (!launch_conv_pair<T>(st, a0, a1, pool)) launch_ok = false;
+        } else if (!launch_conv<T>(st, a0, pool) || !launch_conv<T>(st, a1, pool))
+          launch_ok = false;
+      }
+      if (const int rc = vgg_norms(2, nets, S, 3, b0, nb)) return rc;
+      if (r == 0) ev = hipEventRecord((hipEvent_t)sp->ready, st);
+    }
+    HLA_CHECK_HIP(ev);
+  }
   HLA_CHECK_HIP(hipGetLastError());
   return launch_ok ? HLA_OK : HLA_ERR_ARG;
 }
@@ -298,7 +336,7 @@
 #endif
 template void vgg_pack_all<TuT>(const hla_vgg_params* prm, char* packed, int dtype, hipStream_t st);
 template int vgg_forward_t<TuT>(const VggFwdCall& c);
-template int vgg_forward_pair_t<TuT>(const VggFwdCall c[2]);
+template int vgg_forward_pair_t<TuT>(const VggFwdCall c[2], const hla_vgg_split* sp);
 #if HLA_TU_DTYPE == 1 || HLA_TU_DTYPE == 2
 template int vgg_fixup_t<TuT>(const VggFwdCall& c);
 #endif
@@ -306,7 +344,7 @@
 #define HLA_EXTERN_T(T) \
   extern template void vgg_pack_all<T>(const hla_vgg_params* prm, char* packed, int dtype, hipStream_t st); \
   extern template int vgg_forward_t<T>(const VggFwdCall& c); \
-  extern template int vgg_forward_pair_t<T>(const VggFwdCall c[2]);
+  extern template int vgg_forward_pair_t<T>(const VggFwdCall c[2], const hla_vgg_split* sp);
 HLA_EXTERN_T(float) HLA_EXTERN_T(bf16) HLA_EXTERN_T(f16) HLA_EXTERN_T(split32)
 extern template int vgg_fixup_t<bf16>(const VggFwdCall& c);
 extern template int vgg_fixup_t<f16>(const VggFwdCall& c);
@@ -435,8 +473,21 @@
 }
 
 extern "C" int hla_vgg_forward_pair(const hla_vgg_branch br[2], int B, int level, int dtype, int flags, int* paired_out, hla_stream_t stream) {
+  return hla_vgg_forward_pair_split(br, B, level, dtype, flags, nullptr, paired_out, nullptr, stream);
+}
+
+extern "C" int hla_vgg_forward_pair_split(const hla_vgg_branch br[2], int B, int level, int dtype, int flags, const hla_vgg_split* split,
+                                          int* paired_out, int* split_out, hla_stream_t stream) {
   HLA_REQUIRE(br, "hla_vgg_forward_pair: null argument");
   if (paired_out) *paired_out = 0;
+  if (split_out) *split_out = 0;
+  HLA_REQUIRE(!split || (split->ready && vgg_split_b_ok(split->split_b, B)),
+              "hla_vgg_forward_pair_split: split_b must be a multiple of 8 with 0 < split_b < B, and the event is required (got %d, B = %d)",
+              split ? split->split_b : 0, B);
+  auto hand_over = [&](int rc) -> int {
+    if (rc == HLA_OK && split) HLA_CHECK_HIP(hipEventRecord((hipEvent_t)split->ready, (hipStream_t)stream));
+    return rc;
+  };
   auto plain = [&]() -> int {
     for (int k = 0; k < 2; ++k)
       if (const int rc = hla_vgg_forward_cols(br[k].x, br[k].x_plane, br[k].params, br[k].packed_weights, br[k].feat, br[k].conf, br[k].inv_norm,
@@ -445,17 +496,19 @@
         return rc;
     return HLA_OK;
   };
-  if (level != 3 || (flags & (HLA_VGG_SAVE_FOR_BACKWARD | HLA_VGG_FOLD_DECODER | HLA_VGG_WANT_CONF)) || !hla_dtype_ok(dtype)) return plain();
+  if (level != 3 || (flags & (HLA_VGG_SAVE_FOR_BACKWARD | HLA_VGG_FOLD_DECODER | HLA_VGG_WANT_CONF)) || !hla_dtype_ok(dtype)) return hand_over(plain());
   VggFwdCall c[2];
   for (int k = 0; k < 2; ++k) {
     const hla_vgg_branch& b = br[k];
     c[k] = VggFwdCall{b.x, b.x_plane, b.params, (const char*)b.packed_weights, b.feat, nullptr, b.inv_norm, (char*)b.workspace,
                       b.workspace_bytes, B, b.H, b.W, level, dtype, flags, b.first_row8, b.first_col32, nullptr, (hipStream_t)stream, {}};
-    if (vgg_forward_check(c[k], true) != HLA_OK) return plain();
-  }
-  const int rc = hla_dispatch_dtype(dtype, [&](auto t) { return vgg_forward_pair_t<typename decltype(t)::type>(c); });
-  if (rc == HLA_PAIR_FALLBACK) return plain();
+    if (vgg_forward_check(c[k], true) != HLA_OK) return hand_over(plain());
+  }
+  const bool ranges = split && vgg_split_applies(true, dtype == HLA_BF16 || dtype == HLA_F16, hla_prof_on());
+  const int rc = hla_dispatch_dtype(dtype, [&](auto t) { return vgg_forward_pair_t<typename decltype(t)::type>(c, ranges ? split : nullptr); });
+  if (rc == HLA_PAIR_FALLBACK) return hand_over(plain());
   if (rc == HLA_OK && paired_out) *paired_out = 1;
-  return rc;
+  if (rc == HLA_OK && ranges && split_out) *split_out = 1;
+  return ranges ? rc : hand_over(rc);
 }
 #endif
diff --git a/include/hla.h b/include/hla.h
--- a/include/hla.h
+++ b/include/hla.h
@@ -26,13 +26,13 @@
 
 const char* hla_last_error(void);
 
-#define HLA_ABI_VERSION 32
+#define HLA_ABI_VERSION 33
 int hla_abi_version(void);
 const char* hla_source_hash(void);
 typedef enum hla_struct_id {
   HLA_STRUCT_VGG_PARAMS = 0, HLA_STRUCT_VGG_GRADS = 1, HLA_STRUCT_S2G_LEVEL = 2, HLA_STRUCT_S2G_CONFIG = 3,
   HLA_STRUCT_S2G_LEVEL_GRAD = 4, HLA_STRUCT_PROF_RECORD = 5, HLA_STRUCT_POSE_LOSS_ARGS = 6, HLA_STRUCT_FILL_REGION = 7,
-  HLA_STRUCT_VGG_BRANCH = 8
+  HLA_STRUCT_VGG_BRANCH = 8, HLA_STRUCT_VGG_SPLIT = 9
 } hla_struct_id;
 size_t hla_sizeof_struct(int id);
 
@@ -84,6 +84,14 @@
 } hla_vgg_branch;
 
 int hla_vgg_forward_pair(const hla_vgg_branch br[2], int B, int level, int dtype, int flags, int* paired_out, hla_stream_t stream);
+
+typedef struct hla_vgg_split {
+  int split_b;
+  void* ready;
+} hla_vgg_split;
+
+int hla_vgg_forward_pair_split(const hla_vgg_branch br[2], int B, int level, int dtype, int flags, const hla_vgg_split* split,
+                               int* paired_out, int* split_out, hla_stream_t stream);
 
 typedef struct hla_vgg_grads {
   float* dw[17];
@@ -162,9 +170,12 @@
   int reach_mode;
   int* reach_flag;
   int reach_col0[4];
+  void* group0_ready;
+  int group0_samples;
 } hla_s2g_config;
 
 size_t hla_s2g_workspace_bytes(const hla_s2g_config* cfg, const hla_s2g_level* levels, int B);
+int hla_s2g_split_b(int B);
 
 int hla_s2g_lm_solve(const hla_s2g_config* cfg, const hla_s2g_level* levels, const float* R_FL,
                      const float* T_FL, const float* pose0, const float* rand_uv, float* trace,
```

After: 6114 pairs/s. About the same (-0.8%).
